# Visual-Behavior/detr-tensorflow

Measured on AMD Instinct MI355X. Metric: images/sec training step, DETR-R50 800x1333 bs=8/GPU, higher is better.
Workload: dtype bf16

## Files before the change

### detr-tensorflow_amd/csrc/common.h

```cpp
#pragma once
#include <hip/hip_runtime.h>
#include <stdint.h>
#include <stdio.h>
#include <stdarg.h>
#include <stdlib.h>

#include "../../include/detr_hip.h"

namespace detr {

void set_error(const char *fmt, ...);

#define DETR_REQUIRE(cond, ...)                 \
    do {                                        \
        if (!(cond)) {                          \
            ::detr::set_error(__VA_ARGS__);     \
            return -1;                          \
        }                                       \
    } while (0)

#define DETR_LAUNCH_CHECK(name)                                                         \
    do {                                                                                \
        hipError_t e__ = hipGetLastError();                                             \
        if (e__ != hipSuccess) {                                                        \
            ::detr::set_error("%s: launch failed: %s", name, hipGetErrorString(e__));   \
            return -2;                                                                  \
        }                                                                               \
    } while (0)

void launch_splitk_reduce(const float *ws, int splits, long long part_stride, int rows, int cols, float *C, long long ldc,
                          float alpha, const float *scale, hipStream_t stream, const float *rs_ws = nullptr,
                          float *rs_out = nullptr, float rs_alpha = 1.0f, int ts_bm = 0, int ts_bn = 0, int ts_tiles_n = 0);

constexpr int MIN_WAVES_64X64 = 1;

#if defined(__HIPCC__)
__device__ __forceinline__ void wave_lds_sync() {
    __builtin_amdgcn_fence(__ATOMIC_SEQ_CST, "wavefront");
    __builtin_amdgcn_wave_barrier();
}
__device__ __forceinline__ void lds_barrier() {
    __builtin_amdgcn_fence(__ATOMIC_RELEASE, "workgroup", "local");
    __builtin_amdgcn_s_barrier();
    __builtin_amdgcn_fence(__ATOMIC_ACQUIRE, "workgroup", "local");
}
#endif

enum TuneKey {
    T_GEMM_TILE,
    T_SPLIT_XCD,
    T_GEMM_STREAM,
    T_GEMM_GROUP,
    T_STREAM_SL,
    T_STREAM_NW,
    T_CONV_HALO,
    T_CONV_TILE,
    T_DGRAD_S2_CLASSES,
    T_WGRAD_FUSED,
    T_WGRAD_FUSED_WGS,
    T_WGRAD_TILE,
    T_STEM_ROWS,
    T_ATTN_WAVES,
    T_ATTN_SPLIT,
    T_GEMM_K64,
    T_EPI_WIDE,
    T_SLAB_TS,
    T_GEMM_RING,
    T_RING_NS,
    T_RING_BN,
    T_RING_WGS,
    T_RING_ROWS,
    T_RING_WTILE,
    T_CONV_DMA,
    T_SPLIT3_T128,
    T_X3_DB,
    T_X3_T192,
    T_X3_WG_ROUNDS,
    T_X3_CONV,
    T_SPLIT3_ALL,
    T_COUNT
};
int tune(TuneKey k);

static inline bool aligned16(const void *p) { return (reinterpret_cast<uintptr_t>(p) & 15) == 0; }
static inline int cdiv(long long a, long long b) { return (int)((a + b - 1) / b); }

__host__ __device__ __forceinline__ uint32_t mix32(uint32_t x) {
    x ^= x >> 16; x *= 0x7feb352du;
    x ^= x >> 15; x *= 0x846ca68bu;
    x ^= x >> 16;
    return x;
}
__host__ __device__ __forceinline__ uint32_t drop_key(uint32_t site, const uint32_t *step) {
    return mix32((step ? *step : 0u) + site * 0x9E3779B9u);
}
__host__ __device__ __forceinline__ uint32_t drop_hash(uint32_t key, unsigned long long pair) {
    const uint32_t key2 = key * 0x85EBCA6Bu + 0xC2B2AE35u;
    uint32_t x = (uint32_t)pair ^ key;
    x ^= (uint32_t)(pair >> 32) * 0x9E3779B9u;
    x ^= x >> 16; x *= 0x7feb352du;
    x ^= key2;
    x ^= x >> 15; x *= 0x846ca68bu;
    x ^= x >> 16;
    return x;
}
__host__ __device__ __forceinline__ bool drop_keep(uint32_t key, unsigned long long idx, uint32_t thresh16) {
    const uint32_t h = drop_hash(key, idx >> 1);
    return ((idx & 1ull) ? (h >> 16) : (h & 0xFFFFu)) >= thresh16;
}
static inline uint32_t drop_thresh16(float p) { return (uint32_t)(p * 65536.0f); }

template <int CTRL, int ROW_MASK>
__device__ __forceinline__ float dpp_mov_f32(float identity, float x) {
    return __builtin_bit_cast(float, __builtin_amdgcn_update_dpp(__builtin_bit_cast(int, identity), __builtin_bit_cast(int, x),
                                                                 CTRL, ROW_MASK, 0xf, false));
}
__device__ __forceinline__ float wave_sum(float v) {
    v += dpp_mov_f32<0x111, 0xf>(0.0f, v);
    v += dpp_mov_f32<0x112, 0xf>(0.0f, v);
    v += dpp_mov_f32<0x114, 0xf>(0.0f, v);
    v += dpp_mov_f32<0x118, 0xf>(0.0f, v);
    v += dpp_mov_f32<0x142, 0xa>(0.0f, v);
    v += dpp_mov_f32<0x143, 0xc>(0.0f, v);
    return __builtin_bit_cast(float, __builtin_amdgcn_readlane(__builtin_bit_cast(int, v), 63));
}
__device__ __forceinline__ float wave_max(float v) {
    const float ninf = -INFINITY;
    v = fmaxf(v, dpp_mov_f32<0x111, 0xf>(ninf, v));
    v = fmaxf(v, dpp_mov_f32<0x112, 0xf>(ninf, v));
    v = fmaxf(v, dpp_mov_f32<0x114, 0xf>(ninf, v));
    v = fmaxf(v, dpp_mov_f32<0x118, 0xf>(ninf, v));
    v = fmaxf(v, dpp_mov_f32<0x142, 0xa>(ninf, v));
    v = fmaxf(v, dpp_mov_f32<0x143, 0xc>(ninf, v));
    return __builtin_bit_cast(float, __builtin_amdgcn_readlane(__builtin_bit_cast(int, v), 63));
}

}
```

### detr-tensorflow_amd/csrc/common.hip

```cpp
#include "common.h"
#include <string.h>

namespace detr {
static thread_local char g_err[512] = "";
void set_error(const char *fmt, ...) {
    va_list ap;
    va_start(ap, fmt);
    vsnprintf(g_err, sizeof(g_err), fmt, ap);
    va_end(ap);
}
static const char *const g_tune_names[T_COUNT] = {
    "DETR_HIP_GEMM_TILE",
    "DETR_HIP_SPLIT_XCD",
    "DETR_HIP_GEMM_STREAM",
    "DETR_HIP_GEMM_GROUP",
    "DETR_HIP_STREAM_SL",
    "DETR_HIP_STREAM_NW",
    "DETR_HIP_CONV_HALO",
    "DETR_HIP_CONV_TILE",
    "DETR_HIP_DGRAD_S2_CLASSES",
    "DETR_HIP_WGRAD_FUSED",
    "DETR_HIP_WGRAD_FUSED_WGS",
    "DETR_HIP_WGRAD_TILE",
    "DETR_HIP_STEM_ROWS",
    "DETR_HIP_ATTN_WAVES",
    "DETR_HIP_ATTN_SPLIT",
    "DETR_HIP_GEMM_K64",
    "DETR_HIP_EPI_WIDE",
    "DETR_HIP_SLAB_TS",
    "DETR_HIP_GEMM_RING",
    "DETR_HIP_RING_NS",
    "DETR_HIP_RING_BN",
    "DETR_HIP_RING_WGS",
    "DETR_HIP_RING_ROWS",
    "DETR_HIP_RING_WTILE",
    "DETR_HIP_CONV_DMA",
    "DETR_HIP_SPLIT3_T128",
    "DETR_HIP_X3_DB",
    "DETR_HIP_X3_T192",
    "DETR_HIP_X3_WG_ROUNDS",
    "DETR_HIP_X3_CONV",
    "DETR_HIP_SPLIT3_ALL",
};
static int g_tune[T_COUNT];
static void load_tuning() {
    for (int i = 0; i < T_COUNT; ++i) {
        const char *v = getenv(g_tune_names[i]);
        __atomic_store_n(&g_tune[i], v ? atoi(v) : 0, __ATOMIC_RELAXED);
    }
}
static const bool g_tune_loaded = (load_tuning(), true);
int tune(TuneKey k) { return __atomic_load_n(&g_tune[k], __ATOMIC_RELAXED); }
}

extern "C" int detr_hip_reload_tuning(void) {
    detr::load_tuning();
    return 0;
}
extern "C" const char *detr_hip_last_error(void) { return detr::g_err; }
extern "C" int detr_hip_abi_version(void) { return DETR_HIP_ABI_VERSION; }
__global__ __launch_bounds__(256) void zero_fill_kernel(uint4 *__restrict__ p16, size_t n16, unsigned char *__restrict__ tail, int ntail) {
    const uint4 z = make_uint4(0u, 0u, 0u, 0u);
    for (size_t i = blockIdx.x * (size_t)blockDim.x + threadIdx.x; i < n16; i += (size_t)gridDim.x * blockDim.x) p16[i] = z;
    if (blockIdx.x == 0 && (int)threadIdx.x < ntail) tail[threadIdx.x] = 0;
}

extern "C" int detr_hip_memset_zero(void *ptr, size_t bytes, void *stream) {
    if (bytes == 0) return 0;
    unsigned char *b = reinterpret_cast<unsigned char *>(ptr);
    const size_t head = (16 - (reinterpret_cast<uintptr_t>(b) & 15)) & 15;
    if (head >= bytes || bytes < 64) {
        if (bytes > 255) { detr::set_error("memset_zero: %zu unaligned bytes", bytes); return -2; }
        hipLaunchKernelGGL(zero_fill_kernel, dim3(1), dim3(256), 0, (hipStream_t)stream, nullptr, (size_t)0, b, (int)bytes);
    } else {
        if (head) hipLaunchKernelGGL(zero_fill_kernel, dim3(1), dim3(256), 0, (hipStream_t)stream, nullptr, (size_t)0, b, (int)head);
        const size_t n16 = (bytes - head) / 16;
        const int ntail = (int)((bytes - head) % 16);
        size_t grid = (n16 + 255) / 256;
        if (grid > 2048) grid = 2048;
        if (grid < 1) grid = 1;
        hipLaunchKernelGGL(zero_fill_kernel, dim3((unsigned)grid), dim3(256), 0, (hipStream_t)stream, reinterpret_cast<uint4 *>(b + head), n16,
                           b + head + n16 * 16, ntail);
    }
    hipError_t e = hipGetLastError();
    if (e != hipSuccess) {
        detr::set_error("memset_zero: %s", hipGetErrorString(e));
        return -2;
    }
    return 0;
}
#include <stddef.h>
#define DETR_OFF(S, f) (int32_t)offsetof(S, f)
extern "C" int detr_hip_struct_layout(int32_t which, int32_t *out, int32_t cap) {
    int n = 0;
#define DETR_PUT(v) do { if (n < cap) out[n] = (v); ++n; } while (0)
    switch (which) {
    case 0:
        DETR_PUT((int32_t)sizeof(detr_reduce_desc));
        DETR_PUT(DETR_OFF(detr_reduce_desc, ws)); DETR_PUT(DETR_OFF(detr_reduce_desc, splits)); DETR_PUT(DETR_OFF(detr_reduce_desc, part_stride));
        DETR_PUT(DETR_OFF(detr_reduce_desc, rows)); DETR_PUT(DETR_OFF(detr_reduce_desc, cols)); DETR_PUT(DETR_OFF(detr_reduce_desc, C));
        DETR_PUT(DETR_OFF(detr_reduce_desc, ldc)); DETR_PUT(DETR_OFF(detr_reduce_desc, alpha)); DETR_PUT(DETR_OFF(detr_reduce_desc, scale));
        DETR_PUT(DETR_OFF(detr_reduce_desc, rs_ws)); DETR_PUT(DETR_OFF(detr_reduce_desc, rs_out)); DETR_PUT(DETR_OFF(detr_reduce_desc, rs_alpha));
        DETR_PUT(DETR_OFF(detr_reduce_desc, ts_bm)); DETR_PUT(DETR_OFF(detr_reduce_desc, ts_bn)); DETR_PUT(DETR_OFF(detr_reduce_desc, ts_tiles_n));
        break;
    case 1:
        DETR_PUT((int32_t)sizeof(detr_gemm_desc));
        DETR_PUT(DETR_OFF(detr_gemm_desc, M)); DETR_PUT(DETR_OFF(detr_gemm_desc, N)); DETR_PUT(DETR_OFF(detr_gemm_desc, K));
        DETR_PUT(DETR_OFF(detr_gemm_desc, A)); DETR_PUT(DETR_OFF(detr_gemm_desc, lda)); DETR_PUT(DETR_OFF(detr_gemm_desc, a_kcontig));
        DETR_PUT(DETR_OFF(detr_gemm_desc, B)); DETR_PUT(DETR_OFF(detr_gemm_desc, ldb)); DETR_PUT(DETR_OFF(detr_gemm_desc, b_kcontig));
        DETR_PUT(DETR_OFF(detr_gemm_desc, C)); DETR_PUT(DETR_OFF(detr_gemm_desc, ldc)); DETR_PUT(DETR_OFF(detr_gemm_desc, batch));
        DETR_PUT(DETR_OFF(detr_gemm_desc, batch_inner)); DETR_PUT(DETR_OFF(detr_gemm_desc, sA0)); DETR_PUT(DETR_OFF(detr_gemm_desc, sA1));
        DETR_PUT(DETR_OFF(detr_gemm_desc, sB0)); DETR_PUT(DETR_OFF(detr_gemm_desc, sB1)); DETR_PUT(DETR_OFF(detr_gemm_desc, sC0));
        DETR_PUT(DETR_OFF(detr_gemm_desc, sC1)); DETR_PUT(DETR_OFF(detr_gemm_desc, alpha)); DETR_PUT(DETR_OFF(detr_gemm_desc, scale));
        DETR_PUT(DETR_OFF(detr_gemm_desc, bias)); DETR_PUT(DETR_OFF(detr_gemm_desc, residual)); DETR_PUT(DETR_OFF(detr_gemm_desc, ldr));
        DETR_PUT(DETR_OFF(detr_gemm_desc, mask)); DETR_PUT(DETR_OFF(detr_gemm_desc, ldmask)); DETR_PUT(DETR_OFF(detr_gemm_desc, act));
        DETR_PUT(DETR_OFF(detr_gemm_desc, split_k)); DETR_PUT(DETR_OFF(detr_gemm_desc, workspace)); DETR_PUT(DETR_OFF(detr_gemm_desc, workspace_bytes));
        DETR_PUT(DETR_OFF(detr_gemm_desc, dropout_p)); DETR_PUT(DETR_OFF(detr_gemm_desc, dropout_seed)); DETR_PUT(DETR_OFF(detr_gemm_desc, compute));
        DETR_PUT(DETR_OFF(detr_gemm_desc, rowsum_a)); DETR_PUT(DETR_OFF(detr_gemm_desc, rowsum_alpha)); DETR_PUT(DETR_OFF(detr_gemm_desc, b_dtype));
        DETR_PUT(DETR_OFF(detr_gemm_desc, a_dtype)); DETR_PUT(DETR_OFF(detr_gemm_desc, c_dtype)); DETR_PUT(DETR_OFF(detr_gemm_desc, r_dtype));
        DETR_PUT(DETR_OFF(detr_gemm_desc, m_dtype)); DETR_PUT(DETR_OFF(detr_gemm_desc, dropout_step)); DETR_PUT(DETR_OFF(detr_gemm_desc, defer_out));
        DETR_PUT(DETR_OFF(detr_gemm_desc, maskbits_out)); DETR_PUT(DETR_OFF(detr_gemm_desc, ld_maskbits_out));
        DETR_PUT(DETR_OFF(detr_gemm_desc, ln_gamma)); DETR_PUT(DETR_OFF(detr_gemm_desc, ln_beta)); DETR_PUT(DETR_OFF(detr_gemm_desc, ln_y));
        DETR_PUT(DETR_OFF(detr_gemm_desc, ln_mean)); DETR_PUT(DETR_OFF(detr_gemm_desc, ln_rstd)); DETR_PUT(DETR_OFF(detr_gemm_desc, ln_add));
        DETR_PUT(DETR_OFF(detr_gemm_desc, ln_add_rows)); DETR_PUT(DETR_OFF(detr_gemm_desc, ln_y2)); DETR_PUT(DETR_OFF(detr_gemm_desc, ln_y16));
        DETR_PUT(DETR_OFF(detr_gemm_desc, ln_eps));
        break;
    case 2:
        DETR_PUT((int32_t)sizeof(detr_conv3x3_desc));
        DETR_PUT(DETR_OFF(detr_conv3x3_desc, N)); DETR_PUT(DETR_OFF(detr_conv3x3_desc, Hi)); DETR_PUT(DETR_OFF(detr_conv3x3_desc, Wi));
        DETR_PUT(DETR_OFF(detr_conv3x3_desc, Ci)); DETR_PUT(DETR_OFF(detr_conv3x3_desc, Ho)); DETR_PUT(DETR_OFF(detr_conv3x3_desc, Wo));
        DETR_PUT(DETR_OFF(detr_conv3x3_desc, Co)); DETR_PUT(DETR_OFF(detr_conv3x3_desc, stride)); DETR_PUT(DETR_OFF(detr_conv3x3_desc, pad));
        DETR_PUT(DETR_OFF(detr_conv3x3_desc, x)); DETR_PUT(DETR_OFF(detr_conv3x3_desc, w)); DETR_PUT(DETR_OFF(detr_conv3x3_desc, y));
        DETR_PUT(DETR_OFF(detr_conv3x3_desc, alpha)); DETR_PUT(DETR_OFF(detr_conv3x3_desc, scale)); DETR_PUT(DETR_OFF(detr_conv3x3_desc, bias));
        DETR_PUT(DETR_OFF(detr_conv3x3_desc, residual)); DETR_PUT(DETR_OFF(detr_conv3x3_desc, mask)); DETR_PUT(DETR_OFF(detr_conv3x3_desc, act));
        DETR_PUT(DETR_OFF(detr_conv3x3_desc, split)); DETR_PUT(DETR_OFF(detr_conv3x3_desc, workspace)); DETR_PUT(DETR_OFF(detr_conv3x3_desc, workspace_bytes));
        DETR_PUT(DETR_OFF(detr_conv3x3_desc, compute)); DETR_PUT(DETR_OFF(detr_conv3x3_desc, w_dtype)); DETR_PUT(DETR_OFF(detr_conv3x3_desc, x_dtype));
        DETR_PUT(DETR_OFF(detr_conv3x3_desc, y_dtype)); DETR_PUT(DETR_OFF(detr_conv3x3_desc, r_dtype)); DETR_PUT(DETR_OFF(detr_conv3x3_desc, m_dtype));
        DETR_PUT(DETR_OFF(detr_conv3x3_desc, maskbits_out));
        break;
    case 3:
        DETR_PUT((int32_t)sizeof(detr_stem_desc));
        DETR_PUT(DETR_OFF(detr_stem_desc, N)); DETR_PUT(DETR_OFF(detr_stem_desc, H)); DETR_PUT(DETR_OFF(detr_stem_desc, W));
        DETR_PUT(DETR_OFF(detr_stem_desc, Ho)); DETR_PUT(DETR_OFF(detr_stem_desc, Wo)); DETR_PUT(DETR_OFF(detr_stem_desc, img));
        DETR_PUT(DETR_OFF(detr_stem_desc, w)); DETR_PUT(DETR_OFF(detr_stem_desc, y)); DETR_PUT(DETR_OFF(detr_stem_desc, alpha));
        DETR_PUT(DETR_OFF(detr_stem_desc, scale)); DETR_PUT(DETR_OFF(detr_stem_desc, bias)); DETR_PUT(DETR_OFF(detr_stem_desc, act));
        DETR_PUT(DETR_OFF(detr_stem_desc, split)); DETR_PUT(DETR_OFF(detr_stem_desc, workspace)); DETR_PUT(DETR_OFF(detr_stem_desc, workspace_bytes));
        DETR_PUT(DETR_OFF(detr_stem_desc, compute)); DETR_PUT(DETR_OFF(detr_stem_desc, w_dtype)); DETR_PUT(DETR_OFF(detr_stem_desc, y_dtype));
        break;
    case 4:
        DETR_PUT((int32_t)sizeof(detr_layernorm_desc));
        DETR_PUT(DETR_OFF(detr_layernorm_desc, rows)); DETR_PUT(DETR_OFF(detr_layernorm_desc, C)); DETR_PUT(DETR_OFF(detr_layernorm_desc, eps));
        DETR_PUT(DETR_OFF(detr_layernorm_desc, x)); DETR_PUT(DETR_OFF(detr_layernorm_desc, gamma)); DETR_PUT(DETR_OFF(detr_layernorm_desc, beta));
        DETR_PUT(DETR_OFF(detr_layernorm_desc, y)); DETR_PUT(DETR_OFF(detr_layernorm_desc, mean)); DETR_PUT(DETR_OFF(detr_layernorm_desc, rstd));
        DETR_PUT(DETR_OFF(detr_layernorm_desc, add)); DETR_PUT(DETR_OFF(detr_layernorm_desc, add_rows)); DETR_PUT(DETR_OFF(detr_layernorm_desc, y2));
        DETR_PUT(DETR_OFF(detr_layernorm_desc, y16)); DETR_PUT(DETR_OFF(detr_layernorm_desc, dy)); DETR_PUT(DETR_OFF(detr_layernorm_desc, dx));
        DETR_PUT(DETR_OFF(detr_layernorm_desc, dgamma)); DETR_PUT(DETR_OFF(detr_layernorm_desc, dbeta)); DETR_PUT(DETR_OFF(detr_layernorm_desc, workspace));
        DETR_PUT(DETR_OFF(detr_layernorm_desc, workspace_bytes)); DETR_PUT(DETR_OFF(detr_layernorm_desc, dx_add));
        DETR_PUT(DETR_OFF(detr_layernorm_desc, dx_drop)); DETR_PUT(DETR_OFF(detr_layernorm_desc, dropout_p)); DETR_PUT(DETR_OFF(detr_layernorm_desc, dropout_site));
        DETR_PUT(DETR_OFF(detr_layernorm_desc, dropout_step)); DETR_PUT(DETR_OFF(detr_layernorm_desc, dx_drop16));
        DETR_PUT(DETR_OFF(detr_layernorm_desc, defer_blocks_out)); DETR_PUT(DETR_OFF(detr_layernorm_desc, dy_add));
        break;
    case 5:
        DETR_PUT((int32_t)sizeof(detr_attn_desc));
        DETR_PUT(DETR_OFF(detr_attn_desc, B)); DETR_PUT(DETR_OFF(detr_attn_desc, H)); DETR_PUT(DETR_OFF(detr_attn_desc, T));
        DETR_PUT(DETR_OFF(detr_attn_desc, S)); DETR_PUT(DETR_OFF(detr_attn_desc, q)); DETR_PUT(DETR_OFF(detr_attn_desc, ldq));
        DETR_PUT(DETR_OFF(detr_attn_desc, k)); DETR_PUT(DETR_OFF(detr_attn_desc, ldk)); DETR_PUT(DETR_OFF(detr_attn_desc, v));
        DETR_PUT(DETR_OFF(detr_attn_desc, ldv)); DETR_PUT(DETR_OFF(detr_attn_desc, o)); DETR_PUT(DETR_OFF(detr_attn_desc, ldo));
        DETR_PUT(DETR_OFF(detr_attn_desc, lse)); DETR_PUT(DETR_OFF(detr_attn_desc, d_o)); DETR_PUT(DETR_OFF(detr_attn_desc, ldd_o));
        DETR_PUT(DETR_OFF(detr_attn_desc, dq)); DETR_PUT(DETR_OFF(detr_attn_desc, lddq)); DETR_PUT(DETR_OFF(detr_attn_desc, dk));
        DETR_PUT(DETR_OFF(detr_attn_desc, lddk)); DETR_PUT(DETR_OFF(detr_attn_desc, dv)); DETR_PUT(DETR_OFF(detr_attn_desc, lddv));
        DETR_PUT(DETR_OFF(detr_attn_desc, delta)); DETR_PUT(DETR_OFF(detr_attn_desc, scale)); DETR_PUT(DETR_OFF(detr_attn_desc, dropout_p));
        DETR_PUT(DETR_OFF(detr_attn_desc, dropout_site)); DETR_PUT(DETR_OFF(detr_attn_desc, dropout_step)); DETR_PUT(DETR_OFF(detr_attn_desc, compute));
        DETR_PUT(DETR_OFF(detr_attn_desc, io_dtype)); DETR_PUT(DETR_OFF(detr_attn_desc, dropmask));
        break;
    case 6:
        DETR_PUT((int32_t)sizeof(detr_setloss_desc));
        DETR_PUT(DETR_OFF(detr_setloss_desc, levels)); DETR_PUT(DETR_OFF(detr_setloss_desc, B)); DETR_PUT(DETR_OFF(detr_setloss_desc, Q));
        DETR_PUT(DETR_OFF(detr_setloss_desc, C)); DETR_PUT(DETR_OFF(detr_setloss_desc, R)); DETR_PUT(DETR_OFF(detr_setloss_desc, logits));
        DETR_PUT(DETR_OFF(detr_setloss_desc, sL_l)); DETR_PUT(DETR_OFF(detr_setloss_desc, sL_b)); DETR_PUT(DETR_OFF(detr_setloss_desc, sL_q));
        DETR_PUT(DETR_OFF(detr_setloss_desc, boxes)); DETR_PUT(DETR_OFF(detr_setloss_desc, sB_l)); DETR_PUT(DETR_OFF(detr_setloss_desc, sB_b));
        DETR_PUT(DETR_OFF(detr_setloss_desc, sB_q)); DETR_PUT(DETR_OFF(detr_setloss_desc, t_bbox)); DETR_PUT(DETR_OFF(detr_setloss_desc, t_class));
        DETR_PUT(DETR_OFF(detr_setloss_desc, background_class));
        break;
    case 7:
        DETR_PUT((int32_t)sizeof(detr_input_desc));
        DETR_PUT(DETR_OFF(detr_input_desc, B)); DETR_PUT(DETR_OFF(detr_input_desc, Hs)); DETR_PUT(DETR_OFF(detr_input_desc, Ws));
        DETR_PUT(DETR_OFF(detr_input_desc, Hd)); DETR_PUT(DETR_OFF(detr_input_desc, Wd)); DETR_PUT(DETR_OFF(detr_input_desc, src));
        DETR_PUT(DETR_OFF(detr_input_desc, src_batch_stride)); DETR_PUT(DETR_OFF(detr_input_desc, dst)); DETR_PUT(DETR_OFF(detr_input_desc, lut));
        DETR_PUT(DETR_OFF(detr_input_desc, perm)); DETR_PUT(DETR_OFF(detr_input_desc, interpolation));
        break;
    case 8:
        DETR_PUT((int32_t)sizeof(detr_postprocess_desc));
        DETR_PUT(DETR_OFF(detr_postprocess_desc, B)); DETR_PUT(DETR_OFF(detr_postprocess_desc, Q)); DETR_PUT(DETR_OFF(detr_postprocess_desc, C));
        DETR_PUT(DETR_OFF(detr_postprocess_desc, logits)); DETR_PUT(DETR_OFF(detr_postprocess_desc, sL_b)); DETR_PUT(DETR_OFF(detr_postprocess_desc, sL_q));
        DETR_PUT(DETR_OFF(detr_postprocess_desc, boxes)); DETR_PUT(DETR_OFF(detr_postprocess_desc, sB_b)); DETR_PUT(DETR_OFF(detr_postprocess_desc, sB_q));
// ... 76 lines not shown
```

### detr-tensorflow_amd/csrc/gemm_f32.hip

```cpp
#include "gemm_core.h"
#include "gemm_bf16_core.h"
#include "gemm_stream.h"

#include "gemm_kernels.h"
#include "gemm_x3.h"
#include "gemm_ring.h"

namespace detr {

struct ReduceOne {
    const float *ws; int splits; long long part_stride; int rows, cols; float *C; long long ldc;
    float alpha; const float *scale; int vec; const float *rs_ws; float *rs_out; float rs_alpha; int nblocks;
    int ts_bm, ts_bn, ts_tn;
};
struct ReduceGroupArgs { ReduceOne r[GEMM_MAX_GROUP]; };

template <int G>
__device__ __forceinline__ void splitk_reduce_body(const float *__restrict__ ws, int splits, long long part_stride,
                                                   int rows, int cols, float *__restrict__ C, long long ldc,
                                                   float alpha, const float *__restrict__ scale, int vec,
                                                   const float *__restrict__ rs_ws, float *__restrict__ rs_out,
                                                   float rs_alpha, const int bid, const int nbid,
                                                   const int ts_bm = 0, const int ts_bn = 0, const int ts_tn = 1) {
    constexpr int OUT = 256 / G;
    __shared__ float4 red[G][OUT];
    if (rs_ws) {
        for (int m = bid * 256 + threadIdx.x; m < rows; m += nbid * 256) {
            float t = 0.0f;
            for (int k = 0; k < splits; ++k) t += rs_ws[(long long)k * rows + m];
            rs_out[m] += rs_alpha * t;
        }
    }
    const int lo = threadIdx.x % OUT, grp = threadIdx.x / OUT;
    if (ts_bm > 0) {
        __shared__ float tr[OUT][5];
        const int upt = (ts_bm * ts_bn) >> 2;
        const long long total = part_stride >> 2;
        for (long long base = (long long)bid * OUT; base < total; base += (long long)nbid * OUT) {
            const long long i = base + lo;
            const bool valid = i < total;
            float4 s = make_float4(0.f, 0.f, 0.f, 0.f);
            if (valid) {
                const float *p = ws + i * 4;
#pragma unroll 4
                for (int k = grp; k < splits; k += G) {
                    const float4 v = *reinterpret_cast<const float4 *>(p + k * part_stride);
                    s.x += v.x; s.y += v.y; s.z += v.z; s.w += v.w;
                }
            }
            red[grp][lo] = s;
            __syncthreads();
            if (grp == 0) {
#pragma unroll
                for (int q = 1; q < G; ++q) {
                    const float4 t = red[q][lo];
                    s.x += t.x; s.y += t.y; s.z += t.z; s.w += t.w;
                }
                tr[lo][0] = s.x; tr[lo][1] = s.y; tr[lo][2] = s.z; tr[lo][3] = s.w;
            }
            __syncthreads();
            if (grp == 0 && valid) {
                const int qb = lo & ~3, t = lo & 3;
                const long long iq = base + qb;
                const int tile = (int)(iq / upt), u = (int)(iq - (long long)tile * upt);
                int row0, col;
                slab_ts_unit(u, ts_bm, ts_bn, row0, col);
                const int row = row0 + (tile / ts_tn) * ts_bm + t;
                col += (tile % ts_tn) * ts_bn;
                if (row < rows && col < cols) {
                    const float4 v = make_float4(tr[qb][t], tr[qb + 1][t], tr[qb + 2][t], tr[qb + 3][t]);
                    float4 sc = make_float4(1.f, 1.f, 1.f, 1.f);
                    if (scale) sc = *reinterpret_cast<const float4 *>(scale + col);
                    float4 *dst = reinterpret_cast<float4 *>(C + (long long)row * ldc + col);
                    float4 o = *dst;
                    o.x += alpha * sc.x * v.x; o.y += alpha * sc.y * v.y; o.z += alpha * sc.z * v.z; o.w += alpha * sc.w * v.w;
                    *dst = o;
                }
            }
        }
    } else if (vec) {
        const int c4n = cols >> 2;
        const long long total = (long long)rows * c4n;
        for (long long base = (long long)bid * OUT; base < total; base += (long long)nbid * OUT) {
            const long long i = base + lo;
            const bool valid = i < total;
            int r = 0, c = 0;
            float4 s = make_float4(0.f, 0.f, 0.f, 0.f);
            if (valid) {
                r = (int)(i / c4n);
                c = (int)(i - (long long)r * c4n) * 4;
                const float *p = ws + (long long)r * cols + c;
#pragma unroll 4
                for (int k = grp; k < splits; k += G) {
                    const float4 v = *reinterpret_cast<const float4 *>(p + k * part_stride);
                    s.x += v.x; s.y += v.y; s.z += v.z; s.w += v.w;
                }
            }
            red[grp][lo] = s;
            __syncthreads();
            if (grp == 0 && valid) {
#pragma unroll
                for (int q = 1; q < G; ++q) {
                    const float4 t = red[q][lo];
                    s.x += t.x; s.y += t.y; s.z += t.z; s.w += t.w;
                }
                float4 sc = make_float4(1.f, 1.f, 1.f, 1.f);
                if (scale) sc = *reinterpret_cast<const float4 *>(scale + c);
                float4 *dst = reinterpret_cast<float4 *>(C + (long long)r * ldc + c);
                float4 o = *dst;
                o.x += alpha * sc.x * s.x; o.y += alpha * sc.y * s.y; o.z += alpha * sc.z * s.z; o.w += alpha * sc.w * s.w;
                *dst = o;
            }
            __syncthreads();
        }
    } else {
        const long long total = (long long)rows * cols;
        for (long long i = bid * (long long)blockDim.x + threadIdx.x; i < total; i += (long long)nbid * blockDim.x) {
            const int r = (int)(i / cols), c = (int)(i - (long long)r * cols);
            float s = 0.f;
            for (int k = 0; k < splits; ++k) s += ws[k * part_stride + i];
            C[(long long)r * ldc + c] += alpha * (scale ? scale[c] : 1.0f) * s;
        }
    }
}

template <int G>
__global__ __launch_bounds__(256) void splitk_reduce_kernel(const float *__restrict__ ws, int splits, long long part_stride,
                                                            int rows, int cols, float *__restrict__ C, long long ldc,
                                                            float alpha, const float *__restrict__ scale, int vec,
                                                            const float *__restrict__ rs_ws, float *__restrict__ rs_out,
                                                            float rs_alpha, int ts_bm, int ts_bn, int ts_tn) {
    splitk_reduce_body<G>(ws, splits, part_stride, rows, cols, C, ldc, alpha, scale, vec, rs_ws, rs_out, rs_alpha, blockIdx.x,
                          gridDim.x, ts_bm, ts_bn, ts_tn);
}
template <int G>
__global__ __launch_bounds__(256) void splitk_reduce_group_kernel(ReduceGroupArgs R) {
    const ReduceOne &r = R.r[blockIdx.y];
    if ((int)blockIdx.x >= r.nblocks) return;
    splitk_reduce_body<G>(r.ws, r.splits, r.part_stride, r.rows, r.cols, r.C, r.ldc, r.alpha, r.scale, r.vec, r.rs_ws, r.rs_out,
                          r.rs_alpha, blockIdx.x, r.nblocks, r.ts_bm, r.ts_bn, r.ts_tn);
}

constexpr int REDUCE_MANY = 16;
struct ReduceManyArgs { ReduceOne r[REDUCE_MANY]; };
template <int G>
__global__ __launch_bounds__(256) void splitk_reduce_many_kernel(ReduceManyArgs R) {
    const ReduceOne &r = R.r[blockIdx.y];
    if ((int)blockIdx.x >= r.nblocks) return;
    splitk_reduce_body<G>(r.ws, r.splits, r.part_stride, r.rows, r.cols, r.C, r.ldc, r.alpha, r.scale, r.vec, r.rs_ws, r.rs_out,
                          r.rs_alpha, blockIdx.x, r.nblocks, r.ts_bm, r.ts_bn, r.ts_tn);
}

static void reduce_plan(ReduceOne &r, bool &small) {
    r.vec = (r.cols % 4 == 0) && (r.ldc % 4 == 0) && (r.part_stride % 4 == 0) && aligned16(r.ws) && aligned16(r.C) &&
            (!r.scale || aligned16(r.scale));
    const bool ts = r.ts_bm > 0;
    const bool vec_like = r.vec || ts;
    const long long total = (long long)r.rows * (vec_like ? r.cols / 4 : r.cols);
    small = vec_like && total <= 65536 && r.splits >= 8;
    const long long units = ts ? r.part_stride / 4 : total;
    long long grid = vec_like ? (units + (small ? 15 : 63)) / (small ? 16 : 64) : (units + 255) / 256;
    if (grid > 8192) grid = 8192;
    if (grid < 1) grid = 1;
    r.nblocks = (int)grid;
}

void launch_splitk_reduce(const float *ws, int splits, long long part_stride, int rows, int cols, float *C, long long ldc,
                          float alpha, const float *scale, hipStream_t stream, const float *rs_ws, float *rs_out,
                          float rs_alpha, int ts_bm, int ts_bn, int ts_tiles_n) {
    ReduceOne r;
    r.ws = ws; r.splits = splits; r.part_stride = part_stride; r.rows = rows; r.cols = cols; r.C = C; r.ldc = ldc;
    r.alpha = alpha; r.scale = scale; r.rs_ws = rs_ws; r.rs_out = rs_out; r.rs_alpha = rs_alpha;
    r.ts_bm = ts_bm; r.ts_bn = ts_bn; r.ts_tn = ts_tiles_n > 0 ? ts_tiles_n : 1;
    bool small;
    reduce_plan(r, small);
    if (small)
        hipLaunchKernelGGL(splitk_reduce_kernel<16>, dim3((unsigned)r.nblocks), dim3(256), 0, stream, ws, splits, part_stride, rows, cols,
                           C, ldc, alpha, scale, r.vec, rs_ws, rs_out, rs_alpha, r.ts_bm, r.ts_bn, r.ts_tn);
    else
        hipLaunchKernelGGL(splitk_reduce_kernel<4>, dim3((unsigned)r.nblocks), dim3(256), 0, stream, ws, splits, part_stride, rows, cols,
                           C, ldc, alpha, scale, r.vec, rs_ws, rs_out, rs_alpha, r.ts_bm, r.ts_bn, r.ts_tn);
}

template <int BM, int BN, int WGM, int WGN>
static int launch_cfg(const GemmArgs &g, int batch, hipStream_t s, bool ak, bool bk) {
    GemmArgs a = g;
    a.tiles_m = cdiv(g.M, BM);
    a.tiles_n = cdiv(g.N, BN);
    dim3 grid((unsigned)(a.tiles_m * a.tiles_n), 1, (unsigned)(batch * g.split_k));
    dim3 block(GEMM_THREADS);
    if (ak && bk) hipLaunchKernelGGL((gemm_f32_kernel<BM, BN, WGM, WGN, true, true>), grid, block, 0, s, a);
    else if (ak && !bk) hipLaunchKernelGGL((gemm_f32_kernel<BM, BN, WGM, WGN, true, false>), grid, block, 0, s, a);
    else if (!ak && bk) hipLaunchKernelGGL((gemm_f32_kernel<BM, BN, WGM, WGN, false, true>), grid, block, 0, s, a);
    else hipLaunchKernelGGL((gemm_f32_kernel<BM, BN, WGM, WGN, false, false>), grid, block, 0, s, a);
    return 0;
}

template <int BM, int BN>
static int launch_x3(const GemmArgs &g, int batch, hipStream_t s, bool ak, bool bk) {
    GemmArgs a = g;
    a.tiles_m = cdiv(g.M, BM);
    a.tiles_n = cdiv(g.N, BN);
    dim3 grid((unsigned)(a.tiles_m * a.tiles_n), 1, (unsigned)(batch * g.split_k));
    dim3 block(GEMM_THREADS);
    const bool db = tune(T_X3_DB) == 1;
    if constexpr (BM == 192) {
        if (bk) hipLaunchKernelGGL((gemm_x3_kernel<BM, BN, true, true, false>), grid, block, 0, s, a);
        else hipLaunchKernelGGL((gemm_x3_kernel<BM, BN, true, false, false>), grid, block, 0, s, a);
    } else {
#define DETR_X3_LAUNCH(DB_)                                                                                              \
    do {                                                                                                                 \
        if (ak && bk) hipLaunchKernelGGL((gemm_x3_kernel<BM, BN, true, true, DB_>), grid, block, 0, s, a);               \
        else if (ak && !bk) hipLaunchKernelGGL((gemm_x3_kernel<BM, BN, true, false, DB_>), grid, block, 0, s, a);        \
        else if (!ak && bk) hipLaunchKernelGGL((gemm_x3_kernel<BM, BN, false, true, DB_>), grid, block, 0, s, a);        \
        else hipLaunchKernelGGL((gemm_x3_kernel<BM, BN, false, false, DB_>), grid, block, 0, s, a);                      \
    } while (0)
        if (db) {
            DETR_X3_LAUNCH(true);
        } else DETR_X3_LAUNCH(false);
    }
#undef DETR_X3_LAUNCH
    return 0;
}

template <int BM, int BN, int WGM, int WGN>
static int launch_cfg_bf16(const GemmArgs &g, int batch, hipStream_t s, bool ak, bool bk, int deep = 0) {
    GemmArgs a = g;
    a.tiles_m = cdiv(g.M, BM);
    a.tiles_n = cdiv(g.N, BN);
    dim3 grid((unsigned)(a.tiles_m * a.tiles_n), 1, (unsigned)(batch * g.split_k));
    dim3 block(GEMM_THREADS);
    if constexpr ((BM == 64 && BN == 64) || (BM == 128 && BN == 128)) {
        if (deep && g.a16 && g.b16) {
            if (ak && bk) hipLaunchKernelGGL((gemm_bf16c_k64_kernel<BM, BN, WGM, WGN, true, true>), grid, block, 0, s, a);
            else if (ak && !bk) hipLaunchKernelGGL((gemm_bf16c_k64_kernel<BM, BN, WGM, WGN, true, false>), grid, block, 0, s, a);
            else if (!ak && bk) hipLaunchKernelGGL((gemm_bf16c_k64_kernel<BM, BN, WGM, WGN, false, true>), grid, block, 0, s, a);
            else hipLaunchKernelGGL((gemm_bf16c_k64_kernel<BM, BN, WGM, WGN, false, false>), grid, block, 0, s, a);
            return 0;
        }
    }
#define DETR_BF16_LAUNCH(A16_, B16_)                                                                                          \
    do {                                                                                                                          \
        if (ak && bk) hipLaunchKernelGGL((gemm_bf16c_kernel<BM, BN, WGM, WGN, true, true, A16_, B16_>), grid, block, 0, s, a);        \
        else if (ak && !bk) hipLaunchKernelGGL((gemm_bf16c_kernel<BM, BN, WGM, WGN, true, false, A16_, B16_>), grid, block, 0, s, a); \
        else if (!ak && bk) hipLaunchKernelGGL((gemm_bf16c_kernel<BM, BN, WGM, WGN, false, true, A16_, B16_>), grid, block, 0, s, a); \
        else hipLaunchKernelGGL((gemm_bf16c_kernel<BM, BN, WGM, WGN, false, false, A16_, B16_>), grid, block, 0, s, a);               \
    } while (0)
    if (g.a16 && g.b16) DETR_BF16_LAUNCH(true, true);
    else if (g.a16) DETR_BF16_LAUNCH(true, false);
    else if (g.b16) DETR_BF16_LAUNCH(false, true);
    else DETR_BF16_LAUNCH(false, false);
#undef DETR_BF16_LAUNCH
    return 0;
}

}

using namespace detr;

struct GemmPlan {
    GemmArgs g;
    int batch, split;
    bool ak, bk, bf16c, partial;
    bool split3;
    int deep;
    int tile;
    long long part;
    int ts_bm, ts_bn, ts_tn;
    EpiArgs final_e;
    const detr_gemm_desc *d;
};

static bool gemm_split3_shape(const detr_gemm_desc *d) {
    return d->compute == 2 && d->N > 32 && (tune(T_SPLIT3_ALL) == 1 || (d->N >= 128 && d->K >= 256 && d->M >= 128));
}
static int gemm_pick_tile(const detr_gemm_desc *d, int split, int batch) {
    const bool bf16c = d->compute == 1;
    const int force = tune(T_GEMM_TILE);
    int tile = 0;
    if (bf16c) {
        const long long t128 = (long long)cdiv(d->M, 128) * cdiv(d->N, 128) * batch;
        const bool big_split = (d->N >= 128 && d->K >= 16384) || (d->M >= 512 && d->N >= 512 && d->K >= 4096) ||
                               (d->K >= 4096 && ((d->M >= 256 && d->N >= 2048) || (d->M >= 2048 && d->N >= 256)));
        const bool big_plain = (d->K >= 1024 && t128 >= 512) || (d->K >= 512 && d->N >= 512 && t128 >= 1024) ||
                               (d->K >= 512 && d->N >= 256 && t128 >= 2048);
        const bool small = (split > 1) ? !big_split : !big_plain;
        if (force == 2) tile = 2;
        else if (force == 5) tile = 4;
        else if (force == 3 || (force == 0 && small)) tile = 0;
        else if (force == 0 && split > 1 && d->M <= 64) tile = 4;
        else tile = 1;
        if (tile == 1 && split > 1 && batch == 1 && d->a_dtype == 1 && d->b_dtype == 1 && !d->a_kcontig && !d->b_kcontig && !d->rowsum_a &&
            tune(T_GEMM_RING) != 2 && tune(T_GEMM_RING) != 3 && tune(T_SLAB_TS) != 2 && d->M % 8 == 0 && d->N % 8 == 0 && d->lda % 8 == 0 &&
            d->ldb % 8 == 0 && aligned16(d->A) && aligned16(d->B) && aligned16(d->C) && d->ldc % 4 == 0 && (!d->scale || aligned16(d->scale))) {
            const int wt = tune(T_RING_WTILE);
            if (wt == 1 && d->N >= 256) tile = 6;
            else if (wt == 2 && d->M >= 256) tile = 7;
        }
    } else if (gemm_split3_shape(d)) {
        const long long t128 = (long long)cdiv(d->M, 128) * cdiv(d->N, 128) * batch * split;
        const int lim = tune(T_SPLIT3_T128) > 0 ? tune(T_SPLIT3_T128) : 192;
        if (force == 1 || (force == 0 && t128 >= lim)) tile = 1;
        else if (force == 2) tile = 2;
        else tile = 0;
        if (tile == 1 && force == 0 && split == 1 && batch == 1 && d->a_kcontig && !d->rowsum_a && tune(T_X3_T192) != 2) {
            const long long slots = 512;
            const long long t192 = (long long)cdiv(d->M, 192) * cdiv(d->N, 128);
            const long long r128 = (t128 + slots - 1) / slots, r192 = (t192 + slots - 1) / slots;
            if (tune(T_X3_T192) == 1 || 3 * r192 < 2 * r128) tile = 8;
        }
        if (tile == 1 && force == 0 && split == 1 && batch == 1 && tune(T_X3_T192) != 2 && d->M >= 4096) {
            const long long over = t128 % 512;
            if ((t128 > 512 && over > 0 && over <= 128) || (t128 <= 384 && d->K <= 512)) tile = 2;
        }
    } else if (force == 1) tile = 1;
    else if (force == 2) tile = 2;
    else if (force == 3) tile = 0;
    else if (force == 4) tile = 3;
    else if (force == 5) tile = 4;
    else if (force == 6) tile = 5;
    else if (d->N <= 32) tile = 3;
    else tile = 0;
    return tile;
}
static void gemm_tile_dims(bool bf16c, int tile, int &bm, int &bn, bool &ts_ok) {
    ts_ok = true;
    if (tile == 1) { bm = 128; bn = 128; }
    else if (tile == 8 && !bf16c) { bm = 192; bn = 128; }
    else if (tile == 6 && bf16c) { bm = 128; bn = 256; }
    else if (tile == 7 && bf16c) { bm = 256; bn = 128; }
    else if (tile == 2) { bm = 128; bn = 64; }
    else if (tile == 4 && bf16c) { bm = 64; bn = 128; }
    else if (tile == 0) { bm = 64; bn = 64; }
    else { bm = bn = 0; ts_ok = false; }
// ... 97 lines not shown
                 (!d->mask || bits_in || (d->ldmask % 8 == 0 && aligned16(d->mask))) && (!d->scale || aligned16(d->scale)) &&
                 (!d->bias || aligned16(d->bias)) && (tune(T_EPI_WIDE) != 2 || bits_in || bits_out);
    DETR_REQUIRE(!(bits_in || bits_out) || (bf16c && g.e.wide16 && (!bits_in || d->ldmask >= d->N / 8) && (!bits_out || d->ld_maskbits_out >= d->N / 8)),
                 "gemm: bit-packed masks need bf16 C / residual, N %% 8 == 0, 16-byte aligned rows, no split-K / batch, and a row pitch >= N / 8 bytes");

    const bool ak = d->a_kcontig != 0, bk = d->b_kcontig != 0;
    DETR_REQUIRE(!(bf16c && d->a_dtype == 1 && !ak) || (d->lda % 8 == 0 && d->M % 8 == 0 && aligned16(d->A)),
                 "gemm: an M-contiguous bf16 A operand needs lda %% 8 == 0, M %% 8 == 0 and a 16-byte aligned base (16-byte requests)");
    DETR_REQUIRE(!(bf16c && d->b_dtype == 1 && !bk) || (d->ldb % 8 == 0 && d->N % 8 == 0 && aligned16(d->B)),
                 "gemm: an N-contiguous bf16 B operand needs ldb %% 8 == 0, N %% 8 == 0 and a 16-byte aligned base (16-byte requests)");
    const int tile = gemm_pick_tile(d, split, batch);
    long long part = (long long)d->M * d->N;
    int ts_bm = 0, ts_bn = 0;
    const long long rs_extra = d->rowsum_a ? d->M : 0;
    bool ts = gemm_slab_ts(d, split, batch, tile, ts_bm, ts_bn);
    const long long part_ts = ts ? (long long)cdiv(d->M, ts_bm) * cdiv(d->N, ts_bn) * ts_bm * ts_bn : 0;
    const bool ws_ok = split > 1 && batch == 1 && d->workspace && aligned16(d->workspace);
    if (ts && !(ws_ok && d->workspace_bytes >= (long long)split * (part_ts + rs_extra) * 4)) ts = false;
    if (ts) part = part_ts;
    const bool partial = ws_ok && d->workspace_bytes >= (long long)split * (part + rs_extra) * 4;
    DETR_REQUIRE(!(d->rowsum_a && split > 1 && !partial), "gemm: rowsum_a with split_k needs the workspace path");
    g.rowsum = d->rowsum_a;
    g.rowsum_alpha = d->rowsum_alpha;
    g.rowsum_partial = 0;
    g.b16 = d->b_dtype == 1;
    g.a16 = d->a_dtype == 1;
    g.split_xcd = tune(T_SPLIT_XCD) != 2;
    g.slab_ts = 0;
    p.ts_bm = p.ts_bn = 0; p.ts_tn = 1;
    EpiArgs final_e = g.e;
    if (partial) {
        g.C = d->workspace;
        g.ldc = d->N;
        g.part_stride = part;
        g.e.alpha = 1.0f;
        g.e.scale = nullptr;
        g.e.atomic = 0;
        g.e.vec = (d->N % 4 == 0);
        if (ts) {
            g.slab_ts = 1;
            p.ts_bm = ts_bm; p.ts_bn = ts_bn; p.ts_tn = cdiv(d->N, ts_bn);
        }
        if (d->rowsum_a) {
            g.rowsum = d->workspace + (long long)split * part;
            g.rowsum_partial = 1;
        }
    }
    {
        const int k64 = tune(T_GEMM_K64);
        const int per_split = cdiv(d->K, split);
        p.deep = (bf16c && g.a16 && g.b16 && (tile == 0 || tile == 1) && k64 != 2 &&
                  (k64 == 1 || (per_split >= 512 && (tile == 0 || split > 1)))) ? 1 : 0;
    }
    p.batch = batch; p.split = split; p.ak = ak; p.bk = bk; p.bf16c = bf16c; p.partial = partial; p.tile = tile;
    p.split3 = gemm_split3_shape(d) && (tile == 0 || tile == 1 || tile == 2 || tile == 8);
    p.part = part; p.final_e = final_e; p.d = d;
    return 0;
}

static bool gemm_stream_eligible(const GemmPlan &p) {
    const detr_gemm_desc *d = p.d;
    const GemmArgs &g = p.g;
    if (!(p.bf16c && g.a16 && g.b16 && g.e.c16 && p.ak && p.batch == 1 && p.split == 1 && !g.rowsum)) return false;
    const bool ext = d->alpha != 1.0f || d->dropout_p > 0.0f;
    if (!((d->K == 64 || d->K == 128 || d->K == 256) && d->N % 64 == 0 && d->M >= ((d->K == 256 && d->N >= 1024) ? 4096 : 16384))) return false;
    if (d->scale || (ext && d->K != 256) || !(d->act == 0 || d->act == 1)) return false;
    if (d->residual && !(g.e.r16 && d->ldr % 8 == 0 && aligned16(d->residual))) return false;
    if (d->mask && g.e.m16 != 2 && !(g.e.m16 && d->ldmask % 8 == 0 && aligned16(d->mask))) return false;
    if (!(d->lda % 8 == 0 && d->ldb % 8 == 0 && d->ldc % 8 == 0 && aligned16(d->A) && aligned16(d->B) && aligned16(d->C))) return false;
    const long long ldm_eff = g.e.m16 == 2 ? 0 : d->ldmask;
    long long pitch = d->ldr > ldm_eff ? d->ldr : ldm_eff;
    if (d->ldc > pitch) pitch = d->ldc;
    const long long span = (long long)(d->M - 1) * pitch + d->N;
    if (span * 2 > BUF_MAX_BYTES) return false;
    if (d->maskbits_out && (p.bk || !d->residual || d->mask || ext)) return false;
    return tune(T_GEMM_STREAM) != 2;
}

static void gemm_stream_launch(const GemmPlan &p, hipStream_t s) {
    const detr_gemm_desc *d = p.d;
    StreamArgs a;
    a.M = d->M; a.N = d->N;
    a.A = reinterpret_cast<const unsigned short *>(d->A); a.lda = d->lda;
    a.B = reinterpret_cast<const unsigned short *>(d->B); a.ldb = d->ldb;
    a.C = reinterpret_cast<unsigned short *>(d->C); a.ldc = d->ldc;
    a.res = reinterpret_cast<const unsigned short *>(d->residual); a.ldr = d->ldr;
    a.mask = reinterpret_cast<const unsigned short *>(d->mask); a.ldm = d->ldmask;
    a.mbits_out = d->maskbits_out; a.ld_mbits = d->ld_maskbits_out;
    a.bias = d->bias;
    a.act = d->act;
    a.alpha = d->alpha;
    a.drop_scale = p.g.e.drop_scale; a.drop_thresh = p.g.e.drop_thresh; a.drop_seed = p.g.e.drop_seed; a.drop_step = p.g.e.drop_step;
    a.n_tiles = a.row_tiles = a.q = 0;
    const bool mb = d->mask && d->m_dtype == 2;
    if (d->K == 64) launch_gemm_stream<64>(a, p.bk, s, mb);
    else if (d->K == 128) launch_gemm_stream<128>(a, p.bk, s, mb);
    else launch_gemm_stream<256>(a, p.bk, s, mb);
}

static int gemm_ln_launch(const GemmPlan &p, hipStream_t s) {
    const detr_gemm_desc *d = p.d;
    const GemmArgs &g0 = p.g;
    DETR_REQUIRE(p.bf16c && d->N == LN_TILE_N && d->ldc == LN_TILE_N && p.ak && p.bk && g0.b16 && p.batch == 1 && p.split == 1,
                 "gemm + LayerNorm: needs compute = 1, N = ldc = 256, k-contiguous A and bf16 k-contiguous B, no batch / split_k");
    DETR_REQUIRE(d->act == 0 && !d->scale && !d->mask && !g0.e.c16 && !g0.e.r16 && !d->rowsum_a && !d->maskbits_out && d->K % 8 == 0,
                 "gemm + LayerNorm: epilogue is bias, alpha, dropout and an fp32 residual only (K %% 8 == 0)");
    DETR_REQUIRE(d->ln_gamma && d->ln_beta && d->ln_mean && d->ln_rstd && (!d->ln_y2 || (d->ln_add && d->ln_add_rows > 0)),
                 "gemm + LayerNorm: gamma, beta, mean, rstd are required (and add / add_rows with y2)");
    DETR_REQUIRE((!d->residual || (d->ldr % 4 == 0 && aligned16(d->residual))) && aligned16(d->C) && aligned16(d->ln_y) &&
                 (!d->bias || aligned16(d->bias)) && aligned16(d->ln_gamma) && aligned16(d->ln_beta) &&
                 (!d->ln_y2 || (aligned16(d->ln_y2) && aligned16(d->ln_add))) && (!d->ln_y16 || aligned16(d->ln_y16)),
                 "gemm + LayerNorm: rows must be 16-byte aligned");
    GemmArgs a = g0;
    a.tiles_m = cdiv(d->M, LN_TILE_M);
    a.tiles_n = 1;
    a.ln.gamma = d->ln_gamma; a.ln.beta = d->ln_beta; a.ln.y = d->ln_y; a.ln.mean = d->ln_mean; a.ln.rstd = d->ln_rstd;
    a.ln.add = d->ln_add; a.ln.add_rows = d->ln_add_rows; a.ln.y2 = d->ln_y2; a.ln.y16 = d->ln_y16; a.ln.eps = d->ln_eps;
    const dim3 grid((unsigned)a.tiles_m), block(GEMM_THREADS);
    if (g0.a16) hipLaunchKernelGGL(gemm_bf16c_ln_kernel<true>, grid, block, 0, s, a);
    else hipLaunchKernelGGL(gemm_bf16c_ln_kernel<false>, grid, block, 0, s, a);
    DETR_LAUNCH_CHECK("gemm + LayerNorm");
    if (d->defer_out) d->defer_out->splits = 0;
    return 0;
}

static bool gemm_ring_eligible(const GemmPlan &p, RingPlan &rp) {
    const detr_gemm_desc *d = p.d;
    const GemmArgs &g = p.g;
    const int mode = tune(T_GEMM_RING);
    if (mode == 2) return false;
    if (!(p.bf16c && g.a16 && g.b16 && p.ak && p.batch == 1 && p.split == 1 && !g.rowsum && !d->ln_y)) return false;
    if (!(d->K % RING_BK == 0 && d->K >= 2 * RING_BK && d->N >= 128 && d->N % 8 == 0 && d->lda % 8 == 0 && d->ldb % 8 == 0 && aligned16(d->A) &&
          aligned16(d->B))) return false;
    const bool tall = d->M >= 4096 && d->K >= 512;
    const bool dec_ffn = d->M >= 512 && d->K >= 1024;
    const bool k256 = d->K == 256 && d->N >= 1024 && (d->M >= 16384 || (d->M >= 4096 && !p.bk));
    if (mode != 1 && !(tall || dec_ffn || k256)) return false;
    return gemm_ring_plan(d->M, d->N, d->K, rp);
}

static bool gemm_ring_f32_eligible(const GemmPlan &p, RingPlan &rp) {
    const detr_gemm_desc *d = p.d;
    const GemmArgs &g = p.g;
    const int mode = tune(T_GEMM_RING);
    if (mode == 2) return false;
    if (p.bf16c || p.split3 || g.a16 || g.b16 || !p.ak || p.batch != 1 || p.split != 1 || g.rowsum || d->ln_y) return false;
    if (d->c_dtype || d->r_dtype || d->m_dtype) return false;
    if (!(d->K % 32 == 0 && d->K >= 64 && d->N >= 128 && d->lda % 4 == 0 && d->ldb % 4 == 0 && aligned16(d->A) && aligned16(d->B) &&
          (p.bk || d->N % 4 == 0))) return false;
    if (mode != 1 && !(d->M >= 16384)) return false;
    return gemm_ring_f32_plan(d->M, d->N, d->K, rp);
}

static int gemm_launch(const GemmPlan &p, hipStream_t s) {
    const GemmArgs &g = p.g;
    const detr_gemm_desc *d = p.d;
    const int batch = p.batch;
    const bool ak = p.ak, bk = p.bk;
    if (d->ln_y) return gemm_ln_launch(p, s);
    {
        RingPlan rp;
        const bool ring_first = tune(T_GEMM_STREAM) != 3 && gemm_ring_eligible(p, rp);
        if (!ring_first && gemm_stream_eligible(p)) {
            gemm_stream_launch(p, s);
            DETR_LAUNCH_CHECK("gemm (stream)");
            return 0;
        }
        if (ring_first) {
            if (gemm_ring_launch(g, bk, rp, s)) return -1;
            DETR_LAUNCH_CHECK("gemm (ring)");
            if (d->defer_out) d->defer_out->splits = 0;
            return 0;
        }
        if (gemm_ring_f32_eligible(p, rp)) {
            if (gemm_ring_f32_launch(g, bk, rp, s)) return -1;
            DETR_LAUNCH_CHECK("gemm (ring, fp32)");
            if (d->defer_out) d->defer_out->splits = 0;
            return 0;
        }
    }
    const bool ring_wgrad = p.bf16c && (p.tile == 1 || p.tile == 6 || p.tile == 7) && g.a16 && g.b16 && !ak && !bk && batch == 1 && p.split > 1 &&
                            g.slab_ts && !g.rowsum && d->M % 8 == 0 && d->N % 8 == 0 && d->lda % 8 == 0 && d->ldb % 8 == 0 && aligned16(d->A) &&
                            aligned16(d->B) && tune(T_GEMM_RING) != 2 && tune(T_GEMM_RING) != 3;
    DETR_REQUIRE(ring_wgrad || (p.tile != 6 && p.tile != 7), "gemm: the 128 x 256 / 256 x 128 tiles exist for the ring weight gradient only "
                 "(tile-ordered slabs in a workspace of detr_hip_workspace_bytes_gemm bytes are required)");
    if (ring_wgrad) {
        if (gemm_ring_wgrad_launch(g, p.ts_bm, p.ts_bn, p.split, s)) return -1;
    } else if (p.bf16c) {
        if (p.tile == 2) launch_cfg_bf16<128, 64, 2, 2>(g, batch, s, ak, bk);
        else if (p.tile == 4) launch_cfg_bf16<64, 128, 2, 2>(g, batch, s, ak, bk);
        else if (p.tile == 0) launch_cfg_bf16<64, 64, 2, 2>(g, batch, s, ak, bk, p.deep);
        else launch_cfg_bf16<128, 128, 2, 2>(g, batch, s, ak, bk, p.deep);
    } else if (p.split3 && p.tile == 8) launch_x3<192, 128>(g, batch, s, ak, bk);
    else if (p.split3 && p.tile == 1) launch_x3<128, 128>(g, batch, s, ak, bk);
    else if (p.split3 && p.tile == 2) launch_x3<128, 64>(g, batch, s, ak, bk);
    else if (p.split3) launch_x3<64, 64>(g, batch, s, ak, bk);
    else if (p.tile == 1) launch_cfg<128, 128, 2, 2>(g, batch, s, ak, bk);
    else if (p.tile == 2) launch_cfg<128, 64, 2, 2>(g, batch, s, ak, bk);
    else if (p.tile == 3) launch_cfg<128, 32, 4, 1>(g, batch, s, ak, bk);
    else if (p.tile == 4) launch_cfg<64, 256, 1, 4>(g, batch, s, ak, bk);
    else if (p.tile == 5) launch_cfg<256, 64, 4, 1>(g, batch, s, ak, bk);
    else launch_cfg<64, 64, 2, 2>(g, batch, s, ak, bk);
    DETR_LAUNCH_CHECK("gemm");
    if (p.partial && d->defer_out) {
        detr_reduce_desc *o = d->defer_out;
        o->ws = d->workspace; o->splits = p.split; o->part_stride = p.part; o->rows = d->M; o->cols = d->N;
        o->C = d->C; o->ldc = d->ldc; o->alpha = p.final_e.alpha; o->scale = p.final_e.scale;
        o->rs_ws = d->rowsum_a ? d->workspace + (long long)p.split * p.part : nullptr;
        o->rs_out = d->rowsum_a; o->rs_alpha = d->rowsum_alpha;
        o->ts_bm = p.ts_bm; o->ts_bn = p.ts_bn; o->ts_tiles_n = p.ts_tn;
        return 0;
    }
    if (d->defer_out) d->defer_out->splits = 0;
    if (p.partial) {
        launch_splitk_reduce(d->workspace, p.split, p.part, d->M, d->N, d->C, d->ldc, p.final_e.alpha, p.final_e.scale, s,
                             d->rowsum_a ? d->workspace + (long long)p.split * p.part : nullptr, d->rowsum_a, d->rowsum_alpha,
                             p.ts_bm, p.ts_bn, p.ts_tn);
        DETR_LAUNCH_CHECK("gemm split-k reduce");
    }
    return 0;
}

extern "C" int detr_hip_gemm_family(const detr_gemm_desc *d) {
    GemmPlan p;
    if (gemm_prepare(d, p)) return -1;
    if (d->ln_y) return 4;
    RingPlan rp;
    const bool ring_first = tune(T_GEMM_STREAM) != 3 && gemm_ring_eligible(p, rp);
    if (!ring_first && gemm_stream_eligible(p)) return 1;
    if (ring_first) return 2;
    if (gemm_ring_f32_eligible(p, rp)) return 3;
    const GemmArgs &g = p.g;
    const bool ring_wgrad = p.bf16c && (p.tile == 1 || p.tile == 6 || p.tile == 7) && g.a16 && g.b16 && !p.ak && !p.bk && p.batch == 1 && p.split > 1 &&
                            g.slab_ts && !g.rowsum && d->M % 8 == 0 && d->N % 8 == 0 && d->lda % 8 == 0 && d->ldb % 8 == 0 && aligned16(d->A) &&
                            aligned16(d->B) && tune(T_GEMM_RING) != 2 && tune(T_GEMM_RING) != 3;
    return ring_wgrad ? 5 : 0;
}

extern "C" int detr_hip_gemm_f32(const detr_gemm_desc *d, void *stream) {
    GemmPlan p;
    if (gemm_prepare(d, p)) return -1;
    return gemm_launch(p, (hipStream_t)stream);
}

template <bool AK, bool BKC>
static void launch_group_f32(const GemmGroupArgs &G, dim3 grid, hipStream_t s, bool split3) {
    if (split3) hipLaunchKernelGGL((gemm_x3_group_kernel<64, 64, AK, BKC>), grid, dim3(GEMM_THREADS), 0, s, G);
    else hipLaunchKernelGGL((gemm_f32_group_kernel<64, 64, 2, 2, AK, BKC>), grid, dim3(GEMM_THREADS), 0, s, G);
}
template <bool AK, bool BKC, bool A16, bool B16>
static void launch_group_bf16(const GemmGroupArgs &G, dim3 grid, hipStream_t s) {
    hipLaunchKernelGGL((gemm_bf16c_group_kernel<64, 64, 2, 2, AK, BKC, A16, B16>), grid, dim3(GEMM_THREADS), 0, s, G);
}

extern "C" int detr_hip_gemm_group_f32(const detr_gemm_desc *descs, int32_t n, void *stream) {
    DETR_REQUIRE(descs != nullptr && n >= 1 && n <= 64, "gemm group: 1..64 descriptors");
    hipStream_t s = (hipStream_t)stream;
    int done = 0;
    while (done < n) {
        const int m = (n - done) < GEMM_MAX_GROUP ? (n - done) : GEMM_MAX_GROUP;
        GemmPlan p[GEMM_MAX_GROUP];
        for (int i = 0; i < m; ++i) {
            DETR_REQUIRE(!descs[done + i].ln_y, "gemm group: the fused LayerNorm (ln_y) exists for single launches only");
            if (gemm_prepare(descs + done + i, p[i])) return -1;
        }
        bool same = m > 1 && tune(T_GEMM_GROUP) != 2;
        for (int i = 0; i < m && same; ++i)
            same = p[i].tile == 0 && p[i].batch == 1 && p[i].bf16c == p[0].bf16c && p[i].split3 == p[0].split3 && p[i].ak == p[0].ak && p[i].bk == p[0].bk &&
                   p[i].g.a16 == p[0].g.a16 && p[i].g.b16 == p[0].g.b16 && (p[i].split == 1 || p[i].partial) &&
                   !gemm_stream_eligible(p[i]);
        if (same) { RingPlan rp; for (int i = 0; i < m && same; ++i) same = !gemm_ring_eligible(p[i], rp) && !gemm_ring_f32_eligible(p[i], rp); }
        if (!same) {
            for (int i = 0; i < m; ++i)
                if (gemm_launch(p[i], s)) return -1;
            done += m;
            continue;
        }
        GemmGroupArgs G;
        G.n = m;
        G.work_off[0] = 0;
        for (int i = 0; i < m; ++i) {
            G.g[i] = p[i].g;
            G.g[i].tiles_m = cdiv(p[i].g.M, 64);
            G.g[i].tiles_n = cdiv(p[i].g.N, 64);
            G.work_off[i + 1] = G.work_off[i] + G.g[i].tiles_m * G.g[i].tiles_n * p[i].split;
        }
        for (int i = m; i < GEMM_MAX_GROUP; ++i) { G.g[i] = G.g[0]; G.work_off[i + 1] = G.work_off[m]; }
        const dim3 grid((unsigned)G.work_off[m]);
        const bool ak = p[0].ak, bk = p[0].bk, a16 = p[0].g.a16 != 0, b16 = p[0].g.b16 != 0;
#define DETR_GROUP_BF16(A16_, B16_)                                          \
    do {                                                                     \
        if (ak && bk) launch_group_bf16<true, true, A16_, B16_>(G, grid, s);    \
        else if (ak) launch_group_bf16<true, false, A16_, B16_>(G, grid, s);    \
        else if (bk) launch_group_bf16<false, true, A16_, B16_>(G, grid, s);    \
        else launch_group_bf16<false, false, A16_, B16_>(G, grid, s);           \
    } while (0)
        if (p[0].bf16c) {
            if (a16 && b16) DETR_GROUP_BF16(true, true);
            else if (a16) DETR_GROUP_BF16(true, false);
            else if (b16) DETR_GROUP_BF16(false, true);
            else DETR_GROUP_BF16(false, false);
        } else if (ak && bk) launch_group_f32<true, true>(G, grid, s, p[0].split3);
        else if (ak) launch_group_f32<true, false>(G, grid, s, p[0].split3);
        else if (bk) launch_group_f32<false, true>(G, grid, s, p[0].split3);
        else launch_group_f32<false, false>(G, grid, s, p[0].split3);
#undef DETR_GROUP_BF16
        DETR_LAUNCH_CHECK("gemm group");
        ReduceGroupArgs R;
        int nr = 0;
        unsigned rx = 1;
        bool all_small = true, any_small = false;
        for (int i = 0; i < m; ++i) {
            const detr_gemm_desc *d = p[i].d;
            if (d->defer_out) {
                detr_reduce_desc *o = d->defer_out;
                o->splits = 0;
                if (p[i].partial) {
                    o->ws = d->workspace; o->splits = p[i].split; o->part_stride = p[i].part; o->rows = d->M; o->cols = d->N;
                    o->C = d->C; o->ldc = d->ldc; o->alpha = p[i].final_e.alpha; o->scale = p[i].final_e.scale;
                    o->rs_ws = d->rowsum_a ? d->workspace + (long long)p[i].split * p[i].part : nullptr;
                    o->rs_out = d->rowsum_a; o->rs_alpha = d->rowsum_alpha;
                    o->ts_bm = p[i].ts_bm; o->ts_bn = p[i].ts_bn; o->ts_tiles_n = p[i].ts_tn;
                }
                continue;
            }
            if (!p[i].partial) continue;
            ReduceOne &r = R.r[nr];
            r.ws = d->workspace; r.splits = p[i].split; r.part_stride = p[i].part; r.rows = d->M; r.cols = d->N;
            r.C = d->C; r.ldc = d->ldc; r.alpha = p[i].final_e.alpha; r.scale = p[i].final_e.scale;
            r.rs_ws = d->rowsum_a ? d->workspace + (long long)p[i].split * p[i].part : nullptr;
            r.rs_out = d->rowsum_a; r.rs_alpha = d->rowsum_alpha;
            r.ts_bm = p[i].ts_bm; r.ts_bn = p[i].ts_bn; r.ts_tn = p[i].ts_tn;
            bool small;
            reduce_plan(r, small);
            all_small = all_small && small;
            any_small = any_small || small;
            rx = (unsigned)r.nblocks > rx ? (unsigned)r.nblocks : rx;
            ++nr;
        }
        if (nr > 0 && (all_small || !any_small)) {
            for (int i = nr; i < GEMM_MAX_GROUP; ++i) R.r[i] = R.r[0];
            if (all_small) hipLaunchKernelGGL(splitk_reduce_group_kernel<16>, dim3(rx, (unsigned)nr), dim3(256), 0, s, R);
            else hipLaunchKernelGGL(splitk_reduce_group_kernel<4>, dim3(rx, (unsigned)nr), dim3(256), 0, s, R);
            DETR_LAUNCH_CHECK("gemm group split-k reduce");
        } else if (nr > 0) {
            for (int i = 0; i < nr; ++i) {
                const ReduceOne &r = R.r[i];
                launch_splitk_reduce(r.ws, r.splits, r.part_stride, r.rows, r.cols, r.C, r.ldc, r.alpha, r.scale, s, r.rs_ws, r.rs_out,
                                     r.rs_alpha, r.ts_bm, r.ts_bn, r.ts_tn);
            }
            DETR_LAUNCH_CHECK("gemm group split-k reduce (sequential)");
        }
        done += m;
    }
    return 0;
}


extern "C" int detr_hip_splitk_reduce_many(const detr_reduce_desc *descs, int32_t n, void *stream) {
    DETR_REQUIRE(descs != nullptr && n >= 1, "splitk_reduce_many: bad args");
    hipStream_t s = (hipStream_t)stream;
    for (int pass = 0; pass < 2; ++pass) {
        ReduceManyArgs R;
        int cnt = 0;
        unsigned rx = 1;
        auto flush = [&]() {
            if (cnt == 0) return;
            for (int i = cnt; i < REDUCE_MANY; ++i) R.r[i] = R.r[0];
            if (pass == 0) hipLaunchKernelGGL(splitk_reduce_many_kernel<16>, dim3(rx, (unsigned)cnt), dim3(256), 0, s, R);
            else hipLaunchKernelGGL(splitk_reduce_many_kernel<4>, dim3(rx, (unsigned)cnt), dim3(256), 0, s, R);
            cnt = 0;
            rx = 1;
        };
        for (int i = 0; i < n; ++i) {
            const detr_reduce_desc &d = descs[i];
            if (d.splits <= 0) continue;
            DETR_REQUIRE(d.ws && d.C && d.rows > 0 && d.cols > 0, "splitk_reduce_many: entry %d is malformed", i);
            ReduceOne r;
            r.ws = d.ws; r.splits = d.splits; r.part_stride = d.part_stride; r.rows = d.rows; r.cols = d.cols; r.C = d.C; r.ldc = d.ldc;
            r.alpha = d.alpha; r.scale = d.scale; r.rs_ws = d.rs_ws; r.rs_out = d.rs_out; r.rs_alpha = d.rs_alpha;
            r.ts_bm = d.ts_bm; r.ts_bn = d.ts_bn; r.ts_tn = d.ts_tiles_n > 0 ? d.ts_tiles_n : 1;
            DETR_REQUIRE(d.ts_bm == 0 || ((d.ts_bm == 64 || d.ts_bm == 128 || d.ts_bm == 256) && (d.ts_bn == 64 || d.ts_bn == 128 || d.ts_bn == 256) && d.ts_tiles_n > 0 &&
                                          d.part_stride % ((long long)d.ts_bm * d.ts_bn) == 0),
                         "splitk_reduce_many: entry %d has a malformed tile-ordered slab description", i);
            bool small;
            reduce_plan(r, small);
            if (small != (pass == 0)) continue;
            R.r[cnt++] = r;
            rx = (unsigned)r.nblocks > rx ? (unsigned)r.nblocks : rx;
            if (cnt == REDUCE_MANY) flush();
        }
        flush();
    }
    DETR_LAUNCH_CHECK("splitk_reduce_many");
    return 0;
}
```

### detr-tensorflow_amd/csrc/gemm_ring.h

```cpp
#pragma once
#include "gemm_kernels.h"

namespace detr {

typedef __attribute__((address_space(3))) void lds_void_t;
constexpr int RING_BK = 64;
constexpr int RING_THREADS = 512;
constexpr int RING_STAGE_ROW = RING_BK * 2;

struct RingArgs {
    GemmArgs g;
    int tile_rows;
    int a_rows8;
    int stage_bytes;
    int dump_off;
};

struct RingPlan {
    int tm, tn, ns;
    int tile_rows, tiles_m, tiles_n, wgs;
    int a_rows8, stage_bytes, dump_off, lds_bytes;
    double cost;
};
bool gemm_ring_plan(int M, int N, int K, RingPlan &p);
int gemm_ring_wgrad_launch(const GemmArgs &g, int bm, int bn, int split, hipStream_t s);
int gemm_ring_launch(const GemmArgs &g, bool b_kcontig, const RingPlan &p, hipStream_t s);
bool gemm_ring_f32_plan(int M, int N, int K, RingPlan &p);
int gemm_ring_f32_launch(const GemmArgs &g, bool b_kcontig, const RingPlan &p, hipStream_t s);

template <int N>
__device__ __forceinline__ void ring_wait_vmcnt() {
    static_assert(N >= 0 && N < 64, "vmcnt is a 6-bit counter");
    asm volatile("s_waitcnt vmcnt(%0)" ::"n"(N) : "memory");
}

__device__ __forceinline__ void ring_dma_piece(u32x4 rs, unsigned lds_addr, unsigned voff) {
    asm volatile("s_mov_b32 m0, %0\n\ts_nop 0\n\tbuffer_load_dwordx4 %1, %2, 0 offen lds" ::"s"(lds_addr), "v"(voff), "s"(rs) : "memory", "m0");
}
__device__ __forceinline__ u32x4 ring_rsrc(const void *base, unsigned bytes) {
    const unsigned long long b = (unsigned long long)base;
    u32x4 r;
    r[0] = (unsigned)b;
    r[1] = (unsigned)(b >> 32) & 0xFFFFu;
    r[2] = bytes;
    r[3] = 0x00020000u;
    return r;
}
__device__ __forceinline__ unsigned ring_lds_addr(char *p) {
    return (unsigned)(unsigned long long)(lds_void_t *)p;
}

template <int NP, int ES = 2>
struct RingDmaK {
    static constexpr int NPIECES = NP;
    const char *base;
    long long text;
    unsigned voff[NP];
    int lds_off[NP];
    int in_img[NP];
    __device__ __forceinline__ void init(const void *p, long long ld, int row0, int row_end, int rows_total, int K, int img_rows8,
                                         int lane, int wave) {
        base = reinterpret_cast<const char *>(p);
        text = ((long long)(rows_total - 1) * ld + K) * ES;
#pragma unroll
        for (int i = 0; i < NP; ++i) {
            const int P = wave + 8 * i;
            const int r = 8 * P + (lane >> 3);
            const int c = (lane & 7) ^ ((r >> 1) & 7);
            const int g = row0 + r;
            voff[i] = (g < row_end) ? (unsigned)((long long)g * ld * ES) + 16u * (unsigned)c : BUF_OOB;
            lds_off[i] = P * 1024;
            in_img[i] = (8 * P < img_rows8) ? -1 : 0;
        }
    }
    __device__ __forceinline__ u32x4 stage_rsrc(int k0, int K) const {
        const unsigned left = (k0 < K) ? (unsigned)(text - (long long)ES * k0) : 0u;
        return ring_rsrc(base + (long long)ES * k0, left);
    }
    __device__ __forceinline__ void issue_one(const int I, u32x4 rs, unsigned lds0, int img, int dump) const {
        const int off = dump + (in_img[I] & (img + lds_off[I] - dump));
        ring_dma_piece(rs, lds0 + (unsigned)off, voff[I]);
    }
    __device__ __forceinline__ void issue(int k0, int K, unsigned lds0, int img, int dump) const {
        const u32x4 rs = stage_rsrc(k0, K);
#pragma unroll
        for (int i = 0; i < NP; ++i) issue_one(i, rs, lds0, img, dump);
    }
};

template <int BMN>
struct RingDmaMN {
    static constexpr int NH = BMN / 128;
    static constexpr int NP = BMN / 64;
    const unsigned short *base;
    long long text;
    unsigned ld2b;
    unsigned voff[NP];
    int wave;
    __device__ __forceinline__ void init(const void *p, long long ld, int mn0, int MN, int K, int lane, int wave_) {
        wave = wave_;
        base = reinterpret_cast<const unsigned short *>(p);
        text = ((long long)(K - 1) * ld + MN) * 2;
        ld2b = (unsigned)(ld * 2);
        const int kr = lane >> 4, pc = lane & 15;
#pragma unroll
        for (int i = 0; i < NP; ++i) {
            const int P = wave + 8 * i;
            const int kb = P / NH, nh = P % NH;
            const int col = mn0 + nh * 128 + 8 * (pc ^ (4 * kr));
            voff[i] = (col + 8 <= MN) ? (unsigned)(4 * kb + kr) * ld2b + 2u * (unsigned)col : BUF_OOB;
        }
    }
    __device__ __forceinline__ u32x4 stage_rsrc(int k0, int K) const {
        const unsigned left = (k0 < K) ? (unsigned)(text - (long long)k0 * ld2b) : 0u;
        return ring_rsrc(base + (long long)k0 * (ld2b >> 1), left);
    }
    __device__ __forceinline__ void issue_one(const int I, u32x4 rs, unsigned lds0, int img, int) const {
        ring_dma_piece(rs, lds0 + (unsigned)(img + (wave + 8 * I) * 1024), voff[I]);
    }
    __device__ __forceinline__ void issue(int k0, int K, unsigned lds0, int img, int dump) const {
        const u32x4 rs = stage_rsrc(k0, K);
#pragma unroll
        for (int i = 0; i < NP; ++i) issue_one(i, rs, lds0, img, dump);
    }
};

template <int NH>
__device__ __forceinline__ int ring_tr_lane_off(int col_base, int lane) {
    const int g = lane >> 4, t = lane & 15;
    const int kr = t >> 2, q = t & 3;
    const int ibg = (col_base >> 4) + (g & 1);
    const int nh = ibg >> 3, ib = ibg & 7;
    return (2 * (g >> 1) * NH + nh) * 1024 + kr * 256 + (((2 * ib + (q >> 1)) ^ (4 * kr)) * 16) + (q & 1) * 8;
}
template <int NH>
__device__ __forceinline__ bf16x8 ring_frag_tr(const char *img, int lane_off, int kk) {
    const char *p = img + lane_off + kk * (4 * NH * 1024);
    typedef __attribute__((address_space(3))) s16x4 lds_s16x4;
    const s16x4 lo = __builtin_amdgcn_ds_read_tr16_b64_v4i16((lds_s16x4 *)p);
    const s16x4 hi = __builtin_amdgcn_ds_read_tr16_b64_v4i16((lds_s16x4 *)(p + NH * 1024));
    typedef short s16x8 __attribute__((ext_vector_type(8)));
    const s16x8 v = __builtin_shufflevector(lo, hi, 0, 1, 2, 3, 4, 5, 6, 7);
    return __builtin_bit_cast(bf16x8, v);
}

template <int IDX, int P0, int P1, int NPA_, class LA, class LB>
__device__ __forceinline__ void ring_issue_range(const LA &la, const LB &lb, u32x4 rsa, u32x4 rsb, unsigned lds0, int ia, int ib, int dump) {
    if constexpr (IDX < P1) {
        if constexpr (IDX >= P0) {
            if constexpr (IDX < NPA_) la.issue_one(IDX, rsa, lds0, ia, dump);
            else lb.issue_one(IDX - NPA_, rsb, lds0, ib, dump);
        }
        ring_issue_range<IDX + 1, P0, P1, NPA_>(la, lb, rsa, rsb, lds0, ia, ib, dump);
    }
}
template <int NM, int TM, int TN, bool AKC, bool BKC, class LA, class LB>
__device__ __forceinline__ void ring_stage(const char *As, const char *Bs, f32x16 (&acc)[TM][TN], int a_lane, const int (&atr)[TM], int b_lane, const int (&btr)[TN],
                                           const int (&xo)[4], const LA &la, const LB &lb, int k_next, int K, unsigned lds0, int na, int nb, int dump) {
    const u32x4 rsa = la.stage_rsrc(k_next, K), rsb = lb.stage_rsrc(k_next, K);
    constexpr int NPA = TM, NPB = 2 * TN, PW = NPA + NPB;
    constexpr int READS = NM * (AKC ? 1 : 2) + TN * (BKC ? 1 : 2), MF = NM * TN;
    bf16x8 a[2][NM > 0 ? NM : 1], b[2][TN];
    auto read = [&](const int kk, const int set) {
#pragma unroll
        for (int mi = 0; mi < NM; ++mi) {
            if constexpr (AKC) a[set][mi] = *reinterpret_cast<const bf16x8 *>(As + a_lane + mi * (32 * RING_STAGE_ROW) + xo[kk]);
            else a[set][mi] = ring_frag_tr<TM / 2>(As, atr[mi], kk);
        }
#pragma unroll
        for (int ni = 0; ni < TN; ++ni) {
            if constexpr (BKC) b[set][ni] = *reinterpret_cast<const bf16x8 *>(Bs + b_lane + ni * (32 * RING_STAGE_ROW) + xo[kk]);
            else b[set][ni] = ring_frag_tr<TN>(Bs, btr[ni], kk);
        }
    };
    if constexpr (NM == 0) {
        ring_issue_range<0, 0, PW, NPA>(la, lb, rsa, rsb, lds0, na, nb, dump);
        return;
    } else {
// ... 122 lines not shown
        wave = wave_;
        base = reinterpret_cast<const char *>(p);
        text = ((long long)(K - 1) * ld + MN) * 4;
        ld4b = (unsigned)(ld * 4);
#pragma unroll
        for (int i = 0; i < NP; ++i) {
            const int P = wave + 8 * i;
            const int k = P * RPP + lane / LPR;
            const int col = mn0 + 4 * (lane % LPR);
            voff[i] = (col + 4 <= MN) ? (unsigned)k * ld4b + 4u * (unsigned)col : BUF_OOB;
        }
    }
    __device__ __forceinline__ u32x4 stage_rsrc(int k0, int K) const {
        const unsigned left = (k0 < K) ? (unsigned)(text - (long long)k0 * ld4b) : 0u;
        return ring_rsrc(base + (long long)k0 * ld4b, left);
    }
    __device__ __forceinline__ void issue_one(const int I, u32x4 rs, unsigned lds0, int img, int) const {
        ring_dma_piece(rs, lds0 + (unsigned)(img + (wave + 8 * I) * 1024), voff[I]);
    }
    __device__ __forceinline__ void issue(int k0, int K, unsigned lds0, int img, int dump) const {
        const u32x4 rs = stage_rsrc(k0, K);
#pragma unroll
        for (int i = 0; i < NP; ++i) issue_one(i, rs, lds0, img, dump);
    }
};

template <int NM, int TM, int TN, bool AKC, bool BKC, int BM, int BN, class LA, class LB>
__device__ __forceinline__ void ring_stage_f32(const char *As, const char *Bs, f32x16 (&acc)[TM][TN], int a_lane, int b_lane, const int (&xo8)[8],
                                               int h, const LA &la, const LB &lb, int k_next, int K, unsigned lds0, int na, int nb, int dump) {
    constexpr int NPA = LA::NPIECES, NPB = LB::NPIECES, PW = NPA + NPB;
    const u32x4 rsa = la.stage_rsrc(k_next, K), rsb = lb.stage_rsrc(k_next, K);
    if constexpr (NM == 0) {
        ring_issue_range<0, 0, PW, NPA>(la, lb, rsa, rsb, lds0, na, nb, dump);
        return;
    } else {
#pragma unroll
        for (int gq = 0; gq < 8; ++gq) {
            float av[2][NM], bv[2][TN];
#pragma unroll
            for (int mi = 0; mi < NM; ++mi) {
                if constexpr (AKC) {
                    const float4 v = *reinterpret_cast<const float4 *>(As + a_lane + mi * (32 * RING_STAGE_ROW) + xo8[gq]);
                    av[0][mi] = h ? v.y : v.x;
                    av[1][mi] = h ? v.w : v.z;
                } else {
                    av[0][mi] = *reinterpret_cast<const float *>(As + a_lane + mi * 128 + (4 * gq) * (BM * 4));
                    av[1][mi] = *reinterpret_cast<const float *>(As + a_lane + mi * 128 + (4 * gq + 2) * (BM * 4));
                }
            }
#pragma unroll
            for (int ni = 0; ni < TN; ++ni) {
                if constexpr (BKC) {
                    const float4 v = *reinterpret_cast<const float4 *>(Bs + b_lane + ni * (32 * RING_STAGE_ROW) + xo8[gq]);
                    bv[0][ni] = h ? v.y : v.x;
                    bv[1][ni] = h ? v.w : v.z;
                } else {
                    bv[0][ni] = *reinterpret_cast<const float *>(Bs + b_lane + ni * 128 + (4 * gq) * (BN * 4));
                    bv[1][ni] = *reinterpret_cast<const float *>(Bs + b_lane + ni * 128 + (4 * gq + 2) * (BN * 4));
                }
            }
            if (gq == 1) ring_issue_range<0, (0 * PW) / 4, (1 * PW) / 4, NPA>(la, lb, rsa, rsb, lds0, na, nb, dump);
            if (gq == 3) ring_issue_range<0, (1 * PW) / 4, (2 * PW) / 4, NPA>(la, lb, rsa, rsb, lds0, na, nb, dump);
            if (gq == 5) ring_issue_range<0, (2 * PW) / 4, (3 * PW) / 4, NPA>(la, lb, rsa, rsb, lds0, na, nb, dump);
            if (gq == 7) ring_issue_range<0, (3 * PW) / 4, (4 * PW) / 4, NPA>(la, lb, rsa, rsb, lds0, na, nb, dump);
#pragma unroll
            for (int j = 0; j < 2; ++j)
#pragma unroll
                for (int mi = 0; mi < NM; ++mi)
#pragma unroll
                    for (int ni = 0; ni < TN; ++ni) acc[mi][ni] = __builtin_amdgcn_mfma_f32_32x32x2f32(av[j][mi], bv[j][ni], acc[mi][ni], 0, 0, 0);
        }
    }
}

template <int TM, int TN, bool BKC, int NS>
__device__ __forceinline__ void gemm_ring_f32_body(const RingArgs &ra, const int id) {
    constexpr int BM = 64 * TM, BN = 128 * TN, WGM = 2, WGN = 4, BKF = 32;
    using T = TileCfg<BM, BN, WGM, WGN>;
    extern __shared__ __attribute__((aligned(1024))) char ring_smem[];
    const GemmArgs &g = ra.g;
    const int tid = threadIdx.x, lane = tid & 63;
    const int wave = __builtin_amdgcn_readfirstlane(tid >> 6);
    const int wm = wave / WGN, wn = wave % WGN;
    const int tn = id % g.tiles_n, tm = id / g.tiles_n;
    const int m0 = tm * ra.tile_rows, n0 = tn * BN;
    const int row_end = min(g.M, m0 + ra.tile_rows);
    const int my_rows = row_end - (m0 + wm * T::WTM);
    const int nmi = my_rows <= 0 ? 0 : (my_rows >= T::WTM ? TM : (my_rows + 31) >> 5);
    using LAt = RingDmaK<TM, 4>;
    LAt la;
    la.init(g.A, g.lda, m0, row_end, g.M, g.K, ra.a_rows8, lane, wave);
    using LB = typename std::conditional<BKC, RingDmaK<2 * TN, 4>, RingDmaMN32<BN>>::type;
    LB lb;
    if constexpr (BKC) lb.init(g.B, g.ldb, n0, g.N, g.N, g.K, BN, lane, wave);
    else lb.init(g.B, g.ldb, n0, g.N, g.K, lane, wave);
    constexpr int PW = LAt::NPIECES + LB::NPIECES;
    f32x16 acc[TM][TN];
#pragma unroll
    for (int i = 0; i < TM; ++i)
#pragma unroll
        for (int j = 0; j < TN; ++j)
#pragma unroll
            for (int r = 0; r < 16; ++r) acc[i][j][r] = 0.0f;
    const int a_bytes = ra.a_rows8 * RING_STAGE_ROW;
    const int dump = ra.dump_off;
    const unsigned lds0 = ring_lds_addr(ring_smem);
    auto stage_a = [&](int s) { return s * ra.stage_bytes; };
    auto stage_b = [&](int s) { return s * ra.stage_bytes + a_bytes; };
    const int l31 = lane & 31, h = lane >> 5;
    const int sw = (l31 >> 1) & 7;
    int xo8[8];
#pragma unroll
    for (int q = 0; q < 8; ++q) xo8[q] = 16 * (q ^ sw);
    const int a_lane = (wm * T::WTM + l31) * RING_STAGE_ROW;
    const int b_lane = BKC ? (wn * T::WTN + l31) * RING_STAGE_ROW : (wn * T::WTN + l31) * 4 + h * (BN * 4);
    const int nkt = g.K / BKF;
#pragma unroll
    for (int t = 0; t < NS - 1; ++t) {
        la.issue(t * BKF, g.K, lds0, stage_a(t), dump);
        lb.issue(t * BKF, g.K, lds0, stage_b(t), dump);
    }
    auto kloop = [&](auto NMC) {
        constexpr int NM = decltype(NMC)::value;
        int cur = 0, nxt = NS - 1;
        for (int t = 0; t < nkt; ++t) {
            ring_wait_vmcnt<(NS - 2) * PW>();
            __builtin_amdgcn_s_barrier();
            asm volatile("" ::: "memory");
            ring_stage_f32<NM, TM, TN, true, BKC, BM, BN>(ring_smem + stage_a(cur), ring_smem + stage_b(cur), acc, a_lane, b_lane, xo8, h, la, lb,
                                                          (t + NS - 1) * BKF, g.K, lds0, stage_a(nxt), stage_b(nxt), dump);
            __builtin_amdgcn_sched_barrier(0);
            cur = (cur + 1 == NS) ? 0 : cur + 1;
            nxt = (nxt + 1 == NS) ? 0 : nxt + 1;
        }
    };
    if (nmi == TM) kloop(std::integral_constant<int, TM>{});
    else if (TM >= 2 && nmi == TM - 1) kloop(std::integral_constant<int, (TM >= 2 ? TM - 1 : 0)>{});
    else if (TM >= 3 && nmi == TM - 2) kloop(std::integral_constant<int, (TM >= 3 ? TM - 2 : 0)>{});
    else if (TM >= 4 && nmi == TM - 3) kloop(std::integral_constant<int, (TM >= 4 ? TM - 3 : 0)>{});
    else kloop(std::integral_constant<int, 0>{});
    ring_wait_vmcnt<0>();
    __syncthreads();
    epilogue<BM, BN, WGM, WGN, false>(acc, reinterpret_cast<float *>(ring_smem), g.C, g.ldc, row_end, g.N, m0, n0, wm, wn, lane, wave, g.e);
}

template <int TM, int TN, bool BKC, int NS>
__global__ __launch_bounds__(RING_THREADS) void gemm_ring_f32_kernel(RingArgs ra) {
#if defined(__HIP_DEVICE_COMPILE__)
    gemm_ring_f32_body<TM, TN, BKC, NS>(ra, xcd_remap((int)blockIdx.x, (int)gridDim.x));
#endif
}

template <int TM, int TN, int NS>
__device__ __forceinline__ void gemm_ring_wgrad_body(const RingArgs &ra) {
    constexpr int BM = 64 * TM, BN = 128 * TN, WGM = 2, WGN = 4;
    static_assert(TM % 2 == 0, "the A image is made of 128-row pieces");
    using T = TileCfg<BM, BN, WGM, WGN>;
    extern __shared__ __attribute__((aligned(1024))) char ring_smem[];
    const GemmArgs &g = ra.g;
    const int tid = threadIdx.x, lane = tid & 63;
    const int wave = __builtin_amdgcn_readfirstlane(tid >> 6);
    const int wm = wave / WGN, wn = wave % WGN;
    const int tiles = g.tiles_m * g.tiles_n;
    const int id = xcd_remap((int)blockIdx.x, (int)gridDim.x);
    const int tile = id % tiles, split = id / tiles;
    const int tn = tile % g.tiles_n, tm = tile / g.tiles_n;
    const int m0 = tm * BM, n0 = tn * BN;
    const int nkt32 = (g.K + BF_BK - 1) / BF_BK;
    const int per = (nkt32 + g.split_k - 1) / g.split_k;
    const int kbeg = split * per * BF_BK;
    const int kend = min(g.K, kbeg + per * BF_BK);
    if (kbeg >= kend) return;
    RingDmaMN<BM> la;
    RingDmaMN<BN> lb;
    la.init(g.A, g.lda, m0, g.M, kend, lane, wave);
    lb.init(g.B, g.ldb, n0, g.N, kend, lane, wave);
    f32x16 acc[TM][TN];
#pragma unroll
    for (int i = 0; i < TM; ++i)
#pragma unroll
        for (int j = 0; j < TN; ++j)
#pragma unroll
            for (int r = 0; r < 16; ++r) acc[i][j][r] = 0.0f;
    constexpr int A_BYTES = BM * RING_STAGE_ROW, STAGE = (BM + BN) * RING_STAGE_ROW, PW = TM + 2 * TN;
    const unsigned lds0 = ring_lds_addr(ring_smem);
    int atr[TM], btr[TN];
#pragma unroll
    for (int mi = 0; mi < TM; ++mi) atr[mi] = ring_tr_lane_off<TM / 2>(wm * T::WTM + mi * 32, lane);
#pragma unroll
    for (int ni = 0; ni < TN; ++ni) btr[ni] = ring_tr_lane_off<TN>(wn * T::WTN + ni * 32, lane);
    const int xo[4] = {0, 0, 0, 0};
    const int nkt = (kend - kbeg + RING_BK - 1) / RING_BK;
#pragma unroll
    for (int t = 0; t < NS - 1; ++t) {
        la.issue(kbeg + t * RING_BK, kend, lds0, t * STAGE, 0);
        lb.issue(kbeg + t * RING_BK, kend, lds0, t * STAGE + A_BYTES, 0);
    }
    int cur = 0, nxt = NS - 1;
    for (int t = 0; t < nkt; ++t) {
        ring_wait_vmcnt<(NS - 2) * PW>();
        __builtin_amdgcn_s_barrier();
        asm volatile("" ::: "memory");
        ring_stage<TM, TM, TN, false, false>(ring_smem + cur * STAGE, ring_smem + cur * STAGE + A_BYTES, acc, 0, atr, 0, btr, xo, la, lb,
                                             kbeg + (t + NS - 1) * RING_BK, kend, lds0, nxt * STAGE, nxt * STAGE + A_BYTES, 0);
        __builtin_amdgcn_sched_barrier(0);
        cur = (cur + 1 == NS) ? 0 : cur + 1;
        nxt = (nxt + 1 == NS) ? 0 : nxt + 1;
    }
    ring_wait_vmcnt<0>();
    float4 *slab = reinterpret_cast<float4 *>(g.C + (long long)split * g.part_stride + (long long)tile * (BM * BN));
    const int w2 = 2 * wm + (wn >> 1);
#pragma unroll
    for (int mi = 0; mi < TM; ++mi)
#pragma unroll
        for (int ni = 0; ni < TN; ++ni) {
            const int blk = (w2 * TM + mi) * (2 * TN) + (wn & 1) * TN + ni;
#pragma unroll
            for (int q = 0; q < 4; ++q)
                slab[(blk * 4 + q) * 64 + lane] = make_float4(acc[mi][ni][4 * q], acc[mi][ni][4 * q + 1], acc[mi][ni][4 * q + 2], acc[mi][ni][4 * q + 3]);
        }
}

template <int TM, int TN, int NS>
__global__ __launch_bounds__(RING_THREADS) void gemm_ring_wgrad_kernel(RingArgs ra) {
#if defined(__HIP_DEVICE_COMPILE__)
    gemm_ring_wgrad_body<TM, TN, NS>(ra);
#endif
}

}
```

### detr-tensorflow_amd/csrc/gemm_ring.hip

```cpp
#include "gemm_ring.h"

namespace detr {

bool gemm_ring_plan(int M, int N, int K, RingPlan &p) {
    if (M < 1 || N < 128 || K < RING_BK || K % RING_BK != 0) return false;
    const int force_bn = tune(T_RING_BN), force_wgs = tune(T_RING_WGS), force_ns = tune(T_RING_NS), force_rows = tune(T_RING_ROWS);
    int bn = 128;
    if (force_bn == 256 && N >= 256) bn = 256;
    const int tiles_n = cdiv(N, bn);
    int rows = 176, ns = 2;
    if (cdiv(M, 176) * tiles_n < 320) {
        rows = (int)(((long long)M * tiles_n + 199) / 200);
        rows = (rows + 3) & ~3;
        if (rows > 176) rows = 176;
        ns = 3;
    }
    if (force_wgs > 0) {
        const int tm_ = force_wgs / tiles_n > 0 ? force_wgs / tiles_n : 1;
        rows = (cdiv(M, tm_) + 3) & ~3;
    }
    if (force_rows >= 8) rows = (force_rows + 3) & ~3;
    if (rows < 8) rows = 8;
    if (rows > 256) return false;
    p.tile_rows = rows;
    p.tm = cdiv(cdiv(rows, 32), 2);
    p.tn = bn / 128;
    p.tiles_m = cdiv(M, rows);
    p.tiles_n = tiles_n;
    p.wgs = p.tiles_m * tiles_n;
    p.a_rows8 = (rows + 7) & ~7;
    p.stage_bytes = (p.a_rows8 + bn) * RING_STAGE_ROW;
    const int epi_bytes = 8 * 32 * (bn / 4 + 4) * 4;
    if (3 * p.stage_bytes + 1024 > 160 * 1024) ns = 2;
    if (force_ns == 2 || (force_ns == 3 && 3 * p.stage_bytes + 1024 <= 160 * 1024)) ns = force_ns;
    p.ns = ns;
    p.dump_off = p.ns * p.stage_bytes;
    const int ring_bytes = p.dump_off + (p.a_rows8 < 64 * p.tm ? 1024 : 0);
    p.lds_bytes = ring_bytes > epi_bytes ? ring_bytes : epi_bytes;
    p.cost = 0.0;
    return p.lds_bytes <= 160 * 1024;
}

template <int TM, int TN, bool BKC, int NS>
static int ring_launch_one(const RingArgs &ra, int wgs, int lds, hipStream_t s) {
    static int reserved = 0;
    if (lds > reserved) {
        hipError_t e = hipFuncSetAttribute(reinterpret_cast<const void *>(gemm_ring_kernel<TM, TN, BKC, NS>),
                                           hipFuncAttributeMaxDynamicSharedMemorySize, 160 * 1024);
        DETR_REQUIRE(e == hipSuccess, "gemm (ring): cannot reserve %d bytes of LDS: %s", lds, hipGetErrorString(e));
        reserved = 160 * 1024;
    }
    hipLaunchKernelGGL((gemm_ring_kernel<TM, TN, BKC, NS>), dim3((unsigned)wgs), dim3(RING_THREADS), (size_t)lds, s, ra);
    return 0;
}

template <int TM, int TN>
static int ring_launch_tt(const RingArgs &ra, const RingPlan &p, bool bk, hipStream_t s) {
    if (p.ns == 3) return bk ? ring_launch_one<TM, TN, true, 3>(ra, p.wgs, p.lds_bytes, s) : ring_launch_one<TM, TN, false, 3>(ra, p.wgs, p.lds_bytes, s);
    return bk ? ring_launch_one<TM, TN, true, 2>(ra, p.wgs, p.lds_bytes, s) : ring_launch_one<TM, TN, false, 2>(ra, p.wgs, p.lds_bytes, s);
}

int gemm_ring_launch(const GemmArgs &g, bool bk, const RingPlan &p, hipStream_t s) {
    RingArgs ra;
    ra.g = g;
    ra.g.tiles_m = p.tiles_m;
    ra.g.tiles_n = p.tiles_n;
    ra.tile_rows = p.tile_rows;
    ra.a_rows8 = p.a_rows8;
    ra.stage_bytes = p.stage_bytes;
    ra.dump_off = p.dump_off;
    int rc = -1;
    switch (p.tm * 2 + (p.tn - 1)) {
        case 2: rc = ring_launch_tt<1, 1>(ra, p, bk, s); break;
        case 3: rc = ring_launch_tt<1, 2>(ra, p, bk, s); break;
        case 4: rc = ring_launch_tt<2, 1>(ra, p, bk, s); break;
        case 5: rc = ring_launch_tt<2, 2>(ra, p, bk, s); break;
        case 6: rc = ring_launch_tt<3, 1>(ra, p, bk, s); break;
        case 7: rc = ring_launch_tt<3, 2>(ra, p, bk, s); break;
        case 8: rc = ring_launch_tt<4, 1>(ra, p, bk, s); break;
        case 9: rc = ring_launch_tt<4, 2>(ra, p, bk, s); break;
        default: DETR_REQUIRE(false, "gemm (ring): no instantiation for TM=%d TN=%d", p.tm, p.tn);
    }
    return rc;
}

bool gemm_ring_f32_plan(int M, int N, int K, RingPlan &p) {
    if (M < 1 || N < 128 || K < 32 || K % 32 != 0) return false;
    const int bn = 128, tiles_n = cdiv(N, bn);
    const int force_rows = tune(T_RING_ROWS);
    long long best = -1;
    int rows = 64;
    for (int r = 64; r <= 192; r += 32) {
        const long long c = (long long)cdiv((long long)cdiv(M, r) * tiles_n, 256) * (r / 32);
        if (best < 0 || c <= best) { best = c; rows = r; }
    }
    if (force_rows >= 8) rows = (force_rows + 3) & ~3;
    if (rows > 192) return false;
    p.tile_rows = rows;
    p.tm = cdiv(cdiv(rows, 32), 2);
    p.tn = 1;
    p.tiles_m = cdiv(M, rows);
    p.tiles_n = tiles_n;
    p.wgs = p.tiles_m * tiles_n;
    p.a_rows8 = (rows + 7) & ~7;
    p.stage_bytes = (p.a_rows8 + bn) * RING_STAGE_ROW;
    p.ns = 2;
    p.dump_off = p.ns * p.stage_bytes;
    const int epi_bytes = 8 * 32 * (bn / 4 + 4) * 4;
    const int ring_bytes = p.dump_off + (p.a_rows8 < 64 * p.tm ? 1024 : 0);
    p.lds_bytes = ring_bytes > epi_bytes ? ring_bytes : epi_bytes;
    p.cost = (double)best;
    return p.lds_bytes <= 160 * 1024;
}

template <int TM, bool BKC>
static int ring_f32_launch_one(const RingArgs &ra, int wgs, int lds, hipStream_t s) {
    static bool reserved = false;
    if (!reserved) {
        hipError_t e = hipFuncSetAttribute(reinterpret_cast<const void *>(gemm_ring_f32_kernel<TM, 1, BKC, 2>), hipFuncAttributeMaxDynamicSharedMemorySize, 160 * 1024);
        DETR_REQUIRE(e == hipSuccess, "gemm (ring, fp32): cannot reserve %d bytes of LDS: %s", lds, hipGetErrorString(e));
        reserved = true;
    }
    hipLaunchKernelGGL((gemm_ring_f32_kernel<TM, 1, BKC, 2>), dim3((unsigned)wgs), dim3(RING_THREADS), (size_t)lds, s, ra);
    return 0;
}

int gemm_ring_f32_launch(const GemmArgs &g, bool bk, const RingPlan &p, hipStream_t s) {
    RingArgs ra;
    ra.g = g;
    ra.g.tiles_m = p.tiles_m;
    ra.g.tiles_n = p.tiles_n;
    ra.tile_rows = p.tile_rows;
    ra.a_rows8 = p.a_rows8;
    ra.stage_bytes = p.stage_bytes;
    ra.dump_off = p.dump_off;
    DETR_REQUIRE(p.tn == 1 && p.ns == 2 && p.tm >= 1 && p.tm <= 3, "gemm (ring, fp32): no instantiation for TM=%d TN=%d NS=%d", p.tm, p.tn, p.ns);
    if (p.tm == 1) return bk ? ring_f32_launch_one<1, true>(ra, p.wgs, p.lds_bytes, s) : ring_f32_launch_one<1, false>(ra, p.wgs, p.lds_bytes, s);
    if (p.tm == 2) return bk ? ring_f32_launch_one<2, true>(ra, p.wgs, p.lds_bytes, s) : ring_f32_launch_one<2, false>(ra, p.wgs, p.lds_bytes, s);
    return bk ? ring_f32_launch_one<3, true>(ra, p.wgs, p.lds_bytes, s) : ring_f32_launch_one<3, false>(ra, p.wgs, p.lds_bytes, s);
}

template <int TM, int TN, int NS>
static int ring_wgrad_launch_one(const RingArgs &ra, int wgs, hipStream_t s) {
    constexpr int LDS = NS * (64 * TM + 128 * TN) * RING_STAGE_ROW;
    static_assert(LDS <= 160 * 1024, "ring does not fit the LDS");
    static bool reserved = false;
    if (!reserved) {
        hipError_t e = hipFuncSetAttribute(reinterpret_cast<const void *>(gemm_ring_wgrad_kernel<TM, TN, NS>), hipFuncAttributeMaxDynamicSharedMemorySize, 160 * 1024);
        DETR_REQUIRE(e == hipSuccess, "gemm (ring wgrad): cannot reserve LDS: %s", hipGetErrorString(e));
        reserved = true;
    }
    hipLaunchKernelGGL((gemm_ring_wgrad_kernel<TM, TN, NS>), dim3((unsigned)wgs), dim3(RING_THREADS), (size_t)LDS, s, ra);
    return 0;
}

int gemm_ring_wgrad_launch(const GemmArgs &g, int bm, int bn, int split, hipStream_t s) {
    RingArgs ra;
    ra.g = g;
    ra.g.tiles_m = cdiv(g.M, bm);
    ra.g.tiles_n = cdiv(g.N, bn);
    ra.tile_rows = ra.a_rows8 = ra.stage_bytes = ra.dump_off = 0;
    const int wgs = ra.g.tiles_m * ra.g.tiles_n * split;
    if (bm == 128 && bn == 128) return tune(T_RING_NS) == 3 ? ring_wgrad_launch_one<2, 1, 3>(ra, wgs, s) : ring_wgrad_launch_one<2, 1, 4>(ra, wgs, s);
    if (bm == 128 && bn == 256) return ring_wgrad_launch_one<2, 2, 3>(ra, wgs, s);
    if (bm == 256 && bn == 128) return ring_wgrad_launch_one<4, 1, 3>(ra, wgs, s);
    DETR_REQUIRE(false, "gemm (ring wgrad): no instantiation for %d x %d tiles", bm, bn);
    return -1;
}

}

extern "C" int detr_hip_gemm_ring_plan(int32_t M, int32_t N, int32_t K, int32_t *out) {
    detr::RingPlan p;
    if (!detr::gemm_ring_plan(M, N, K, p)) return 0;
    if (out) {
        out[0] = p.tm; out[1] = p.tn; out[2] = p.ns; out[3] = p.tile_rows; out[4] = p.tiles_m; out[5] = p.tiles_n; out[6] = p.wgs; out[7] = p.lds_bytes;
    }
    return 1;
}
```

### detr-tensorflow_amd/detr_tf/_hip.py

```python
import ctypes
import os
from ctypes import POINTER, Structure, byref, c_float, c_int32, c_int64, c_size_t, c_void_p

import torch

_HERE = os.path.dirname(os.path.abspath(__file__))
LIB_PATH = os.environ.get("DETR_HIP_LIB") or os.path.join(os.path.dirname(_HERE), "lib", "libdetr_hip.so")

f32p = c_void_p


class ReduceDesc(Structure):
    _fields_ = [("ws", c_void_p), ("splits", c_int32), ("part_stride", c_int64), ("rows", c_int32), ("cols", c_int32),
                ("C", c_void_p), ("ldc", c_int64), ("alpha", c_float), ("scale", c_void_p),
                ("rs_ws", c_void_p), ("rs_out", c_void_p), ("rs_alpha", c_float),
                ("ts_bm", c_int32), ("ts_bn", c_int32), ("ts_tiles_n", c_int32)]


class GemmDesc(Structure):
    _fields_ = [("M", c_int32), ("N", c_int32), ("K", c_int32),
                ("A", c_void_p), ("lda", c_int64), ("a_kcontig", c_int32),
                ("B", c_void_p), ("ldb", c_int64), ("b_kcontig", c_int32),
                ("C", c_void_p), ("ldc", c_int64),
                ("batch", c_int32), ("batch_inner", c_int32),
# ... 272 lines not shown
class KernelProfiler:

    def __init__(self, prealloc=0, f32=False):
        self.f32 = f32
        self.records = []
        self._pool = []
        for _ in range(prealloc):
            ev = torch.cuda.Event(enable_timing=True)
            ev.record()
            self._pool.append(ev)

    def _event(self):
        return self._pool.pop() if self._pool else torch.cuda.Event(enable_timing=True)

    def begin(self):
        ev = self._event()
        ev.record()
        return ev

    def end(self, family, flops, ev0, sig=None, nbytes=0.0):
        ev1 = self._event()
        ev1.record()
        self.records.append((family, flops, ev0, ev1, sig, nbytes))

    def by_shape(self, top=40):
        torch.cuda.synchronize()
        agg = {}
        for fam, flops, e0, e1, sig, _nb in self.records:
            d = agg.setdefault((fam, sig), [0, 0.0, 0.0])
            d[0] += 1
            d[1] += e0.elapsed_time(e1)
            d[2] += flops
        rows = sorted(agg.items(), key=lambda kv: -kv[1][1])[:top]
        return [{"family": k[0], "shape": k[1], "launches": v[0], "ms": round(v[1], 3),
                 "tflops": round(v[2] / (v[1] * 1e-3) / 1e12, 2) if v[1] > 0 else 0.0} for k, v in rows]

    def summary(self):
        torch.cuda.synchronize()
        out = {}
        for fam, flops, e0, e1, _sig, nb in self.records:
            d = out.setdefault(fam, {"launches": 0, "ms": 0.0, "flops": 0.0, "bytes": 0.0, "mixed_s": 0.0})
            d["launches"] += 1
            d["ms"] += e0.elapsed_time(e1)
            d["flops"] += flops
            d["bytes"] += nb
            d["mixed_s"] += max(flops / (157.3e12 if fam.startswith("gemm_f32") or self.f32 else 2.5e15), nb / 8.0e12)
        return out


PROFILER = None
DEFER = None
DEFER_WS = None
_defer_top = 0
_defer_outs = set()
COMPUTE_BF16 = 0
WORKSPACE = None


WS_GENERATION = 0
_WS_RETIRED = []
_DEVICE = None


def ensure_workspace(device, floats=2 * 1024 * 1024):
    global WORKSPACE, _DEVICE, WS_GENERATION
    _DEVICE = torch.device(device)
    if WORKSPACE is None or WORKSPACE.device != _DEVICE or WORKSPACE.numel() < floats:
        if WORKSPACE is not None:
            _WS_RETIRED.append(WORKSPACE)
            WS_GENERATION += 1
        WORKSPACE = torch.empty(floats, dtype=torch.float32, device=device)
    return WORKSPACE


def need_workspace(nbytes):
    if WORKSPACE is not None and nbytes > WORKSPACE.numel() * 4:
        ensure_workspace(WORKSPACE.device, max((int(nbytes) + 3) // 4, WORKSPACE.numel() * 3 // 2))
    return WORKSPACE


def workspace_bytes_held():
    n = WORKSPACE.numel() * 4 if WORKSPACE is not None else 0
    return n + sum(t.numel() * 4 for t in _DEFER_CHUNKS) + sum(t.numel() * 4 for t in _WS_RETIRED)


_WS_NEED = {}


def _ws_query(fn, key, *args):
    v = _WS_NEED.get(key)
    if v is None:
        v = int(getattr(load(), fn)(*args))
        if v < 0:
            raise RuntimeError(f"{fn} rejected the descriptor: {load().detr_hip_last_error().decode()}")
        _WS_NEED[key] = v
    return v


DEFER_LIMIT = int(os.environ.get("DETR_HIP_DEFER_MB", "512")) * 1024 * 1024
DEFER_CHUNK = 64 * 1024 * 1024
_DEFER_CHUNKS = []
_defer_chunk_i = 0


def ensure_defer_workspace(device):
    global _DEVICE
    _DEVICE = torch.device(device)
    if _DEFER_CHUNKS and _DEFER_CHUNKS[0].device != _DEVICE:
        _DEFER_CHUNKS.clear()
    return _DEFER_CHUNKS


def begin_deferred_reduces(device):
    global DEFER, _defer_top, _defer_outs, _defer_chunk_i, _defer_pending
    ensure_defer_workspace(device)
    del _WS_RETIRED[:]
    DEFER, _defer_top, _defer_outs, _defer_chunk_i, _defer_pending = [], 0, set(), 0, 0


AFTER_FLUSH = None


def flush_reduces(end=False):
    global DEFER, _defer_top, _defer_outs, _defer_chunk_i, _defer_pending
    if DEFER is None:
        return
    if DEFER:
        arr = (ReduceDesc * len(DEFER))(*DEFER)
        _check(load().detr_hip_splitk_reduce_many(arr, len(DEFER), _stream()), "detr_hip_splitk_reduce_many")
        if AFTER_FLUSH is not None:
            AFTER_FLUSH()
    _defer_top, _defer_outs, _defer_chunk_i, _defer_pending = 0, set(), 0, 0
    DEFER = None if end else []


def _defer_push(rds):
    rds = [r for r in rds if r is not None and r.splits > 0]
    outs = [r.C for r in rds] + [r.rs_out for r in rds if r.rs_out]
    if len(set(outs)) != len(outs) or any(o in _defer_outs for o in outs):
        flush_reduces()
        for r in rds:
            arr = (ReduceDesc * 1)(r)
            _check(load().detr_hip_splitk_reduce_many(arr, 1, _stream()), "detr_hip_splitk_reduce_many")
        if AFTER_FLUSH is not None:
            AFTER_FLUSH()
        return
    DEFER.extend(rds)
    _defer_outs.update(outs)
    if _defer_pending >= DEFER_LIMIT:
        flush_reduces()


_defer_pending = 0


def _defer_slab(nbytes):
    global _defer_top, _defer_chunk_i, _defer_pending
    nbytes = (int(nbytes) + 255) & ~255
    while True:
        if _defer_chunk_i >= len(_DEFER_CHUNKS):
            _DEFER_CHUNKS.append(torch.empty(max(DEFER_CHUNK, nbytes) // 4, dtype=torch.float32, device=_DEVICE))
        chunk = _DEFER_CHUNKS[_defer_chunk_i]
        if _defer_top + nbytes <= chunk.numel() * 4:
            break
        _defer_chunk_i += 1
        _defer_top = 0
    ptr_ = chunk.data_ptr() + _defer_top
    _defer_top += nbytes
    _defer_pending += nbytes
    return ptr_, nbytes


def load():
    global _lib
    if _lib is not None:
        return _lib
    if not os.path.exists(LIB_PATH):
        raise RuntimeError(f"{LIB_PATH} not found: run `python -c 'import __graft_entry__ as g; g.build()'` "
                           "(or `make -C detr-tensorflow_amd`) first; there is no CPU/eager fallback")
    lib = ctypes.CDLL(LIB_PATH)
    for name, argtypes in _SIGNATURES.items():
        fn = getattr(lib, name)
        fn.argtypes = argtypes
        fn.restype = c_int32
    for name, argtypes in _SIGNATURES_I64.items():
        fn = getattr(lib, name)
        fn.argtypes = argtypes
        fn.restype = c_int64
    lib.detr_hip_last_error.argtypes = []
    lib.detr_hip_last_error.restype = ctypes.c_char_p
    if lib.detr_hip_abi_version() != ABI_VERSION:
        raise RuntimeError(f"{LIB_PATH}: ABI version {lib.detr_hip_abi_version()}, this binding speaks {ABI_VERSION}: rebuild the library")
    check_struct_layouts(lib)
    _lib = lib
    return lib


def struct_layout_mirror(S):
    return [ctypes.sizeof(S)] + [getattr(S, f[0]).offset for f in S._fields_]


def check_struct_layouts(lib):
    for which, S in sorted({**LAYOUT_STRUCTS, **LAYOUT_STRUCTS_APPENDED}.items()):
        want = struct_layout_mirror(S)
        buf = (c_int32 * 96)()
        n = lib.detr_hip_struct_layout(which, buf, 96)
        got = list(buf[:max(n, 0)])
        if n != len(want) or got != want:
            raise RuntimeError(f"ctypes mirror of struct {which} ({S.__name__}) does not match {LIB_PATH}: library {got}, mirror {want}")


def set_tuning(name, value):
    if value is None:
        os.environ.pop(name, None)
    else:
        os.environ[name] = str(value)
    _check(load().detr_hip_reload_tuning(), "detr_hip_reload_tuning")
    _WS_NEED.clear()


def _stream():
    return torch.cuda.current_stream().cuda_stream


def _check(rc, what):
    if rc != 0:
        raise RuntimeError(f"{what} failed ({rc}): {load().detr_hip_last_error().decode()}")


def ptr(t):
    return None if t is None else t.data_ptr()


def _f32(t, name="tensor"):
    if t.dtype != torch.float32 or not t.is_cuda:
        raise TypeError(f"{name}: expected a CUDA float32 tensor, got {t.dtype} on {t.device}")
    return t


def _gemm_desc(M, N, K, A, lda, a_kcontig, B, ldb, b_kcontig, C, ldc, *, alpha=1.0, scale=None, bias=None,
               residual=None, ldr=0, mask=None, ldmask=0, act=0, split_k=1, batch=1, batch_inner=1,
               sA=(0, 0), sB=(0, 0), sC=(0, 0), a_off=0, b_off=0, c_off=0, workspace=None, dropout_p=0.0, dropout_seed=0,
               dropout_step=None, compute=None, rowsum_a=None, rowsum_alpha=1.0, ws_slice=None, maskbits_out=None, ln=None):
    d = GemmDesc()
    d.M, d.N, d.K = M, N, K
    if ln is not None:
        d.ln_gamma, d.ln_beta, d.ln_y = ln["gamma"].data_ptr(), ln["beta"].data_ptr(), ln["y"].data_ptr()
        d.ln_mean, d.ln_rstd, d.ln_eps = ln["mean"].data_ptr(), ln["rstd"].data_ptr(), float(ln["eps"])
        if ln.get("y2") is not None:
            d.ln_add, d.ln_add_rows, d.ln_y2 = ln["add"].data_ptr(), ln["add"].shape[0], ln["y2"].data_ptr()
        d.ln_y16 = ptr(ln.get("y16"))
    d.A, d.lda, d.a_kcontig = A.data_ptr() + A.element_size() * a_off, lda, int(a_kcontig)
    is16 = lambda t: 1 if (t is not None and t.dtype == torch.bfloat16) else 0
    d.a_dtype, d.c_dtype, d.r_dtype, d.m_dtype = is16(A), is16(C), is16(residual), is16(mask)
    if mask is not None and mask.dtype == torch.uint8:
        d.m_dtype = 2
    if maskbits_out is not None:
        d.maskbits_out, d.ld_maskbits_out = maskbits_out.data_ptr(), maskbits_out.stride(0)
    d.B, d.ldb, d.b_kcontig = B.data_ptr() + B.element_size() * b_off, ldb, int(b_kcontig)
    d.b_dtype = 1 if B.dtype == torch.bfloat16 else 0
    d.C, d.ldc = C.data_ptr() + C.element_size() * c_off, ldc
    d.batch, d.batch_inner = batch, batch_inner
    d.sA0, d.sA1 = sA
    d.sB0, d.sB1 = sB
    d.sC0, d.sC1 = sC
    d.alpha = alpha
    d.scale, d.bias = ptr(scale), ptr(bias)
    d.residual, d.ldr = ptr(residual), ldr
    d.mask, d.ldmask = ptr(mask), ldmask
    d.act, d.split_k = act, split_k
    d.dropout_p, d.dropout_seed = dropout_p, dropout_seed & 0xFFFFFFFF
    d.dropout_step = ptr(dropout_step)
    d.compute = COMPUTE_BF16 if compute is None else int(compute)
    d.rowsum_a, d.rowsum_alpha = ptr(rowsum_a), rowsum_alpha
    ws_need = 0
    if split_k > 1 and batch == 1 and workspace is None and (WORKSPACE is not None or DEFER is not None):
        ws_need = (_ws_query("detr_hip_workspace_bytes_gemm",
                             ("gemm", M, N, K, int(a_kcontig), int(b_kcontig), split_k, d.compute, d.a_dtype, d.b_dtype, ldc % 4,
                              (d.C or 0) % 16, rowsum_a is not None, scale is not None and (d.scale or 0) % 16), byref(d)) + 255) & ~255
    if workspace is None and WORKSPACE is not None and split_k > 1 and batch == 1 and DEFER is None:
        need_workspace(ws_need * (ws_slice[1] if ws_slice else 1))
    ws = workspace if workspace is not None else WORKSPACE
    if ws is None:
        d.workspace, d.workspace_bytes = None, 0
    elif ws_slice is None:
        d.workspace, d.workspace_bytes = ws.data_ptr(), ws.numel() * 4
    else:
        idx, cnt = ws_slice
        share = (ws.numel() * 4 // cnt) & ~255
        d.workspace, d.workspace_bytes = ws.data_ptr() + idx * share, share
    rd = None
    if DEFER is not None and split_k > 1 and batch == 1 and workspace is None:
        slab = _defer_slab(ws_need)
        if slab is not None:
            rd = ReduceDesc()
            d.workspace, d.workspace_bytes = slab
            d.defer_out = ctypes.pointer(rd)
    fam = "gemm_bf16c_kernel" if d.compute == 1 else "gemm_f32_kernel"
    if PROFILER is not None and d.compute == 1 and load().detr_hip_gemm_family(byref(d)) == 1:
        fam = "gemm_stream_bf16_kernel"
    sig = (f"M{M} N{N} K{K} b{batch} ak{int(a_kcontig)} bk{int(b_kcontig)} a16{d.a_dtype} b16{d.b_dtype} sk{split_k}"
           f"{' res' if residual is not None else ''}{' mask' if mask is not None else ''}")
    nbytes = float(batch) * (A.element_size() * M * K + B.element_size() * K * N + C.element_size() * M * N
                             + (residual.element_size() * M * N if residual is not None else 0)
                             + ((M * N // 8 if mask.dtype == torch.uint8 else mask.element_size() * M * N) if mask is not None else 0)
                             + (M * N // 8 if maskbits_out is not None else 0))
    return d, (fam, 2.0 * M * N * K * batch, sig, nbytes, rd)


def gemm(*args, **kw):
    d, (fam, flops, sig, nbytes, rd) = _gemm_desc(*args, **kw)
    ev0 = PROFILER.begin() if PROFILER is not None else None
    _check(load().detr_hip_gemm_f32(byref(d), _stream()), "detr_hip_gemm_f32")
    if rd is not None:
        _defer_push([rd])
    if ev0 is not None:
        PROFILER.end(fam, flops, ev0, sig, nbytes)


def gemm_group(calls):
    n = len(calls)
    arr = (GemmDesc * n)()
    infos = []
    for i, (a, kw) in enumerate(calls):
        d, info = _gemm_desc(*a, ws_slice=(i, n), **kw)
        arr[i] = d
        infos.append(info)
    ev0 = PROFILER.begin() if PROFILER is not None else None
    _check(load().detr_hip_gemm_group_f32(arr, n, _stream()), "detr_hip_gemm_group_f32")
    if DEFER is not None:
        _defer_push([info[4] for info in infos])
    if ev0 is not None:
        PROFILER.end(infos[0][0], sum(i[1] for i in infos), ev0, f"group{n}: " + infos[0][2], sum(i[3] for i in infos))


SPLIT_TARGET_128 = int(os.environ.get("DETR_HIP_SPLIT_TARGET", "256"))
SPLIT_TARGET_64 = int(os.environ.get("DETR_HIP_SPLIT_TARGET64", "1024"))
X3_SPLIT_TARGET = int(os.environ.get("DETR_HIP_X3_SPLIT_TARGET", "512"))


def pick_split_k(M, N, K, max_split=1024):
    if COMPUTE_BF16 == 1 and ((N >= 128 and K >= 16384) or (M >= 512 and N >= 512 and K >= 4096) or
                         (K >= 4096 and ((M >= 256 and N >= 2048) or (M >= 2048 and N >= 256)))):
        tiles = -(-M // 128) * -(-N // 128)
        ktiles = -(-K // 32)
        return int(max(1, min(max(1, SPLIT_TARGET_128 // tiles), max_split, ktiles // 8 if ktiles >= 16 else 1)))
    if COMPUTE_BF16 == 2 and X3_SPLIT_TARGET > 0 and N >= 128 and K >= 256 and M >= 128:
        t128 = -(-M // 128) * -(-N // 128)
        ktiles = -(-K // 32)
        cap = ktiles // 8 if ktiles >= 64 else max(1, ktiles // 4)
        s128 = int(max(1, min(X3_SPLIT_TARGET // t128, max_split, cap)))
        if t128 * s128 >= 192:
            return s128
    tiles = -(-M // 64) * -(-N // 64)
    want = max(1, SPLIT_TARGET_64 // max(tiles, 1))
    ktiles = -(-K // (32 if COMPUTE_BF16 == 1 else 16))
    cap = ktiles // 8 if ktiles >= 64 else ktiles // 4
    return int(max(1, min(want, max_split, cap)))


def linear_fwd_call(x2d, w_out_in, bias, out2d, *, alpha=1.0, residual=None, act=0, dropout_p=0.0, dropout_seed=0,
                    dropout_step=None, ln=None):
    M, K = x2d.shape
    N = w_out_in.shape[0]
    return ((M, N, K, x2d, x2d.stride(0), 1, w_out_in, w_out_in.stride(0), 1, out2d, out2d.stride(0)),
            dict(alpha=alpha, bias=bias, residual=residual, ldr=(residual.stride(0) if residual is not None else 0), act=act,
                 dropout_p=dropout_p, dropout_seed=dropout_seed, dropout_step=dropout_step, **({"ln": ln} if ln is not None else {})))


def linear_dgrad_call(dy2d, w_out_in, dx2d, *, alpha=1.0, residual=None, mask=None):
    M, N = dy2d.shape
    K = w_out_in.shape[1]
    return ((M, K, N, dy2d, dy2d.stride(0), 1, w_out_in, w_out_in.stride(0), 0, dx2d, dx2d.stride(0)),
            dict(alpha=alpha, residual=residual, ldr=(residual.stride(0) if residual is not None else 0),
                 mask=mask, ldmask=(mask.stride(0) if mask is not None else 0)))


def linear_wgrad_call(dy2d, x2d, dw_out_in, *, alpha=1.0, bias_grad=None):
    M, N = dy2d.shape
    K = x2d.shape[1]
    sk = pick_split_k(N, K, M)
    args = (N, K, M, dy2d, dy2d.stride(0), 0, x2d, x2d.stride(0), 0, dw_out_in, dw_out_in.stride(0))
    if sk == 1:
        return args, dict(alpha=alpha, residual=dw_out_in, ldr=dw_out_in.stride(0), rowsum_a=bias_grad, rowsum_alpha=alpha)
    return args, dict(alpha=alpha, split_k=sk, rowsum_a=bias_grad, rowsum_alpha=alpha)


def linear_fwd(*a, **kw):
    args, kwargs = linear_fwd_call(*a, **kw)
    gemm(*args, **kwargs)


def linear_dgrad(*a, **kw):
    args, kwargs = linear_dgrad_call(*a, **kw)
    gemm(*args, **kwargs)


def linear_wgrad(*a, **kw):
    args, kwargs = linear_wgrad_call(*a, **kw)
    gemm(*args, **kwargs)


def conv1x1_bwd_fused_scratch_floats(M):
    return int(load().detr_hip_conv1x1_bwd_fused_workspace_floats(int(M)))


def conv1x1_bwd_fused(dy, a, w, da, dw, scratch, *, scale=None, use_mask=True, alpha=1.0):
    M = dy.shape[0]
    for t, shape, dt in ((dy, (M, 256), torch.bfloat16), (a, (M, 64), torch.bfloat16), (w, (64, 256), torch.bfloat16), (da, (M, 64), torch.bfloat16),
                         (dw, (64, 256), torch.float32)):
        if tuple(t.shape) != shape or t.dtype != dt or t.stride(1) != 1:
            raise ValueError(f"conv1x1_bwd_fused: operand of shape {tuple(t.shape)} / {t.dtype} / strides {t.stride()}, expected {shape} {dt}, unit column stride")
    if scratch.dtype != torch.float32 or (scale is not None and (scale.dtype != torch.float32 or scale.numel() != 256)):
        raise ValueError("conv1x1_bwd_fused: scratch / scale must be fp32 (scale: 256 entries)")
    ev0 = PROFILER.begin() if PROFILER is not None else None
    _check(load().detr_hip_conv1x1_bwd_fused_bf16(dy.data_ptr(), dy.stride(0), a.data_ptr(), a.stride(0), w.data_ptr(), w.stride(0), da.data_ptr(),
                                                  da.stride(0), 1 if use_mask else 0, dw.data_ptr(), dw.stride(0), ptr(scale), c_float(alpha), M,
                                                  a.shape[1], dy.shape[1], scratch.data_ptr(), scratch.numel(), _stream()),
           "detr_hip_conv1x1_bwd_fused_bf16")
    if ev0 is not None:
        PROFILER.end("conv1x1_bwd_fused", 4.0 * M * a.shape[1] * dy.shape[1], ev0, f"M{M} {a.shape[1]}->{dy.shape[1]}",
                     float(2 * M * (dy.shape[1] + 2 * a.shape[1])))


def conv3x3(mode, x, w, y, N, Hi, Wi, Ci, Ho, Wo, Co, stride, *, pad=1, alpha=1.0, scale=None, bias=None,
            residual=None, mask=None, act=0, split=0, compute=None, maskbits_out=None, dilation=1):
    if dilation not in (1, 2):
        raise ValueError(f"conv3x3: dilation {dilation} unsupported (1 or 2)")
    dil = dilation == 2
    d = Conv3x3DDesc() if dil else Conv3x3Desc()
    if dil:
        d.dilation = 2
    fn, ws_fn = ("detr_hip_conv3x3_dilated", "detr_hip_workspace_bytes_conv3x3_dilated") if dil else \
        ("detr_hip_conv3x3_f32", "detr_hip_workspace_bytes_conv3x3")
    d.N, d.Hi, d.Wi, d.Ci, d.Ho, d.Wo, d.Co, d.stride, d.pad = N, Hi, Wi, Ci, Ho, Wo, Co, stride, pad
    d.x, d.w, d.y = x.data_ptr(), w.data_ptr(), y.data_ptr()
    is16 = lambda t: 1 if (t is not None and t.dtype == torch.bfloat16) else 0
    d.w_dtype, d.x_dtype, d.y_dtype, d.r_dtype, d.m_dtype = is16(w), is16(x), is16(y), is16(residual), is16(mask)
    if mask is not None and mask.dtype == torch.uint8:
        d.m_dtype = 2
    d.maskbits_out = ptr(maskbits_out)
    d.alpha = alpha
    d.scale, d.bias, d.residual, d.mask = ptr(scale), ptr(bias), ptr(residual), ptr(mask)
    d.act, d.split = act, split
    d.compute = COMPUTE_BF16 if compute is None else int(compute)
    if mode == 2 and WORKSPACE is not None:
        need_workspace(_ws_query(ws_fn, ("convd" if dil else "conv", N, Hi, Wi, Ci, Ho, Wo, Co, stride, pad, split, d.compute, d.x_dtype),
                                 byref(d), mode))
    d.workspace, d.workspace_bytes = (WORKSPACE.data_ptr(), WORKSPACE.numel() * 4) if WORKSPACE is not None else (None, 0)
    ev0 = PROFILER.begin() if PROFILER is not None else None
    _check(getattr(load(), fn)(byref(d), mode, _stream()), fn)
    if ev0 is not None:
        rows = N * (Hi * Wi if mode == 1 else Ho * Wo)
        PROFILER.end(("conv3x3_fwd", "conv3x3_dgrad", "conv3x3_wgrad")[mode], 2.0 * (N * Ho * Wo) * 9 * Ci * Co, ev0,
                     f"N{N} {Hi}x{Wi}x{Ci}->{Ho}x{Wo}x{Co} s{stride}" + (" d2" if dil else ""),
                     float(x.element_size() * (N * Hi * Wi * Ci if mode != 1 else N * Ho * Wo * Co)
                           + (w.element_size() * 9 * Ci * Co if mode != 2 else w.element_size() * N * Ho * Wo * Co)
                           + y.element_size() * (N * Ho * Wo * Co if mode == 0 else (N * Hi * Wi * Ci if mode == 1 else 9 * Ci * Co))
                           + ((rows * (Ci if mode == 1 else Co) // 8 if mask.dtype == torch.uint8 else mask.element_size() * rows * (Ci if mode == 1 else Co))
                              if mask is not None else 0) + (rows * Co // 8 if maskbits_out is not None else 0)
                           + (residual.element_size() * rows * (Ci if mode == 1 else Co) if residual is not None else 0)))


def stem_conv(mode, img, w, y, N, H, W, Ho, Wo, *, alpha=1.0, scale=None, bias=None, act=0, split=0, compute=None):
    d = StemDesc()
    d.N, d.H, d.W, d.Ho, d.Wo = N, H, W, Ho, Wo
    d.img, d.w, d.y = img.data_ptr(), w.data_ptr(), y.data_ptr()
    d.alpha = alpha
    d.scale, d.bias = ptr(scale), ptr(bias)
    d.act, d.split = act, split
    d.w_dtype = 1 if (mode == 2 and w.dtype == torch.bfloat16) else 0
    d.y_dtype = 1 if (mode == 0 and y.dtype == torch.bfloat16) else 0
    d.compute = COMPUTE_BF16 if compute is None else int(compute)
    if mode == 2 and WORKSPACE is not None:
        need_workspace(_ws_query("detr_hip_workspace_bytes_stem", ("stem", N, H, W, Ho, Wo, split, d.compute, d.w_dtype), byref(d), mode))
    d.workspace, d.workspace_bytes = (WORKSPACE.data_ptr(), WORKSPACE.numel() * 4) if WORKSPACE is not None else (None, 0)
    ev0 = PROFILER.begin() if PROFILER is not None else None
    _check(load().detr_hip_stem_conv7x7_f32(byref(d), mode, _stream()), "detr_hip_stem_conv7x7_f32")
    if ev0 is not None:
        M = N * Ho * Wo
        PROFILER.end("stem_conv7x7", 2.0 * M * 64 * 147, ev0, f"stem7x7 mode{mode} M{M}",
                     float(4 * N * H * W * 3 + (y if mode == 0 else w).element_size() * M * 64 + 4 * 147 * 64))


def call(name, *args):
    _check(getattr(load(), name)(*args, _stream()), name)


def zero_(t):
    call("detr_hip_memset_zero", t.data_ptr(), t.numel() * t.element_size())
    return t


def attention_dropmask_words(B, H, T, S):
    return int(load().detr_hip_attention_dropmask_words(B, H, T, S))

# ... 191 lines not shown
```

### detr-tensorflow_amd/detr_tf/engine.py

```python
import math
import os
from ctypes import byref, c_float

import numpy as np
import torch

from . import _hip as hip
from .params import ParamStore, RESNET50_BLOCKS, block_names, bn_conv_pairs, stem_names

D = 256
HEADS = 8
HD = 32
FF = 2048
BN_EPS = 1e-5
KERAS_BN_EPS = 1.001e-5
LN_EPS = 1e-5
DEFER_REDUCE = os.environ.get("DETR_HIP_DEFER_REDUCE", "1") != "0"
WGRAD_STREAM = os.environ.get("DETR_HIP_WGRAD_STREAM", "1") != "0"
BWD_FUSED = os.environ.get("DETR_HIP_BWD_FUSED", "1") != "0"
DROPMASK_AHEAD = int(os.environ.get("DETR_HIP_DROPMASK_AHEAD", "2") or 0)
QK_ALPHA = float(HD) ** -0.5 * 1.4426950408889634


def mix32(x):
    x &= 0xFFFFFFFF
    x ^= x >> 16
    x = (x * 0x7FEB352D) & 0xFFFFFFFF
    x ^= x >> 15
    x = (x * 0x846CA68B) & 0xFFFFFFFF
    x ^= x >> 16
    return x


def step_seed(base_seed, step_no, rank=0):
    return mix32(mix32((base_seed + 0x9E3779B9 * step_no) & 0xFFFFFFFF) ^ ((rank * 0x85EBCA6B) & 0xFFFFFFFF))


def position_embedding_sine_host(H, W, num_pos_features=128, temperature=10000.0, eps=1e-6):
    y = (np.arange(1, H + 1, dtype=np.float32) / np.float32(H + eps) * np.float32(2 * math.pi)).astype(np.float32)
    x = (np.arange(1, W + 1, dtype=np.float32) / np.float32(W + eps) * np.float32(2 * math.pi)).astype(np.float32)
    k = np.arange(num_pos_features, dtype=np.float32)
    dim_t = np.power(np.float32(temperature), (2 * np.floor(k / 2) / np.float32(num_pos_features)).astype(np.float32)).astype(np.float32)
    py = (y[:, None] / dim_t[None, :]).astype(np.float32)
    px = (x[:, None] / dim_t[None, :]).astype(np.float32)
    ey = np.empty_like(py)
    ex = np.empty_like(px)
    ey[:, 0::2], ey[:, 1::2] = np.sin(py[:, 0::2]), np.cos(py[:, 1::2])
    ex[:, 0::2], ex[:, 1::2] = np.sin(px[:, 0::2]), np.cos(px[:, 1::2])
    pos = np.concatenate([np.broadcast_to(ey[:, None, :], (H, W, num_pos_features)),
                          np.broadcast_to(ex[None, :, :], (H, W, num_pos_features))], axis=2)
    return np.ascontiguousarray(pos.reshape(H * W, 2 * num_pos_features), dtype=np.float32)


def position_embedding_sine_table(n_max, num_pos_features=128, temperature=10000.0, eps=1e-6):
    k = np.arange(num_pos_features, dtype=np.float32)
    dim_t = np.power(np.float32(temperature), (2 * np.floor(k / 2) / np.float32(num_pos_features)).astype(np.float32)).astype(np.float32)
    tab = np.zeros((n_max + 1, n_max + 1, num_pos_features), np.float32)
    c = np.arange(0, n_max + 1, dtype=np.float32)
    for n in range(n_max + 1):
        y = (c / np.float32(n + eps) * np.float32(2 * math.pi)).astype(np.float32)
        py = (y[:, None] / dim_t[None, :]).astype(np.float32)
        tab[n, :, 0::2], tab[n, :, 1::2] = np.sin(py[:, 0::2]), np.cos(py[:, 1::2])
    return tab


def downsample_mask_nearest(mask, Hf, Wf):
    mask = np.asarray(mask)
    H, W = mask.shape[1:]
    sy = np.minimum((np.arange(Hf) * H) // Hf, H - 1)
    sx = np.minimum((np.arange(Wf) * W) // Wf, W - 1)
    return mask[:, sy][:, :, sx]


def dilation_flags(replace_stride_with_dilation):
    if replace_stride_with_dilation is None:
        return (False, False, False)
    flags = tuple(bool(f) for f in replace_stride_with_dilation)
    if len(flags) != 3:
        raise ValueError(f"replace_stride_with_dilation: expected 3 flags (layer2, layer3, layer4), got {len(flags)}")
    return flags


def feature_size(H, W, replace_stride_with_dilation=None):
    for halves in (True, True) + tuple(not f for f in dilation_flags(replace_stride_with_dilation)):
        if halves:
            H, W = (H - 1) // 2 + 1, (W - 1) // 2 + 1
    return H, W


def backbone_stride(replace_stride_with_dilation=None):
    return 4 * 2 ** sum(1 for f in dilation_flags(replace_stride_with_dilation) if not f)


class DetrEngine:
    def __init__(self, device="cuda:0", blocks=RESNET50_BLOCKS, num_enc=6, num_dec=6, num_queries=100,
                 num_classes=92, nb_class=None, seed=0, tf_backbone=False, replace_stride_with_dilation=(False, False, False)):
        self.dilate = dilation_flags(replace_stride_with_dilation)
        if tf_backbone and any(self.dilate):
            raise ValueError("replace_stride_with_dilation needs the reference backbone: tf.keras.applications.ResNet50 "
                             "(tf_backbone=True) has no such option")
        hip.load()
        self.device = torch.device(device)
        hip.ensure_workspace(self.device)
        if DEFER_REDUCE:
            hip.ensure_defer_workspace(self.device)
        self.blocks = tuple(blocks)
        self.num_enc, self.num_dec, self.Q = num_enc, num_dec, num_queries
        self.nb_class = nb_class
        self.C = num_classes if nb_class is None else nb_class
        self.tf_backbone = bool(tf_backbone)
        self.bn_eps = KERAS_BN_EPS if self.tf_backbone else BN_EPS
        self.P = ParamStore(self.device, blocks, num_enc, num_dec, num_queries, num_classes, nb_class, seed, tf_backbone=tf_backbone)
        self._stem = stem_names(self.tf_backbone)
        self._pairs = bn_conv_pairs(self.blocks, self.tf_backbone)
        self._bufs = {}
        self._buf_gen = 0
        self._pos_cache = {}
        self._pos_tables = {}
        self.key_valid = None
        self._attn_sites = ()
        self.attn_maps = {}
        self._shape = None
        self.bn_scale, self.bn_shift = {}, {}
        self._weights_version, self._built = 0, {}
        self.P.on_change = self._params_changed
        self.fold_bn()
        self.compute = 0
        self.f32_split = False
        self.dropout_p = 0.1
        self.dropout_seed = 0x5EED
        self.dp_rank = 0
        self._step_no = 0
        self._drop = (0.0, 0)
        self._step_seed = 0
        self._seed_dev = torch.zeros(8, dtype=torch.int32, device=self.device)
        self._cross = {}
        self._graph_replay = False
        self.phase_events = None

    @property
    def gemm_mode(self):
        return 1 if self.compute == 1 else (2 if self.f32_split else 0)

    def bump_weights_version(self):
        self._weights_version += 1

    def _stale(self, key):
        if self._built.get(key) == self._weights_version:
            return False
        self._built[key] = self._weights_version
        return True

    def advance_dropout_step(self):
        self._step_no += 1
        self._step_seed = step_seed(self.dropout_seed, self._step_no, self.dp_rank)
        hip.call("detr_hip_set_u32x8", self._seed_dev.data_ptr(), self._step_seed, step_seed(self.dropout_seed, self._step_no + 1, self.dp_rank),
                 0, 0, 0, 0, 0, 0)
        self._drop = (float(self.dropout_p), self._step_seed)
        return self._step_seed

    def phase(self, name):
        if self.phase_events is not None:
            ev = torch.cuda.Event(enable_timing=True)
            ev.record()
            self.phase_events.append((name, ev))

    def buf(self, name, shape, dtype=torch.float32):
        key = name
        t = self._bufs.get(key)
        shape = tuple(int(s) for s in shape)
        if t is None or tuple(t.shape) != shape or t.dtype != dtype:
            if t is not None:
                self._buf_gen += 1
            t = torch.empty(shape, dtype=dtype, device=self.device)
            self._bufs[key] = t
        return t

    @property
    def buf_generation(self):
        return self._buf_gen + hip.WS_GENERATION

    def buffer_bytes(self):
        return sum(t.numel() * t.element_size() for t in self._bufs.values())

    def fold_bn(self):
        for p, c in self.P.bn.items():
            raw = self.P.bn_raw[p]
            sc = self.buf(f"bnscale:{p}", (c,))
            sh = self.buf(f"bnshift:{p}", (c,))
            hip.call("detr_hip_bn_fold_f32", raw[0].data_ptr(), raw[1].data_ptr(), raw[2].data_ptr(), raw[3].data_ptr(),
                     sc.data_ptr(), sh.data_ptr(), c, c_float(self.bn_eps))
            self.bn_scale[p] = sc
            self.bn_shift[p] = self.buf(f"bnshift_eff:{p}", (c,)) if self.tf_backbone else sh
        self.bump_weights_version()
        self._fold_table = None
        self._shift_table = None

    def _refresh_bias_shift(self):
        if self._shift_table is None:
            rows = []
            for bn_name, conv_name in self._pairs:
                c = self.P.bn[bn_name]
                rows.append([self.P.views[f"{conv_name}/bias"].data_ptr(), self.bn_scale[bn_name].data_ptr(),
                             self._bufs[f"bnshift:{bn_name}"].data_ptr(), self.bn_shift[bn_name].data_ptr(), c])
            self._shift_table = torch.tensor(rows, dtype=torch.int64).to(self.device)
        hip.call("detr_hip_fma_vec_group", self._shift_table.data_ptr(), self._shift_table.shape[0])

    def _params_changed(self):
        self.fold_bn()

    def load_params(self, params):
        return self.P.load_dict(params)

    def _w(self, name):
        if hip.COMPUTE_BF16 == 1 and self.P.views16 is not None:
            return self.P.views16[name]
        return self.P.views[name]

    def _refresh_shadow(self):
        flat16 = self.P.shadow16()
        hip.call("detr_hip_cvt_bf16", self.P.flat.data_ptr(), flat16.data_ptr(), self.P.flat.numel())
        self._refold_group()

    def _refold_group(self):
        if getattr(self, "_fold_table", None) is None:
            rows = []
            for bn_name, conv in self._pairs[1:]:
                conv_name = f"{conv}/kernel"
                w = self.P.views[conv_name]
                co = w.shape[-1]
                ws16 = self.buf(f"ws16:{conv_name}", w.shape, torch.bfloat16)
                rows.append([w.data_ptr(), self.bn_scale[bn_name].data_ptr(), ws16.data_ptr(), w.numel() // 4, co // 4])
            self._fold_table = torch.tensor(rows, dtype=torch.int64).to(self.device)
            self._fold_keep = [self.bn_scale, self._bufs]
        hip.call("detr_hip_scale_cols_bf16_group", self._fold_table.data_ptr(), self._fold_table.shape[0])

    def _scaled_kernel(self, conv_name, bn_name):
        w = self.P.views[conv_name]
        co = w.shape[-1]
        if self.compute == 1 and conv_name != f"{self._stem['conv']}/kernel":
            return self.buf(f"ws16:{conv_name}", w.shape, torch.bfloat16)
        ws = self.buf(f"ws:{conv_name}", w.shape)
        if self._stale(f"ws:{conv_name}"):
            hip.call("detr_hip_scale_cols_f32", w.data_ptr(), self.bn_scale[bn_name].data_ptr(), ws.data_ptr(),
                     w.numel() // co, co)
        return ws

    def _conv1x1_fwd(self, x, M, cin, cout, conv_name, bn_name, out, residual=None, act=1, maskbits_out=None):
        ws = self._scaled_kernel(conv_name, bn_name)
        shift = self.bn_shift[bn_name]
        ldr = cout if residual is not None else 0
        hip.gemm(M, cout, cin, x, cin, 1, ws, cout, 0, out, cout, bias=shift, residual=residual, ldr=ldr, act=act,
                 maskbits_out=maskbits_out)

    @staticmethod
    def _wgrad(M_out, N_out, K_red, A, lda, Bm, ldb, C, ldc, scale=None, alpha=1.0):
        sk = hip.pick_split_k(M_out, N_out, K_red)
        if sk > 1:
            hip.gemm(M_out, N_out, K_red, A, lda, 0, Bm, ldb, 0, C, ldc, alpha=alpha, scale=scale, split_k=sk)
        else:
            hip.gemm(M_out, N_out, K_red, A, lda, 0, Bm, ldb, 0, C, ldc, alpha=alpha, scale=scale, residual=C, ldr=ldc)

    def _colsum(self, x2d, out, alpha=1.0):
        rows, cols = x2d.shape
        n = int(hip.load().detr_hip_colsum_det_scratch_floats(rows, cols))
        scratch = self.buf(f"colsum:{rows}x{cols}", (n,))
        hip.call("detr_hip_colsum_det_f32", x2d.data_ptr(), out.data_ptr(), rows, cols, x2d.stride(0), c_float(alpha),
                 scratch.data_ptr(), n)

    def _ln_fwd(self, x, pfx, y, tag, add=None, y2=None, y16=None):
        rows = x.shape[0]
        mean = self.buf(f"{tag}:mean", (rows,))
        rstd = self.buf(f"{tag}:rstd", (rows,))
        hip.layernorm_fwd(x, self.P.views[f"{pfx}/gamma"], self.P.views[f"{pfx}/beta"], y, mean, rstd, LN_EPS, add=add, y2=y2,
                          y16=y16)

    def _ln_spec(self, rows, pfx, y, tag, add=None, y2=None, y16=None, ffn=False):
        if self.compute != 1 or ffn:
            return None
        return dict(gamma=self.P.views[f"{pfx}/gamma"], beta=self.P.views[f"{pfx}/beta"], y=y, mean=self.buf(f"{tag}:mean", (rows,)),
                    rstd=self.buf(f"{tag}:rstd", (rows,)), eps=LN_EPS, add=add, y2=y2, y16=y16)

    def _side_begin(self, on):
        self._side_on = bool(on)
        hip.AFTER_FLUSH = self._side_sync if self._side_on else None
        if self._side_on:
            self._side_main = torch.cuda.current_stream()
            if getattr(self, "_wg_stream", None) is None:
                self._wg_stream = torch.cuda.Stream(device=self._side_main.device)

    def _side_sync(self):
        if getattr(self, "_side_on", False):
            self._side_main.wait_stream(self._wg_stream)
            self._wg_stream.wait_stream(self._side_main)

    def _side(self, fn):
        if not getattr(self, "_side_on", False):
            fn()
            return
        ev = torch.cuda.Event()
        ev.record(self._side_main)
        self._wg_stream.wait_event(ev)
        with torch.cuda.stream(self._wg_stream):
            fn()

    def _side_join(self):
        if getattr(self, "_side_on", False):
            self._side_main.wait_stream(self._wg_stream)

    def _sx(self, site):
        return f":{site}" if getattr(self, "_side_on", False) else ""

    def _ln_bwd(self, dy, x, pfx, dx, tag, dx_add=None, drop_site=None, want16=False, dy_add=None):
        dp, _ = self._drop
        dx_drop = dx_drop16 = None
        if drop_site is not None:
            if want16:
                dx_drop16 = self.buf(f"scratch:drop16:{dx.shape[0]}{self._sx(tag)}", dx.shape, torch.bfloat16)
            elif dp > 0.0:
                dx_drop = self.buf(f"scratch:drop:{dx.shape[0]}{self._sx(tag)}", dx.shape)
        hip.layernorm_bwd(dy, x, self.P.views[f"{pfx}/gamma"], self._bufs[f"{tag}:mean"], self._bufs[f"{tag}:rstd"], dx,
                          self.P.gviews[f"{pfx}/gamma"], self.P.gviews[f"{pfx}/beta"], dx_add=dx_add, dx_drop=dx_drop,
                          dropout_p=dp, dropout_site=(drop_site or 0), dropout_step=self._seed_dev, dx_drop16=dx_drop16,
                          dy_add=dy_add)
        if dx_drop16 is not None:
            return dx_drop16
        return dx if dx_drop is None else dx_drop

    def _add_bcast(self, x, p, out):
        hip.call("detr_hip_add_bcast_f32", x.data_ptr(), p.data_ptr(), out.data_ptr(), x.numel(), p.numel())

    @property
    def attn16(self):
        return self.compute == 1

    def _dropmask(self, site, B, T, S, which=None):
        which = getattr(self, "_mask_set", 0) if which is None else which
        return self.buf(f"dropmask:{which}:{site}", (hip.attention_dropmask_words(B, HEADS, T, S),), torch.int32)

    def _mask_sites(self, L):
        Q = self.Q
        sites = [(16 * i, L, L) for i in range(self.num_enc)]
        for i in range(self.num_dec):
            ds = 16 * (32 + i)
            sites += [(ds, Q, Q), (ds + 2, Q, L)]
        return sites

    def _launch_dropmasks(self, B, L, which, seed_slot):
        dp, _ = self._drop
        main = torch.cuda.current_stream()
        if getattr(self, "_mask_stream", None) is None:
            self._mask_stream = torch.cuda.Stream(device=main.device)
        bufs = [(self._dropmask(site, B, T, S, which), T, S, site) for site, T, S in self._mask_sites(L)]
        self._mask_stream.wait_stream(main)
        with torch.cuda.stream(self._mask_stream):
            hip.attention_dropmask_many(bufs, B, HEADS, dropout_p=dp, dropout_step=self._seed_dev[seed_slot:])

    def _gen_dropmasks(self, B, L):
        dp, _ = self._drop
        if not (self.attn16 and dp > 0.0):
            return
        self._mask_set = self._step_no & 1
        tags = self.__dict__.setdefault("_mask_tags", {})
        key = (self._step_seed, B, L, self.Q, dp)
        if not (tags.get(self._mask_set) == key and not self._graph_replay):
            self._launch_dropmasks(B, L, self._mask_set, 0)
            tags[self._mask_set] = None if self._graph_replay else key
        self._mask_pending = True

    def _pregen_dropmasks(self, B, L, now=False):
        dp, _ = self._drop
        if not (self.attn16 and dp > 0.0) or self._graph_replay or not DROPMASK_AHEAD:
            return
        if DROPMASK_AHEAD == 2 and not now:
            self._pregen_args = (B, L)
            return
        nxt = (self._step_no + 1) & 1
        self._launch_dropmasks(B, L, nxt, 1)
        self._mask_tags[nxt] = (step_seed(self.dropout_seed, self._step_no + 1, self.dp_rank), B, L, self.Q, dp)

    def pregen_dropmasks_at_matcher(self):
        args, self._pregen_args = getattr(self, "_pregen_args", None), None
        if args is not None:
            self._pregen_dropmasks(*args, now=True)

    def _join_dropmasks(self):
        if getattr(self, "_mask_pending", False):
            torch.cuda.current_stream().wait_stream(self._mask_stream)
            self._mask_pending = False

    def _self_attn_fwd(self, tag, pfx, qk_in, v_in, B, T, out, site, ln=None, key_valid=None):
        W, bias = self._w(f"{pfx}/in_proj_kernel"), self.P.views[f"{pfx}/in_proj_bias"]
        dp, _ = self._drop
        lse = self.buf(f"{tag}:lse", (B * HEADS, T))
        if self.attn16:
            QKV = self.buf(f"{tag}:QKV16", (B * T, 3 * D), torch.bfloat16)
            hip.gemm_group([hip.linear_fwd_call(qk_in, W[0:D], bias[0:D], QKV[:, 0:D], alpha=QK_ALPHA),
                            hip.linear_fwd_call(qk_in, W[D:2 * D], bias[D:2 * D], QKV[:, D:2 * D]),
                            hip.linear_fwd_call(v_in, W[2 * D:], bias[2 * D:], QKV[:, 2 * D:])])
            O = self.buf(f"{tag}:O16", (B * T, D), torch.bfloat16)
            self._join_dropmasks()
            hip.attention(QKV[:, 0:D], QKV[:, D:2 * D], QKV[:, 2 * D:], O, lse, B, HEADS, T, T, scale=float(HD) ** -0.5, dropout_p=dp,
                          dropout_site=site, dropout_step=self._seed_dev, dropmask=self._dropmask(site, B, T, T) if dp > 0.0 else None,
                          key_valid=key_valid)
        else:
            QKV = self.buf(f"{tag}:QKV", (B * T, 3 * D))
            hip.gemm_group([hip.linear_fwd_call(qk_in, W[0:2 * D], bias[0:2 * D], QKV[:, 0:2 * D]),
                            hip.linear_fwd_call(v_in, W[2 * D:], bias[2 * D:], QKV[:, 2 * D:])])
            O = self.buf(f"{tag}:O", (B * T, D))
            hip.attention(QKV[:, 0:D], QKV[:, D:2 * D], QKV[:, 2 * D:], O, lse, B, HEADS, T, T, scale=float(HD) ** -0.5,
                          dropout_p=dp, dropout_site=site, dropout_step=self._seed_dev, key_valid=key_valid)
        if pfx in self._attn_sites:
            self._attn_map(pfx, QKV[:, 0:D], QKV[:, D:2 * D], lse, B, T, T, key_valid)
        hip.linear_fwd(O, self._w(f"{pfx}/out_proj_kernel"), self.P.views[f"{pfx}/out_proj_bias"], out, residual=v_in,
# ... 427 lines not shown
        feat, Hf, Wf, L = self._feat_meta
        nd = self.num_dec
        memory = self._bufs[f"enc{self.num_enc - 1}:x2"] if self.num_enc > 0 else self._bufs["enc:src0"]
        mem_pos = self._bufs["dec:mem_pos"] if self.num_enc > 0 else self._bufs["enc0:qk"]
        a16 = self.attn16
        adt16 = torch.bfloat16 if a16 else torch.float32
        KV = self._bufs["dec:KV16" if a16 else "dec:KV"]
        ct = self._cross_tables()
        qpos, g_qpos = V["query_embed/kernel"], G["query_embed/kernel"]
        BQ = B * Q
        dp, _ = self._drop
        dKV = self.buf(f"scratch:dKV:{int(a16)}", (B * L, 2 * nd * D), adt16)
        acc_qpos = self.buf("scratch:acc_qpos", (BQ, D))
        hip.zero_(acc_qpos)
        d_next = None
        d_t3n = self.buf("scratch:d_t3n", (nd, BQ, D))
        self._ln_bwd(d_hs3.view(nd * BQ, D), self._bufs["dec:t3all"].view(nd * BQ, D), "transformer/decoder/norm", d_t3n.view(nd * BQ, D), "dec:lnf")
        for i in reversed(range(nd)):
            pfx, tag = f"transformer/decoder/layer_{i}", f"dec{i}"
            cp = f"{pfx}/multihead_attn"
            t1, t2, t3 = self._bufs[f"{tag}:t1"], self._bufs[f"{tag}:t2"], self._bufs[f"{tag}:t3"]
            a1, a2, f = self._bufs[f"{tag}:a1"], self._bufs[f"{tag}:a2"], self._bufs[f"{tag}:f"]
            qin, q2 = self._bufs[f"{tag}:qin"], self._bufs[f"{tag}:q2"]
            tgt = self._bufs[f"dec{i - 1}:t3"] if i > 0 else self._bufs["dec:tgt0"]
            ds = 16 * (32 + i)
            d_f = self.buf(f"scratch:d_f{self._sx(tag)}", (BQ, D))
            d_y = self._ln_bwd(d_t3n[i], f, f"{pfx}/norm3", d_f, f"{tag}:ln3", drop_site=ds + 5, want16=self.ffn16, dy_add=d_next)
            d_t2 = self.buf("scratch:d_t2", (BQ, D))
            self._ffn_bwd(tag, pfx, d_y, d_f, t2, d_t2, x16=self._bufs.get(f"{tag}:t2h") if self.ffn16 else None)
            d_a2 = self.buf(f"scratch:d_a2{self._sx(tag)}", (BQ, D))
            d_out = self._ln_bwd(d_t2, a2, f"{pfx}/norm2", d_a2, f"{tag}:ln2", drop_site=ds + 3)
            Wc = self._w(f"{cp}/in_proj_kernel")
            Qc, Oc = self._bufs[f"{tag}:ca:Q16" if a16 else f"{tag}:ca:Q"], self._bufs[f"{tag}:ca:O16" if a16 else f"{tag}:ca:O"]
            dO = self.buf(f"scratch:dO:{BQ}:{int(a16)}", (BQ, D), adt16)
            hip.linear_dgrad(d_out, self._w(f"{cp}/out_proj_kernel"), dO)
            dQc = self.buf(f"scratch:dQc:{int(a16)}{self._sx(tag)}", (BQ, D), adt16)
            delta = self.buf(f"scratch:delta:{BQ}", (2 * B * HEADS, Q))
            hip.attention(Qc, KV[:, i * D:(i + 1) * D], KV[:, (nd + i) * D:(nd + i + 1) * D], Oc, self._bufs[f"{tag}:ca:lse"],
                          B, HEADS, Q, L, scale=float(HD) ** -0.5, dropout_p=dp, dropout_site=ds + 2, dropout_step=self._seed_dev,
                          d_o=dO, dq=dQc, dk=dKV[:, i * D:(i + 1) * D], dv=dKV[:, (nd + i) * D:(nd + i + 1) * D], delta=delta,
                          dropmask=self._dropmask(ds + 2, B, Q, L) if (a16 and dp > 0.0) else None, key_valid=self.key_valid)
            self._side(lambda d_out=d_out, Oc=Oc, dQc=dQc, q2=q2, cp=cp: hip.gemm_group([
                hip.linear_wgrad_call(d_out, Oc, G[f"{cp}/out_proj_kernel"], bias_grad=G[f"{cp}/out_proj_bias"]),
                hip.linear_wgrad_call(dQc, q2, G[f"{cp}/in_proj_kernel"][0:D], bias_grad=G[f"{cp}/in_proj_bias"][0:D])]))
            d_t1 = self.buf("scratch:d_t1", (BQ, D))
            hip.gemm_group([hip.linear_dgrad_call(dQc, Wc[0:D], acc_qpos, residual=acc_qpos),
                            hip.linear_dgrad_call(dQc, Wc[0:D], d_t1, residual=d_a2)])
            d_a1 = self.buf(f"scratch:d_a1{self._sx(tag)}", (BQ, D))
            d_out = self._ln_bwd(d_t1, a1, f"{pfx}/norm1", d_a1, f"{tag}:ln1", drop_site=ds + 1)
            d_tgt = self.buf(f"scratch:d_tgt{i & 1}", (BQ, D)) if i > 0 else None
            self._self_attn_bwd(f"{tag}:sa", f"{pfx}/self_attn", d_out, d_a1, qin, tgt, B, Q, d_tgt, site=ds, acc_qk=acc_qpos)
            d_next = d_tgt
        self._colsum(acc_qpos.view(B, Q * D), g_qpos.view(Q * D))
        hip.zero_(ct["gW"])
        hip.zero_(ct["gb"])
        hip.gemm_group([hip.linear_wgrad_call(dKV[:, 0:nd * D], mem_pos, ct["gW"][0:nd * D], bias_grad=ct["gb"][0:nd * D]),
                        hip.linear_wgrad_call(dKV[:, nd * D:], memory, ct["gW"][nd * D:], bias_grad=ct["gb"][nd * D:])])
        self._side_join()
        hip.flush_reduces()
        hip.multi_copy(ct["scatter"])
        d_mem = self.buf("scratch:d_mem", (B * L, D))
        hip.linear_dgrad(dKV, ct["Wkv"], d_mem)
        self.phase("bwd encoder")
        d_x = d_mem
        for i in reversed(range(self.num_enc)):
            pfx, tag = f"transformer/encoder/layer_{i}", f"enc{i}"
            x_in = self._bufs[f"enc{i - 1}:x2"] if i > 0 else self._bufs["enc:src0"]
            qk, a, x1, f = (self._bufs[f"{tag}:{n}"] for n in ("qk", "a", "x1", "f"))
            d_f = self.buf(f"scratch:e_d_f{self._sx(tag)}", (B * L, D))
            d_y = self._ln_bwd(d_x, f, f"{pfx}/norm2", d_f, f"{tag}:ln2", drop_site=16 * i + 3, want16=self.ffn16)
            d_x1 = self.buf("scratch:e_d_x1", (B * L, D))
            self._ffn_bwd(tag, pfx, d_y, d_f, x1, d_x1, x16=self._bufs.get(f"{tag}:x1h") if self.ffn16 else None)
            d_a = self.buf(f"scratch:e_d_a{self._sx(tag)}", (B * L, D))
            d_out = self._ln_bwd(d_x1, a, f"{pfx}/norm1", d_a, f"{tag}:ln1", drop_site=16 * i + 1)
            d_xn = self.buf(f"scratch:e_d_x{i & 1}", (B * L, D))
            self._self_attn_bwd(f"{tag}:sa", f"{pfx}/self_attn", d_out, d_a, qk, x_in, B, L, d_xn, site=16 * i, key_valid=self.key_valid)
            d_x = d_xn
        if on_bucket:
            on_bucket(0)
        self.phase("bwd backbone")
        self._wgrad(2048, D, B * L, feat, 2048, d_x, D, G["input_proj/kernel"], D)
        self._colsum(d_x, G["input_proj/bias"])
        if not backbone:
            if on_bucket:
                for i in (1, 2, 3):
                    on_bucket(i)
            return
        adt = self._adt
        g = self.buf("scratch:g_feat", feat.shape, adt)
        hip.gemm(B * L, 2048, D, d_x, D, 1, self._w("input_proj/kernel"), D, 1, g, 2048, mask=feat, ldmask=2048)
        n_blocks = len(self._block_meta)
        tfb = self.tf_backbone
        f32c = 2 if adt == torch.bfloat16 else 1

        def bias_grad(conv, bn, dz, rows, cols):
            if tfb:
                hip.call("detr_hip_colsum_scaled", dz.data_ptr(), 1 if dz.dtype == torch.bfloat16 else 0, rows, cols, cols,
                         self.bn_scale[bn].data_ptr(), G[f"{conv}/bias"].data_ptr())

        ws_on = self._side_on
        main, wside = (self._side_main, self._wg_stream) if ws_on else (None, None)
        side_done = {}
        on_side = self._side

        def side_mark(bi):
            if ws_on:
                ev = torch.cuda.Event()
                ev.record(wside)
                side_done[bi] = ev

        def side_wait(bi):
            ev = side_done.pop(bi, None)
            if ev is not None:
                main.wait_event(ev)

        for bi in reversed(range(n_blocks)):
            m = self._block_meta[bi]
            side_wait(bi + 2)
            par = f":{bi & 1}" if ws_on else ""
            p, n, x, xs, x1, y1, y2 = m["p"], m["n"], m["x"], m["xs"], m["x1"], m["y1"], m["y2"]
            h, w, ho, wo, cin, d1, d2, stride = m["h"], m["w"], m["ho"], m["wo"], m["cin"], m["d1"], m["d2"], m["stride"]
            h1, w1, M1, s2 = m["h1"], m["w1"], m["M1"], m["s2"]
            M_in, M_out = B * h * w, B * ho * wo
            wk = "ws16" if self.compute == 1 else "ws"
            ws1 = self._bufs[f"{wk}:{n['conv1']}/kernel"]
            ws2 = self._bufs[f"{wk}:{n['conv2']}/kernel"]
            ws3 = self._bufs[f"{wk}:{n['conv3']}/kernel"]
            strided = m["first"] and stride == 2
            wsd = self._bufs[f"{wk}:{n['down']}/kernel"] if m["first"] else None
            idg, idg_ready = g, None
            fused_ok = BWD_FUSED and self.compute == 1 and adt == torch.bfloat16 and d2 == 256 and g.is_cuda
            fuse3, fuse_down = fused_ok and d1 == 64, False
            if m["first"] and not (tfb and strided):
                idg = self.buf(f"scratch:idg:{cin}:{h}", (B, h, w, cin), adt)

                fuse_down = fused_ok and not strided and cin == 64

                def dg_down(g=g, idg=idg):
                    if strided:
                        dxs = self.buf(f"scratch:dxs:{cin}:{ho}", (B, ho, wo, cin), adt)
                        hip.gemm(M_out, cin, d2, g, d2, 1, wsd, d2, 1, dxs, cin)
                        hip.call("detr_hip_subsample2_bwd_f32", dxs.data_ptr(), idg.data_ptr(), B, h, w, cin // f32c, ho, wo)
                    elif fuse_down:
                        hip.conv1x1_bwd_fused(g.view(M_out, d2), xs.view(M_out, cin), wsd.view(cin, d2), idg.view(M_out, cin), G[f"{n['down']}/kernel"].view(cin, d2),
                                              self.buf(f"bwdfused:slabs:down:{M_out}", (hip.conv1x1_bwd_fused_scratch_floats(M_out),)),
                                              scale=self.bn_scale[n["bnd"]], use_mask=False)
                    else:
                        hip.gemm(M_out, cin, d2, g, d2, 1, wsd, d2, 1, idg, cin)
                on_side(dg_down)
                if ws_on:
                    idg_ready = torch.cuda.Event()
                    idg_ready.record(wside)

            def wg3(g=g, fuse3=fuse3, fuse_down=fuse_down):
                if not fuse3:
                    self._wgrad(d1, d2, M_out, y2, d1, g, d2, G[f"{n['conv3']}/kernel"], d2, scale=self.bn_scale[n["bn3"]])
                bias_grad(n["conv3"], n["bn3"], g, M_out, d2)
                if m["first"]:
                    if not fuse_down:
                        self._wgrad(cin, d2, M_out, xs, cin, g, d2, G[f"{n['down']}/kernel"], d2, scale=self.bn_scale[n["bnd"]])
                    bias_grad(n["down"], n["bnd"], g, M_out, d2)
            on_side(wg3)
            dz2 = self.buf(f"scratch:dz2:{d1}:{ho}{par}", (B, ho, wo, d1), adt)
            if fuse3:
                hip.conv1x1_bwd_fused(g.view(M_out, d2), y2.view(M_out, d1), ws3.view(d1, d2), dz2.view(M_out, d1), G[f"{n['conv3']}/kernel"].view(d1, d2),
                                      self.buf(f"bwdfused:slabs:{M_out}", (hip.conv1x1_bwd_fused_scratch_floats(M_out),)),
                                      scale=self.bn_scale[n["bn3"]], use_mask=True)
            else:
                hip.gemm(M_out, d1, d2, g, d2, 1, ws3, d2, 1, dz2, d1, mask=y2, ldmask=d1)

            def wg2():
                hip.conv3x3(2, y1, dz2, G[f"{n['conv2']}/kernel"], B, h1, w1, d1, ho, wo, d1, s2, scale=self.bn_scale[n["bn2"]],
                            pad=m["dil"], dilation=m["dil"])
                bias_grad(n["conv2"], n["bn2"], dz2, M_out, d1)
            on_side(wg2)
            dz1 = self.buf(f"scratch:dz1:{d1}:{h1}{par}", (B, h1, w1, d1), adt)
            hip.conv3x3(1, dz2, ws2, dz1, B, h1, w1, d1, ho, wo, d1, s2, mask=y1, pad=m["dil"], dilation=m["dil"])

            def wg1():
                self._wgrad(cin, d1, M1, x1, cin, dz1, d1, G[f"{n['conv1']}/kernel"], d1, scale=self.bn_scale[n["bn1"]])
                bias_grad(n["conv1"], n["bn1"], dz1, M1, d1)
            on_side(wg1)
            side_mark(bi)
            side_wait(bi + 1)
            is_first_block = bi == 0
            gx = self.buf(f"scratch:gx:{cin}:{h}:{bi & 1}", (B, h, w, cin), adt)
            mask = None if is_first_block else x
            xbits = None if is_first_block else self._block_meta[bi - 1].get("out_bits")
            if tfb and strided:
                dxs = self.buf(f"scratch:dxs:{cin}:{ho}", (B, ho, wo, cin), adt)
                hip.gemm(M_out, cin, d2, g, d2, 1, wsd, d2, 1, dxs, cin)
                hip.gemm(M_out, cin, d1, dz1, d1, 1, ws1, d1, 1, dxs, cin, residual=dxs, ldr=cin,
                         mask=(None if is_first_block else xs), ldmask=(0 if is_first_block else cin))
                hip.call("detr_hip_subsample2_bwd_f32", dxs.data_ptr(), gx.data_ptr(), B, h, w, cin // f32c, ho, wo)
            else:
                if idg_ready is not None:
                    main.wait_event(idg_ready)
                if xbits is not None:
                    hip.gemm(M_in, cin, d1, dz1, d1, 1, ws1, d1, 1, gx, cin, residual=idg, ldr=cin, mask=xbits, ldmask=xbits.stride(0))
                else:
                    hip.gemm(M_in, cin, d1, dz1, d1, 1, ws1, d1, 1, gx, cin, residual=idg, ldr=cin, mask=mask,
                             ldmask=(cin if mask is not None else 0))
            g = gx
            if on_bucket:
                if p == block_names(3, 0, tfb)["tag"]:
                    on_bucket(1)
                elif p == block_names(2, 0, tfb)["tag"]:
                    on_bucket(2)
        self._side_join()
        stem, pool, amax = (self._bufs[f"stem:{n}"] for n in ("out", "pool", "amax"))
        H1, W1 = stem.shape[1], stem.shape[2]
        H2, W2 = pool.shape[1], pool.shape[2]
        d_stem = self.buf("scratch:d_stem", stem.shape, adt)
        hip.call("detr_hip_maxpool3x3s2_bwd_bf16" if adt == torch.bfloat16 else "detr_hip_maxpool3x3s2_bwd_f32", g.data_ptr(),
                 amax.data_ptr(), stem.data_ptr(), d_stem.data_ptr(), B, H1, W1, 64, H2, W2)
        M1 = B * H1 * W1
        hip.stem_conv(2, self.images, d_stem, G[f"{self._stem['conv']}/kernel"], B, self._shape[1], self._shape[2], H1, W1,
                      scale=self.bn_scale[self._stem["bn"]], split=max(1, min(512, M1 // 4096)))
        if self.tf_backbone:
            hip.call("detr_hip_colsum_scaled", d_stem.data_ptr(), 1 if d_stem.dtype == torch.bfloat16 else 0, B * H1 * W1, 64, 64,
                     self.bn_scale[self._stem["bn"]].data_ptr(), G[f"{self._stem['conv']}/bias"].data_ptr())
        if on_bucket:
            on_bucket(3)
```

Measured before the change: 532.3.

## Group bottleneck wgrad GEMMs into one launch and add streaming split-K reduce

Adds a streaming split-K reduce path that assigns one float4 unit per thread, sums the splits with unrolled multi-accumulator loads and uses DPP quad broadcasts to transpose slab-tiled output. It is selected for large reductions or through a new tune knob. In the ResNet bottleneck backward, the conv3, downsample and conv1 weight-gradient GEMMs are now issued as a single grouped launch with jointly balanced split-K, and a grouped ring-wgrad kernel is added. The aim is fewer launches, better load balance across the wgrad GEMMs and lower reduce overhead, at the cost of delaying the conv3 wgrad until conv1's inputs are ready.

```diff
diff --git a/detr-tensorflow_amd/csrc/common.h b/detr-tensorflow_amd/csrc/common.h
--- a/detr-tensorflow_amd/csrc/common.h
+++ b/detr-tensorflow_amd/csrc/common.h
@@ -78,6 +78,7 @@
     T_X3_WG_ROUNDS,
     T_X3_CONV,
     T_SPLIT3_ALL,
+    T_REDUCE_FORM,
     T_COUNT
 };
 int tune(TuneKey k);
diff --git a/detr-tensorflow_amd/csrc/common.hip b/detr-tensorflow_amd/csrc/common.hip
--- a/detr-tensorflow_amd/csrc/common.hip
+++ b/detr-tensorflow_amd/csrc/common.hip
@@ -41,6 +41,7 @@
     "DETR_HIP_X3_WG_ROUNDS",
     "DETR_HIP_X3_CONV",
     "DETR_HIP_SPLIT3_ALL",
+    "DETR_HIP_REDUCE_FORM",
 };
 static int g_tune[T_COUNT];
 static void load_tuning() {
diff --git a/detr-tensorflow_amd/csrc/gemm_f32.hip b/detr-tensorflow_amd/csrc/gemm_f32.hip
--- a/detr-tensorflow_amd/csrc/gemm_f32.hip
+++ b/detr-tensorflow_amd/csrc/gemm_f32.hip
@@ -8,6 +8,7 @@
 
 namespace detr {
 
+constexpr int REDUCE_STREAM_THREADS = 256;
 struct ReduceOne {
     const float *ws; int splits; long long part_stride; int rows, cols; float *C; long long ldc;
     float alpha; const float *scale; int vec; const float *rs_ws; float *rs_out; float rs_alpha; int nblocks;
@@ -16,21 +17,97 @@
 struct ReduceGroupArgs { ReduceOne r[GEMM_MAX_GROUP]; };
 
 template <int G>
-__device__ __forceinline__ void splitk_reduce_body(const float *__restrict__ ws, int splits, long long part_stride,
-                                                   int rows, int cols, float *__restrict__ C, long long ldc,
-                                                   float alpha, const float *__restrict__ scale, int vec,
-                                                   const float *__restrict__ rs_ws, float *__restrict__ rs_out,
-                                                   float rs_alpha, const int bid, const int nbid,
-                                                   const int ts_bm = 0, const int ts_bn = 0, const int ts_tn = 1) {
+__device__ __forceinline__ float4 reduce_unit_sum(const float *__restrict__ p, const int splits, const long long part_stride) {
+    constexpr int U = 16;
+    static_assert(U % G == 0, "a block of loads covers whole rounds of the accumulators");
+    float4 acc[G];
+#pragma unroll
+    for (int q = 0; q < G; ++q) acc[q] = make_float4(0.f, 0.f, 0.f, 0.f);
+    int k0 = 0;
+    for (; k0 + U <= splits; k0 += U) {
+        float4 v[U];
+#pragma unroll
+        for (int j = 0; j < U; ++j) v[j] = *reinterpret_cast<const float4 *>(p + (long long)(k0 + j) * part_stride);
+#pragma unroll
+        for (int j = 0; j < U; ++j) { float4 &a = acc[j % G]; a.x += v[j].x; a.y += v[j].y; a.z += v[j].z; a.w += v[j].w; }
+    }
+    const int rem = splits - k0;
+    if (rem > 0) {
+        float4 v[U - 1];
+#pragma unroll
+        for (int j = 0; j < U - 1; ++j) {
+            v[j] = make_float4(0.f, 0.f, 0.f, 0.f);
+            if (j < rem) v[j] = *reinterpret_cast<const float4 *>(p + (long long)(k0 + j) * part_stride);
+        }
+#pragma unroll
+        for (int j = 0; j < U - 1; ++j)
+            if (j < rem) { float4 &a = acc[j % G]; a.x += v[j].x; a.y += v[j].y; a.z += v[j].z; a.w += v[j].w; }
+    }
+    float4 s = acc[0];
+#pragma unroll
+    for (int q = 1; q < G; ++q) { s.x += acc[q].x; s.y += acc[q].y; s.z += acc[q].z; s.w += acc[q].w; }
+    return s;
+}
+
+template <int J>
+__device__ __forceinline__ float quad_bcast(float v) {
+    return __int_as_float(__builtin_amdgcn_mov_dpp(__float_as_int(v), J * 0x55, 0xf, 0xf, true));
+}
+
+template <int G>
+__device__ __forceinline__ void splitk_reduce_stream_body(const float *__restrict__ ws, int splits, long long part_stride, int rows, int cols,
+                                                          float *__restrict__ C, long long ldc, float alpha, const float *__restrict__ scale,
+                                                          const int bid, const int nbid, const int ts_bm, const int ts_bn, const int ts_tn) {
+    const int bt = (int)blockDim.x;
+    if (ts_bm > 0) {
+        const int upt = (ts_bm * ts_bn) >> 2;
+        const long long total = part_stride >> 2;
+        for (long long i = (long long)bid * bt + threadIdx.x; i < total; i += (long long)nbid * bt) {
+            const float4 s = reduce_unit_sum<G>(ws + i * 4, splits, part_stride);
+            const int t = (int)(i & 3);
+            const float4 q0 = make_float4(quad_bcast<0>(s.x), quad_bcast<0>(s.y), quad_bcast<0>(s.z), quad_bcast<0>(s.w));
+            const float4 q1 = make_float4(quad_bcast<1>(s.x), quad_bcast<1>(s.y), quad_bcast<1>(s.z), quad_bcast<1>(s.w));
+            const float4 q2 = make_float4(quad_bcast<2>(s.x), quad_bcast<2>(s.y), quad_bcast<2>(s.z), quad_bcast<2>(s.w));
+            const float4 q3 = make_float4(quad_bcast<3>(s.x), quad_bcast<3>(s.y), quad_bcast<3>(s.z), quad_bcast<3>(s.w));
+            auto pick = [t](const float4 &q) { return t == 0 ? q.x : (t == 1 ? q.y : (t == 2 ? q.z : q.w)); };
+            const float4 v = make_float4(pick(q0), pick(q1), pick(q2), pick(q3));
+            const long long iq = i - t;
+            const int tile = (int)(iq / upt), u = (int)(iq - (long long)tile * upt);
+            int row0, col;
+            slab_ts_unit(u, ts_bm, ts_bn, row0, col);
+            const int row = row0 + (tile / ts_tn) * ts_bm + t;
+            col += (tile % ts_tn) * ts_bn;
+            if (row < rows && col < cols) {
+                float4 sc = make_float4(1.f, 1.f, 1.f, 1.f);
+                if (scale) sc = *reinterpret_cast<const float4 *>(scale + col);
+                float4 *dst = reinterpret_cast<float4 *>(C + (long long)row * ldc + col);
+                float4 o = *dst;
+                o.x += alpha * sc.x * v.x; o.y += alpha * sc.y * v.y; o.z += alpha * sc.z * v.z; o.w += alpha * sc.w * v.w;
+                *dst = o;
+            }
+        }
+    } else {
+        const int c4n = cols >> 2;
+        const long long total = (long long)rows * c4n;
+        for (long long i = (long long)bid * bt + threadIdx.x; i < total; i += (long long)nbid * bt) {
+            const int r = (int)(i / c4n), c = (int)(i - (long long)r * c4n) * 4;
+            const float4 s = reduce_unit_sum<G>(ws + (long long)r * cols + c, splits, part_stride);
+            float4 sc = make_float4(1.f, 1.f, 1.f, 1.f);
+            if (scale) sc = *reinterpret_cast<const float4 *>(scale + c);
+            float4 *dst = reinterpret_cast<float4 *>(C + (long long)r * ldc + c);
+            float4 o = *dst;
+            o.x += alpha * sc.x * s.x; o.y += alpha * sc.y * s.y; o.z += alpha * sc.z * s.z; o.w += alpha * sc.w * s.w;
+            *dst = o;
+        }
+    }
+}
+
+template <int G>
+__device__ __forceinline__ void splitk_reduce_lds_body(const float *__restrict__ ws, int splits, long long part_stride, int rows, int cols,
+                                                       float *__restrict__ C, long long ldc, float alpha, const float *__restrict__ scale, int vec,
+                                                       const int bid, const int nbid, const int ts_bm, const int ts_bn, const int ts_tn) {
     constexpr int OUT = 256 / G;
     __shared__ float4 red[G][OUT];
-    if (rs_ws) {
-        for (int m = bid * 256 + threadIdx.x; m < rows; m += nbid * 256) {
-            float t = 0.0f;
-            for (int k = 0; k < splits; ++k) t += rs_ws[(long long)k * rows + m];
-            rs_out[m] += rs_alpha * t;
-        }
-    }
     const int lo = threadIdx.x % OUT, grp = threadIdx.x / OUT;
     if (ts_bm > 0) {
         __shared__ float tr[OUT][5];
@@ -113,57 +190,106 @@
             }
             __syncthreads();
         }
-    } else {
-        const long long total = (long long)rows * cols;
-        for (long long i = bid * (long long)blockDim.x + threadIdx.x; i < total; i += (long long)nbid * blockDim.x) {
-            const int r = (int)(i / cols), c = (int)(i - (long long)r * cols);
-            float s = 0.f;
-            for (int k = 0; k < splits; ++k) s += ws[k * part_stride + i];
-            C[(long long)r * ldc + c] += alpha * (scale ? scale[c] : 1.0f) * s;
-        }
-    }
-}
-
-template <int G>
+    }
+}
+
+template <int G, bool STREAM>
+__device__ __forceinline__ void splitk_reduce_body(const float *__restrict__ ws, int splits, long long part_stride,
+                                                   int rows, int cols, float *__restrict__ C, long long ldc,
+                                                   float alpha, const float *__restrict__ scale, int vec,
+                                                   const float *__restrict__ rs_ws, float *__restrict__ rs_out,
+                                                   float rs_alpha, const int bid, const int nbid,
+                                                   const int ts_bm = 0, const int ts_bn = 0, const int ts_tn = 1) {
+    if (rs_ws) {
+        const int bt = (int)blockDim.x;
+        for (int m = bid * bt + threadIdx.x; m < rows; m += nbid * bt) {
+            float t = 0.0f;
+            for (int k = 0; k < splits; ++k) t += rs_ws[(long long)k * rows + m];
+            rs_out[m] += rs_alpha * t;
+        }
+    }
+    if constexpr (STREAM) {
+        if (ts_bm > 0 || vec) {
+            splitk_reduce_stream_body<G>(ws, splits, part_stride, rows, cols, C, ldc, alpha, scale, bid, nbid, ts_bm, ts_bn, ts_tn);
+            return;
+        }
+    }
+    if constexpr (!STREAM) {
+        if (ts_bm > 0 || vec) {
+            splitk_reduce_lds_body<G>(ws, splits, part_stride, rows, cols, C, ldc, alpha, scale, vec, bid, nbid, ts_bm, ts_bn, ts_tn);
+            return;
+        }
+    }
+    const long long total = (long long)rows * cols;
+    for (long long i = bid * (long long)blockDim.x + threadIdx.x; i < total; i += (long long)nbid * blockDim.x) {
+        const int r = (int)(i / cols), c = (int)(i - (long long)r * cols);
+        float s = 0.f;
+        for (int k = 0; k < splits; ++k) s += ws[k * part_stride + i];
+        C[(long long)r * ldc + c] += alpha * (scale ? scale[c] : 1.0f) * s;
+    }
+}
+
+template <int G, bool STREAM>
 __global__ __launch_bounds__(256) void splitk_reduce_kernel(const float *__restrict__ ws, int splits, long long part_stride,
                                                             int rows, int cols, float *__restrict__ C, long long ldc,
                                                             float alpha, const float *__restrict__ scale, int vec,
                                                             const float *__restrict__ rs_ws, float *__restrict__ rs_out,
                                                             float rs_alpha, int ts_bm, int ts_bn, int ts_tn) {
-    splitk_reduce_body<G>(ws, splits, part_stride, rows, cols, C, ldc, alpha, scale, vec, rs_ws, rs_out, rs_alpha, blockIdx.x,
-                          gridDim.x, ts_bm, ts_bn, ts_tn);
-}
-template <int G>
+    splitk_reduce_body<G, STREAM>(ws, splits, part_stride, rows, cols, C, ldc, alpha, scale, vec, rs_ws, rs_out, rs_alpha, blockIdx.x,
+                                  gridDim.x, ts_bm, ts_bn, ts_tn);
+}
+template <int G, bool STREAM>
 __global__ __launch_bounds__(256) void splitk_reduce_group_kernel(ReduceGroupArgs R) {
     const ReduceOne &r = R.r[blockIdx.y];
     if ((int)blockIdx.x >= r.nblocks) return;
-    splitk_reduce_body<G>(r.ws, r.splits, r.part_stride, r.rows, r.cols, r.C, r.ldc, r.alpha, r.scale, r.vec, r.rs_ws, r.rs_out,
-                          r.rs_alpha, blockIdx.x, r.nblocks, r.ts_bm, r.ts_bn, r.ts_tn);
+    splitk_reduce_body<G, STREAM>(r.ws, r.splits, r.part_stride, r.rows, r.cols, r.C, r.ldc, r.alpha, r.scale, r.vec, r.rs_ws, r.rs_out,
+                                  r.rs_alpha, blockIdx.x, r.nblocks, r.ts_bm, r.ts_bn, r.ts_tn);
 }
 
 constexpr int REDUCE_MANY = 16;
 struct ReduceManyArgs { ReduceOne r[REDUCE_MANY]; };
-template <int G>
+template <int G, bool STREAM>
 __global__ __launch_bounds__(256) void splitk_reduce_many_kernel(ReduceManyArgs R) {
     const ReduceOne &r = R.r[blockIdx.y];
     if ((int)blockIdx.x >= r.nblocks) return;
-    splitk_reduce_body<G>(r.ws, r.splits, r.part_stride, r.rows, r.cols, r.C, r.ldc, r.alpha, r.scale, r.vec, r.rs_ws, r.rs_out,
-                          r.rs_alpha, blockIdx.x, r.nblocks, r.ts_bm, r.ts_bn, r.ts_tn);
-}
-
-static void reduce_plan(ReduceOne &r, bool &small) {
+    splitk_reduce_body<G, STREAM>(r.ws, r.splits, r.part_stride, r.rows, r.cols, r.C, r.ldc, r.alpha, r.scale, r.vec, r.rs_ws, r.rs_out,
+                                  r.rs_alpha, blockIdx.x, r.nblocks, r.ts_bm, r.ts_bn, r.ts_tn);
+}
+
+constexpr long long REDUCE_STREAM_MIN_UNITS = 16384;
+static int reduce_form_threads(long long launch_units) {
+    const int f = tune(T_REDUCE_FORM);
+    if (f == 2) return 0;
+    if (f == 64 || f == 128 || f == 256) return f;
+    return launch_units >= REDUCE_STREAM_MIN_UNITS ? REDUCE_STREAM_THREADS : 0;
+}
+
+static long long reduce_plan(ReduceOne &r, bool &small) {
     r.vec = (r.cols % 4 == 0) && (r.ldc % 4 == 0) && (r.part_stride % 4 == 0) && aligned16(r.ws) && aligned16(r.C) &&
             (!r.scale || aligned16(r.scale));
     const bool ts = r.ts_bm > 0;
     const bool vec_like = r.vec || ts;
     const long long total = (long long)r.rows * (vec_like ? r.cols / 4 : r.cols);
     small = vec_like && total <= 65536 && r.splits >= 8;
-    const long long units = ts ? r.part_stride / 4 : total;
-    long long grid = vec_like ? (units + (small ? 15 : 63)) / (small ? 16 : 64) : (units + 255) / 256;
+    r.nblocks = 0;
+    return vec_like ? (ts ? r.part_stride / 4 : total) : 0;
+}
+static void reduce_blocks(ReduceOne &r, bool small, long long units, int st) {
+    const int per_block = units == 0 ? 256 : (st > 0 ? st : (small ? 16 : 64));
+    long long grid = ((units == 0 ? (long long)r.rows * r.cols : units) + per_block - 1) / per_block;
     if (grid > 8192) grid = 8192;
     if (grid < 1) grid = 1;
     r.nblocks = (int)grid;
 }
+
+#define DETR_REDUCE_LAUNCH(KERNEL, st_, small_, grid_, stream_, ...)                                                                \
+    do {                                                                                                                            \
+        const dim3 block_((unsigned)((st_) > 0 ? (st_) : 256));                                                                     \
+        if ((st_) > 0 && (small_)) hipLaunchKernelGGL((KERNEL<16, true>), grid_, block_, 0, stream_, __VA_ARGS__);                  \
+        else if ((st_) > 0) hipLaunchKernelGGL((KERNEL<4, true>), grid_, block_, 0, stream_, __VA_ARGS__);                          \
+        else if (small_) hipLaunchKernelGGL((KERNEL<16, false>), grid_, block_, 0, stream_, __VA_ARGS__);                           \
+        else hipLaunchKernelGGL((KERNEL<4, false>), grid_, block_, 0, stream_, __VA_ARGS__);                                        \
+    } while (0)
 
 void launch_splitk_reduce(const float *ws, int splits, long long part_stride, int rows, int cols, float *C, long long ldc,
                           float alpha, const float *scale, hipStream_t stream, const float *rs_ws, float *rs_out,
@@ -173,13 +299,11 @@
     r.alpha = alpha; r.scale = scale; r.rs_ws = rs_ws; r.rs_out = rs_out; r.rs_alpha = rs_alpha;
     r.ts_bm = ts_bm; r.ts_bn = ts_bn; r.ts_tn = ts_tiles_n > 0 ? ts_tiles_n : 1;
     bool small;
-    reduce_plan(r, small);
-    if (small)
-        hipLaunchKernelGGL(splitk_reduce_kernel<16>, dim3((unsigned)r.nblocks), dim3(256), 0, stream, ws, splits, part_stride, rows, cols,
-                           C, ldc, alpha, scale, r.vec, rs_ws, rs_out, rs_alpha, r.ts_bm, r.ts_bn, r.ts_tn);
-    else
-        hipLaunchKernelGGL(splitk_reduce_kernel<4>, dim3((unsigned)r.nblocks), dim3(256), 0, stream, ws, splits, part_stride, rows, cols,
-                           C, ldc, alpha, scale, r.vec, rs_ws, rs_out, rs_alpha, r.ts_bm, r.ts_bn, r.ts_tn);
+    const long long units = reduce_plan(r, small);
+    const int st = reduce_form_threads(units);
+    reduce_blocks(r, small, units, st);
+    DETR_REDUCE_LAUNCH(splitk_reduce_kernel, st, small, dim3((unsigned)r.nblocks), stream, ws, splits, part_stride, rows, cols, C, ldc, alpha,
+                       scale, r.vec, rs_ws, rs_out, rs_alpha, r.ts_bm, r.ts_bn, r.ts_tn);
 }
 
 template <int BM, int BN, int WGM, int WGN>
@@ -583,6 +707,14 @@
     return gemm_ring_f32_plan(d->M, d->N, d->K, rp);
 }
 
+static bool gemm_ring_wgrad_eligible(const GemmPlan &p) {
+    const GemmArgs &g = p.g;
+    const detr_gemm_desc *d = p.d;
+    return p.bf16c && (p.tile == 1 || p.tile == 6 || p.tile == 7) && g.a16 && g.b16 && !p.ak && !p.bk && p.batch == 1 && p.split > 1 &&
+           g.slab_ts && !g.rowsum && d->M % 8 == 0 && d->N % 8 == 0 && d->lda % 8 == 0 && d->ldb % 8 == 0 && aligned16(d->A) &&
+           aligned16(d->B) && tune(T_GEMM_RING) != 2 && tune(T_GEMM_RING) != 3;
+}
+
 static int gemm_launch(const GemmPlan &p, hipStream_t s) {
     const GemmArgs &g = p.g;
     const detr_gemm_desc *d = p.d;
@@ -610,9 +742,7 @@
             return 0;
         }
     }
-    const bool ring_wgrad = p.bf16c && (p.tile == 1 || p.tile == 6 || p.tile == 7) && g.a16 && g.b16 && !ak && !bk && batch == 1 && p.split > 1 &&
-                            g.slab_ts && !g.rowsum && d->M % 8 == 0 && d->N % 8 == 0 && d->lda % 8 == 0 && d->ldb % 8 == 0 && aligned16(d->A) &&
-                            aligned16(d->B) && tune(T_GEMM_RING) != 2 && tune(T_GEMM_RING) != 3;
+    const bool ring_wgrad = gemm_ring_wgrad_eligible(p);
     DETR_REQUIRE(ring_wgrad || (p.tile != 6 && p.tile != 7), "gemm: the 128 x 256 / 256 x 128 tiles exist for the ring weight gradient only "
                  "(tile-ordered slabs in a workspace of detr_hip_workspace_bytes_gemm bytes are required)");
     if (ring_wgrad) {
@@ -661,11 +791,7 @@
     if (!ring_first && gemm_stream_eligible(p)) return 1;
     if (ring_first) return 2;
     if (gemm_ring_f32_eligible(p, rp)) return 3;
-    const GemmArgs &g = p.g;
-    const bool ring_wgrad = p.bf16c && (p.tile == 1 || p.tile == 6 || p.tile == 7) && g.a16 && g.b16 && !p.ak && !p.bk && p.batch == 1 && p.split > 1 &&
-                            g.slab_ts && !g.rowsum && d->M % 8 == 0 && d->N % 8 == 0 && d->lda % 8 == 0 && d->ldb % 8 == 0 && aligned16(d->A) &&
-                            aligned16(d->B) && tune(T_GEMM_RING) != 2 && tune(T_GEMM_RING) != 3;
-    return ring_wgrad ? 5 : 0;
+    return gemm_ring_wgrad_eligible(p) ? 5 : 0;
 }
 
 extern "C" int detr_hip_gemm_f32(const detr_gemm_desc *d, void *stream) {
@@ -682,6 +808,60 @@
 template <bool AK, bool BKC, bool A16, bool B16>
 static void launch_group_bf16(const GemmGroupArgs &G, dim3 grid, hipStream_t s) {
     hipLaunchKernelGGL((gemm_bf16c_group_kernel<64, 64, 2, 2, AK, BKC, A16, B16>), grid, dim3(GEMM_THREADS), 0, s, G);
+}
+
+static int gemm_group_reduces(const GemmPlan *p, int m, hipStream_t s) {
+    ReduceGroupArgs R;
+    bool smalls[GEMM_MAX_GROUP];
+    long long units[GEMM_MAX_GROUP], launch_units = 0;
+    int nr = 0;
+    bool all_small = true, any_small = false;
+    for (int i = 0; i < m; ++i) {
+        const detr_gemm_desc *d = p[i].d;
+        if (d->defer_out) {
+            detr_reduce_desc *o = d->defer_out;
+            o->splits = 0;
+            if (p[i].partial) {
+                o->ws = d->workspace; o->splits = p[i].split; o->part_stride = p[i].part; o->rows = d->M; o->cols = d->N;
+                o->C = d->C; o->ldc = d->ldc; o->alpha = p[i].final_e.alpha; o->scale = p[i].final_e.scale;
+                o->rs_ws = d->rowsum_a ? d->workspace + (long long)p[i].split * p[i].part : nullptr;
+                o->rs_out = d->rowsum_a; o->rs_alpha = d->rowsum_alpha;
+                o->ts_bm = p[i].ts_bm; o->ts_bn = p[i].ts_bn; o->ts_tiles_n = p[i].ts_tn;
+            }
+            continue;
+        }
+        if (!p[i].partial) continue;
+        ReduceOne &r = R.r[nr];
+        r.ws = d->workspace; r.splits = p[i].split; r.part_stride = p[i].part; r.rows = d->M; r.cols = d->N;
+        r.C = d->C; r.ldc = d->ldc; r.alpha = p[i].final_e.alpha; r.scale = p[i].final_e.scale;
+        r.rs_ws = d->rowsum_a ? d->workspace + (long long)p[i].split * p[i].part : nullptr;
+        r.rs_out = d->rowsum_a; r.rs_alpha = d->rowsum_alpha;
+        r.ts_bm = p[i].ts_bm; r.ts_bn = p[i].ts_bn; r.ts_tn = p[i].ts_tn;
+        units[nr] = reduce_plan(r, smalls[nr]);
+        launch_units += units[nr];
+        all_small = all_small && smalls[nr];
+        any_small = any_small || smalls[nr];
+        ++nr;
+    }
+    if (nr > 0 && (all_small || !any_small)) {
+        const int st = reduce_form_threads(launch_units);
+        unsigned rx = 1;
+        for (int i = 0; i < nr; ++i) {
+            reduce_blocks(R.r[i], smalls[i], units[i], st);
+            rx = (unsigned)R.r[i].nblocks > rx ? (unsigned)R.r[i].nblocks : rx;
+        }
+        for (int i = nr; i < GEMM_MAX_GROUP; ++i) R.r[i] = R.r[0];
+        DETR_REDUCE_LAUNCH(splitk_reduce_group_kernel, st, all_small, dim3(rx, (unsigned)nr), s, R);
+        DETR_LAUNCH_CHECK("gemm group split-k reduce");
+    } else if (nr > 0) {
+        for (int i = 0; i < nr; ++i) {
+            const ReduceOne &r = R.r[i];
+            launch_splitk_reduce(r.ws, r.splits, r.part_stride, r.rows, r.cols, r.C, r.ldc, r.alpha, r.scale, s, r.rs_ws, r.rs_out,
+                                 r.rs_alpha, r.ts_bm, r.ts_bn, r.ts_tn);
+        }
+        DETR_LAUNCH_CHECK("gemm group split-k reduce (sequential)");
+    }
+    return 0;
 }
 
 extern "C" int detr_hip_gemm_group_f32(const detr_gemm_desc *descs, int32_t n, void *stream) {
@@ -701,6 +881,18 @@
                    p[i].g.a16 == p[0].g.a16 && p[i].g.b16 == p[0].g.b16 && (p[i].split == 1 || p[i].partial) &&
                    !gemm_stream_eligible(p[i]);
         if (same) { RingPlan rp; for (int i = 0; i < m && same; ++i) same = !gemm_ring_eligible(p[i], rp) && !gemm_ring_f32_eligible(p[i], rp); }
+        bool ring_group = !same && m > 1 && tune(T_GEMM_GROUP) != 2;
+        for (int i = 0; i < m && ring_group; ++i) ring_group = p[i].tile == 1 && gemm_ring_wgrad_eligible(p[i]);
+        if (ring_group) {
+            GemmArgs ga[GEMM_MAX_GROUP];
+            int splits[GEMM_MAX_GROUP];
+            for (int i = 0; i < m; ++i) { ga[i] = p[i].g; splits[i] = p[i].split; }
+            if (gemm_ring_wgrad_group_launch(ga, splits, m, s)) return -1;
+            DETR_LAUNCH_CHECK("gemm group (ring wgrad)");
+            if (gemm_group_reduces(p, m, s)) return -1;
+            done += m;
+            continue;
+        }
         if (!same) {
             for (int i = 0; i < m; ++i)
                 if (gemm_launch(p[i], s)) return -1;
@@ -737,51 +929,7 @@
         else launch_group_f32<false, false>(G, grid, s, p[0].split3);
 #undef DETR_GROUP_BF16
         DETR_LAUNCH_CHECK("gemm group");
-        ReduceGroupArgs R;
-        int nr = 0;
-        unsigned rx = 1;
-        bool all_small = true, any_small = false;
-        for (int i = 0; i < m; ++i) {
-            const detr_gemm_desc *d = p[i].d;
-            if (d->defer_out) {
-                detr_reduce_desc *o = d->defer_out;
-                o->splits = 0;
-                if (p[i].partial) {
-                    o->ws = d->workspace; o->splits = p[i].split; o->part_stride = p[i].part; o->rows = d->M; o->cols = d->N;
-                    o->C = d->C; o->ldc = d->ldc; o->alpha = p[i].final_e.alpha; o->scale = p[i].final_e.scale;
-                    o->rs_ws = d->rowsum_a ? d->workspace + (long long)p[i].split * p[i].part : nullptr;
-                    o->rs_out = d->rowsum_a; o->rs_alpha = d->rowsum_alpha;
-                    o->ts_bm = p[i].ts_bm; o->ts_bn = p[i].ts_bn; o->ts_tiles_n = p[i].ts_tn;
-                }
-                continue;
-            }
-            if (!p[i].partial) continue;
-            ReduceOne &r = R.r[nr];
-            r.ws = d->workspace; r.splits = p[i].split; r.part_stride = p[i].part; r.rows = d->M; r.cols = d->N;
-            r.C = d->C; r.ldc = d->ldc; r.alpha = p[i].final_e.alpha; r.scale = p[i].final_e.scale;
-            r.rs_ws = d->rowsum_a ? d->workspace + (long long)p[i].split * p[i].part : nullptr;
-            r.rs_out = d->rowsum_a; r.rs_alpha = d->rowsum_alpha;
-            r.ts_bm = p[i].ts_bm; r.ts_bn = p[i].ts_bn; r.ts_tn = p[i].ts_tn;
-            bool small;
-            reduce_plan(r, small);
-            all_small = all_small && small;
-            any_small = any_small || small;
-            rx = (unsigned)r.nblocks > rx ? (unsigned)r.nblocks : rx;
-            ++nr;
-        }
-        if (nr > 0 && (all_small || !any_small)) {
-            for (int i = nr; i < GEMM_MAX_GROUP; ++i) R.r[i] = R.r[0];
-            if (all_small) hipLaunchKernelGGL(splitk_reduce_group_kernel<16>, dim3(rx, (unsigned)nr), dim3(256), 0, s, R);
-            else hipLaunchKernelGGL(splitk_reduce_group_kernel<4>, dim3(rx, (unsigned)nr), dim3(256), 0, s, R);
-            DETR_LAUNCH_CHECK("gemm group split-k reduce");
-        } else if (nr > 0) {
-            for (int i = 0; i < nr; ++i) {
-                const ReduceOne &r = R.r[i];
-                launch_splitk_reduce(r.ws, r.splits, r.part_stride, r.rows, r.cols, r.C, r.ldc, r.alpha, r.scale, s, r.rs_ws, r.rs_out,
-                                     r.rs_alpha, r.ts_bm, r.ts_bn, r.ts_tn);
-            }
-            DETR_LAUNCH_CHECK("gemm group split-k reduce (sequential)");
-        }
+        if (gemm_group_reduces(p, m, s)) return -1;
         done += m;
     }
     return 0;
@@ -793,15 +941,20 @@
     hipStream_t s = (hipStream_t)stream;
     for (int pass = 0; pass < 2; ++pass) {
         ReduceManyArgs R;
+        long long units[REDUCE_MANY], launch_units = 0;
         int cnt = 0;
-        unsigned rx = 1;
         auto flush = [&]() {
             if (cnt == 0) return;
+            const int st = reduce_form_threads(launch_units);
+            unsigned rx = 1;
+            for (int i = 0; i < cnt; ++i) {
+                reduce_blocks(R.r[i], pass == 0, units[i], st);
+                rx = (unsigned)R.r[i].nblocks > rx ? (unsigned)R.r[i].nblocks : rx;
+            }
             for (int i = cnt; i < REDUCE_MANY; ++i) R.r[i] = R.r[0];
-            if (pass == 0) hipLaunchKernelGGL(splitk_reduce_many_kernel<16>, dim3(rx, (unsigned)cnt), dim3(256), 0, s, R);
-            else hipLaunchKernelGGL(splitk_reduce_many_kernel<4>, dim3(rx, (unsigned)cnt), dim3(256), 0, s, R);
+            DETR_REDUCE_LAUNCH(splitk_reduce_many_kernel, st, pass == 0, dim3(rx, (unsigned)cnt), s, R);
             cnt = 0;
-            rx = 1;
+            launch_units = 0;
         };
         for (int i = 0; i < n; ++i) {
             const detr_reduce_desc &d = descs[i];
@@ -815,10 +968,11 @@
                                           d.part_stride % ((long long)d.ts_bm * d.ts_bn) == 0),
                          "splitk_reduce_many: entry %d has a malformed tile-ordered slab description", i);
             bool small;
-            reduce_plan(r, small);
+            const long long u = reduce_plan(r, small);
             if (small != (pass == 0)) continue;
+            units[cnt] = u;
+            launch_units += u;
             R.r[cnt++] = r;
-            rx = (unsigned)r.nblocks > rx ? (unsigned)r.nblocks : rx;
             if (cnt == REDUCE_MANY) flush();
         }
         flush();
diff --git a/detr-tensorflow_amd/csrc/gemm_ring.h b/detr-tensorflow_amd/csrc/gemm_ring.h
--- a/detr-tensorflow_amd/csrc/gemm_ring.h
+++ b/detr-tensorflow_amd/csrc/gemm_ring.h
@@ -24,6 +24,7 @@
 };
 bool gemm_ring_plan(int M, int N, int K, RingPlan &p);
 int gemm_ring_wgrad_launch(const GemmArgs &g, int bm, int bn, int split, hipStream_t s);
+int gemm_ring_wgrad_group_launch(const GemmArgs *g, const int *split, int n, hipStream_t s);
 int gemm_ring_launch(const GemmArgs &g, bool b_kcontig, const RingPlan &p, hipStream_t s);
 bool gemm_ring_f32_plan(int M, int N, int K, RingPlan &p);
 int gemm_ring_f32_launch(const GemmArgs &g, bool b_kcontig, const RingPlan &p, hipStream_t s);
@@ -452,17 +453,15 @@
 }
 
 template <int TM, int TN, int NS>
-__device__ __forceinline__ void gemm_ring_wgrad_body(const RingArgs &ra) {
+__device__ __forceinline__ void gemm_ring_wgrad_body(const GemmArgs &g, const int id) {
     constexpr int BM = 64 * TM, BN = 128 * TN, WGM = 2, WGN = 4;
     static_assert(TM % 2 == 0, "the A image is made of 128-row pieces");
     using T = TileCfg<BM, BN, WGM, WGN>;
     extern __shared__ __attribute__((aligned(1024))) char ring_smem[];
-    const GemmArgs &g = ra.g;
     const int tid = threadIdx.x, lane = tid & 63;
     const int wave = __builtin_amdgcn_readfirstlane(tid >> 6);
     const int wm = wave / WGN, wn = wave % WGN;
     const int tiles = g.tiles_m * g.tiles_n;
-    const int id = xcd_remap((int)blockIdx.x, (int)gridDim.x);
     const int tile = id % tiles, split = id / tiles;
     const int tn = tile % g.tiles_n, tm = tile / g.tiles_n;
     const int m0 = tm * BM, n0 = tn * BN;
@@ -524,8 +523,27 @@
 template <int TM, int TN, int NS>
 __global__ __launch_bounds__(RING_THREADS) void gemm_ring_wgrad_kernel(RingArgs ra) {
 #if defined(__HIP_DEVICE_COMPILE__)
-    gemm_ring_wgrad_body<TM, TN, NS>(ra);
+    gemm_ring_wgrad_body<TM, TN, NS>(ra.g, xcd_remap((int)blockIdx.x, (int)gridDim.x));
 #endif
 }
 
-}
+struct RingWgradGroupArgs {
+    GemmArgs g[GEMM_MAX_GROUP];
+    int work_off[GEMM_MAX_GROUP + 1];
+    int n;
+};
+static_assert(sizeof(RingWgradGroupArgs) <= 4096, "the argument block of the grouped ring weight gradient exceeds the kernel-argument limit");
+
+template <int TM, int TN, int NS>
+__global__ __launch_bounds__(RING_THREADS) void gemm_ring_wgrad_group_kernel(RingWgradGroupArgs G) {
+#if defined(__HIP_DEVICE_COMPILE__)
+    const int L = xcd_remap((int)blockIdx.x, (int)gridDim.x);
+    int m = 0;
+#pragma unroll
+    for (int i = 1; i < GEMM_MAX_GROUP; ++i)
+        if (i < G.n && L >= G.work_off[i]) m = i;
+    gemm_ring_wgrad_body<TM, TN, NS>(G.g[m], L - G.work_off[m]);
+#endif
+}
+
+}
diff --git a/detr-tensorflow_amd/csrc/gemm_ring.hip b/detr-tensorflow_amd/csrc/gemm_ring.hip
--- a/detr-tensorflow_amd/csrc/gemm_ring.hip
+++ b/detr-tensorflow_amd/csrc/gemm_ring.hip
@@ -168,6 +168,34 @@
     return -1;
 }
 
+template <int NS>
+static int ring_wgrad_group_launch_one(const RingWgradGroupArgs &G, int wgs, hipStream_t s) {
+    constexpr int LDS = NS * (128 + 128) * RING_STAGE_ROW;
+    static bool reserved = false;
+    if (!reserved) {
+        hipError_t e = hipFuncSetAttribute(reinterpret_cast<const void *>(gemm_ring_wgrad_group_kernel<2, 1, NS>), hipFuncAttributeMaxDynamicSharedMemorySize, 160 * 1024);
+        DETR_REQUIRE(e == hipSuccess, "gemm (ring wgrad group): cannot reserve LDS: %s", hipGetErrorString(e));
+        reserved = true;
+    }
+    hipLaunchKernelGGL((gemm_ring_wgrad_group_kernel<2, 1, NS>), dim3((unsigned)wgs), dim3(RING_THREADS), (size_t)LDS, s, G);
+    return 0;
+}
+
+int gemm_ring_wgrad_group_launch(const GemmArgs *g, const int *split, int n, hipStream_t s) {
+    DETR_REQUIRE(n >= 2 && n <= GEMM_MAX_GROUP, "gemm (ring wgrad group): 2..%d members", GEMM_MAX_GROUP);
+    RingWgradGroupArgs G;
+    G.n = n;
+    G.work_off[0] = 0;
+    for (int i = 0; i < n; ++i) {
+        G.g[i] = g[i];
+        G.g[i].tiles_m = cdiv(g[i].M, 128);
+        G.g[i].tiles_n = cdiv(g[i].N, 128);
+        G.work_off[i + 1] = G.work_off[i] + G.g[i].tiles_m * G.g[i].tiles_n * split[i];
+    }
+    for (int i = n; i < GEMM_MAX_GROUP; ++i) { G.g[i] = G.g[0]; G.work_off[i + 1] = G.work_off[n]; }
+    return tune(T_RING_NS) == 3 ? ring_wgrad_group_launch_one<3>(G, G.work_off[n], s) : ring_wgrad_group_launch_one<4>(G, G.work_off[n], s);
+}
+
 }
 
 extern "C" int detr_hip_gemm_ring_plan(int32_t M, int32_t N, int32_t K, int32_t *out) {
diff --git a/detr-tensorflow_amd/detr_tf/_hip.py b/detr-tensorflow_amd/detr_tf/_hip.py
--- a/detr-tensorflow_amd/detr_tf/_hip.py
+++ b/detr-tensorflow_amd/detr_tf/_hip.py
@@ -448,11 +448,22 @@
 
 
 _defer_pending = 0
+_slab_bytes = 0
+
+
+def slab_bytes():
+    return _slab_bytes
+
+
+def slab_bytes_reset():
+    global _slab_bytes
+    _slab_bytes = 0
 
 
 def _defer_slab(nbytes):
-    global _defer_top, _defer_chunk_i, _defer_pending
+    global _defer_top, _defer_chunk_i, _defer_pending, _slab_bytes
     nbytes = (int(nbytes) + 255) & ~255
+    _slab_bytes += nbytes
     while True:
         if _defer_chunk_i >= len(_DEFER_CHUNKS):
             _DEFER_CHUNKS.append(torch.empty(max(DEFER_CHUNK, nbytes) // 4, dtype=torch.float32, device=_DEVICE))
@@ -576,6 +587,8 @@
                               (d.C or 0) % 16, rowsum_a is not None, scale is not None and (d.scale or 0) % 16), byref(d)) + 255) & ~255
     if workspace is None and WORKSPACE is not None and split_k > 1 and batch == 1 and DEFER is None:
         need_workspace(ws_need * (ws_slice[1] if ws_slice else 1))
+        global _slab_bytes
+        _slab_bytes += ws_need
     ws = workspace if workspace is not None else WORKSPACE
     if ws is None:
         d.workspace, d.workspace_bytes = None, 0
@@ -635,9 +648,47 @@
 X3_SPLIT_TARGET = int(os.environ.get("DETR_HIP_X3_SPLIT_TARGET", "512"))
 
 
+def _split128_shape(M, N, K):
+    return COMPUTE_BF16 == 1 and ((N >= 128 and K >= 16384) or (M >= 512 and N >= 512 and K >= 4096) or
+                                  (K >= 4096 and ((M >= 256 and N >= 2048) or (M >= 2048 and N >= 256))))
+
+
+def _no_empty_split(ktiles, split):
+    per = -(-ktiles // max(1, split))
+    return -(-ktiles // per)
+
+
+def pick_split_k_group(members, max_split=1024):
+    return _group_plan(members, max_split)[0]
+
+
+def wgrad_group_splits(members, max_split=1024):
+    splits, ring = _group_plan(members, max_split)
+    if sum(ring) < 2:
+        return splits
+    return [max(s, 2) if r and -(-K // 32) >= 2 else s for s, r, (M, N, K) in zip(splits, ring, members)]
+
+
+def _group_plan(members, max_split):
+    solo = [pick_split_k(M, N, K, max_split) for M, N, K in members]
+    ring = [bool(_split128_shape(M, N, K) and s > 1 and M % 8 == 0 and N % 8 == 0) for (M, N, K), s in zip(members, solo)]
+    if sum(ring) < 2:
+        return solo, ring
+    tiles = [-(-M // 128) * -(-N // 128) for M, N, K in members]
+    ktiles = [-(-K // 32) for M, N, K in members]
+    work = sum(t * k for t, k, r in zip(tiles, ktiles, ring) if r)
+    out = []
+    for i, s in enumerate(solo):
+        if ring[i]:
+            s = int(SPLIT_TARGET_128 * ktiles[i] / work + 0.5)
+            s = max(1, min(s, max_split, ktiles[i] // 8 if ktiles[i] >= 16 else 1))
+            s = _no_empty_split(ktiles[i], s)
+        out.append(s)
+    return out, ring
+
+
 def pick_split_k(M, N, K, max_split=1024):
-    if COMPUTE_BF16 == 1 and ((N >= 128 and K >= 16384) or (M >= 512 and N >= 512 and K >= 4096) or
-                         (K >= 4096 and ((M >= 256 and N >= 2048) or (M >= 2048 and N >= 256)))):
+    if _split128_shape(M, N, K):
         tiles = -(-M // 128) * -(-N // 128)
         ktiles = -(-K // 32)
         return int(max(1, min(max(1, SPLIT_TARGET_128 // tiles), max_split, ktiles // 8 if ktiles >= 16 else 1)))
diff --git a/detr-tensorflow_amd/detr_tf/engine.py b/detr-tensorflow_amd/detr_tf/engine.py
--- a/detr-tensorflow_amd/detr_tf/engine.py
+++ b/detr-tensorflow_amd/detr_tf/engine.py
@@ -17,6 +17,7 @@
 LN_EPS = 1e-5
 DEFER_REDUCE = os.environ.get("DETR_HIP_DEFER_REDUCE", "1") != "0"
 WGRAD_STREAM = os.environ.get("DETR_HIP_WGRAD_STREAM", "1") != "0"
+WGRAD_GROUP_STAGES = os.environ.get("DETR_HIP_WGRAD_GROUP_STAGES", "234")
 BWD_FUSED = os.environ.get("DETR_HIP_BWD_FUSED", "1") != "0"
 DROPMASK_AHEAD = int(os.environ.get("DETR_HIP_DROPMASK_AHEAD", "2") or 0)
 QK_ALPHA = float(HD) ** -0.5 * 1.4426950408889634
@@ -260,6 +261,12 @@
             hip.gemm(M_out, N_out, K_red, A, lda, 0, Bm, ldb, 0, C, ldc, alpha=alpha, scale=scale, split_k=sk)
         else:
             hip.gemm(M_out, N_out, K_red, A, lda, 0, Bm, ldb, 0, C, ldc, alpha=alpha, scale=scale, residual=C, ldr=ldc)
+
+    @staticmethod
+    def _wgrad_call(M_out, N_out, K_red, A, lda, Bm, ldb, C, ldc, sk, scale=None, alpha=1.0):
+        if sk > 1:
+            return (M_out, N_out, K_red, A, lda, 0, Bm, ldb, 0, C, ldc), dict(alpha=alpha, scale=scale, split_k=sk)
+        return (M_out, N_out, K_red, A, lda, 0, Bm, ldb, 0, C, ldc), dict(alpha=alpha, scale=scale, residual=C, ldr=ldc)
 
     def _colsum(self, x2d, out, alpha=1.0):
         rows, cols = x2d.shape
@@ -993,15 +1000,19 @@
                     idg_ready = torch.cuda.Event()
                     idg_ready.record(wside)
 
-            def wg3(g=g, fuse3=fuse3, fuse_down=fuse_down):
-                if not fuse3:
+            grouped = str({64: 1, 128: 2, 256: 3, 512: 4}.get(d1, 0)) in WGRAD_GROUP_STAGES and d1 >= 128 and not fuse3 \
+                and not fuse_down and not (tfb and strided)
+
+            def wg3(g=g, fuse3=fuse3, fuse_down=fuse_down, grouped=grouped):
+                if not fuse3 and not grouped:
                     self._wgrad(d1, d2, M_out, y2, d1, g, d2, G[f"{n['conv3']}/kernel"], d2, scale=self.bn_scale[n["bn3"]])
                 bias_grad(n["conv3"], n["bn3"], g, M_out, d2)
                 if m["first"]:
-                    if not fuse_down:
+                    if not fuse_down and not grouped:
                         self._wgrad(cin, d2, M_out, xs, cin, g, d2, G[f"{n['down']}/kernel"], d2, scale=self.bn_scale[n["bnd"]])
                     bias_grad(n["down"], n["bnd"], g, M_out, d2)
-            on_side(wg3)
+            if tfb or not grouped:
+                on_side(wg3)
             dz2 = self.buf(f"scratch:dz2:{d1}:{ho}{par}", (B, ho, wo, d1), adt)
             if fuse3:
                 hip.conv1x1_bwd_fused(g.view(M_out, d2), y2.view(M_out, d1), ws3.view(d1, d2), dz2.view(M_out, d1), G[f"{n['conv3']}/kernel"].view(d1, d2),
@@ -1018,8 +1029,16 @@
             dz1 = self.buf(f"scratch:dz1:{d1}:{h1}{par}", (B, h1, w1, d1), adt)
             hip.conv3x3(1, dz2, ws2, dz1, B, h1, w1, d1, ho, wo, d1, s2, mask=y1, pad=m["dil"], dilation=m["dil"])
 
-            def wg1():
-                self._wgrad(cin, d1, M1, x1, cin, dz1, d1, G[f"{n['conv1']}/kernel"], d1, scale=self.bn_scale[n["bn1"]])
+            def wg1(g=g, grouped=grouped):
+                if grouped:
+                    mem = [(d1, d2, M_out, y2, d1, g, d2, G[f"{n['conv3']}/kernel"], d2, self.bn_scale[n["bn3"]])]
+                    if m["first"]:
+                        mem.append((cin, d2, M_out, xs, cin, g, d2, G[f"{n['down']}/kernel"], d2, self.bn_scale[n["bnd"]]))
+                    mem.append((cin, d1, M1, x1, cin, dz1, d1, G[f"{n['conv1']}/kernel"], d1, self.bn_scale[n["bn1"]]))
+                    sks = hip.wgrad_group_splits([a[:3] for a in mem])
+                    hip.gemm_group([self._wgrad_call(*a[:9], sk, scale=a[9]) for a, sk in zip(mem, sks)])
+                else:
+                    self._wgrad(cin, d1, M1, x1, cin, dz1, d1, G[f"{n['conv1']}/kernel"], d1, scale=self.bn_scale[n["bn1"]])
                 bias_grad(n["conv1"], n["bn1"], dz1, M1, d1)
             on_side(wg1)
             side_mark(bi)
```

After: 527.4. Within noise of the previous version (-0.9%).
